# GLAD-RUC/FastEGNN

Hardware: AMD Instinct MI355X
Metric: graphs/sec (fwd+bwd), Water-3D-like 100k-node frame (higher is better)
Workload: dtype f32; 1 GPU; cfg4 Water-3D-like frame (SURVEY 8d): uniform points, radius graph r=0.035 (mean degree ~19), gravity on; 4-layer FastEGNN H=64, fwd+loss+bwd, CSR build inside the step; nodes=100000, edges=1919172, graphs_per_batch=1, virtual_channels=16, layers=4, parallelism=1 GPU, launch=whole step replayed as one captured HIP graph

## Files before the change

### fastegnn_amd/csrc/api.hip

```cpp
#include <vector>
#include "kernels.h"
#include <initializer_list>

namespace fe {

static thread_local std::string g_last_error;

void set_error(const std::string &msg) { g_last_error = msg; }

int check_launch(const char *what) {
  hipError_t e = hipGetLastError();
  if (e != hipSuccess) {
    set_error(std::string(what) + ": " + hipGetErrorString(e));
    return FASTEGNN_E_LAUNCH;
  }
  return FASTEGNN_OK;
}

bool g_prof_on = false;
namespace {
struct ProfRec { int id; hipEvent_t a, b; };
std::vector<ProfRec> g_recs;
std::vector<hipEvent_t> g_free;
std::vector<hipEvent_t> g_open(K_COUNT, nullptr);
hipEvent_t get_event() {
  if (!g_free.empty()) { hipEvent_t e = g_free.back(); g_free.pop_back(); return e; }
  hipEvent_t e; (void)hipEventCreate(&e); return e;
}
const char *kKernelNames[K_COUNT] = {
  "pack_kernel", "node_pre_fwd_kernel", "graph_xsum_kernel", "graph_pre_fwd_kernel", "edge_fwd_kernel",
  "virt_fwd_kernel", "graph_post_fwd_kernel", "graph_post_bwd_kernel", "virt_bwd_kernel", "graph_pre_bwd_kernel",
  "edge_bwd_kernel", "edge_col_reduce_kernel", "node_pre_bwd_kernel", "wgrad_tn_kernel", "wgrad_small_kernel",
  "build_csr", "misc", "wgrad_reduce_kernel", "virt_bwd_node_kernel", "virt_bwd_gv_kernel"};
}
void prof_begin(int id, hipStream_t st) {
  hipEvent_t e = get_event();
  (void)hipEventRecord(e, st);
  g_open[id] = e;
}
void prof_end(int id, hipStream_t st) {
  hipEvent_t e = get_event();
  (void)hipEventRecord(e, st);
  g_recs.push_back({id, g_open[id], e});
}

static int check_layer(const fastegnn_layer_t *L, const char *who) {
  if (!L) {
    set_error(std::string(who) + ": layer descriptor is null");
    return FASTEGNN_E_INVALID;
  }
  if (L->N < 0 || L->B < 1 || L->C < ((L->flags & FASTEGNN_F_EGNN) ? 0 : 1) || L->ea < 0 || L->na < 0) {
    set_error(std::string(who) + ": bad sizes");
    return FASTEGNN_E_INVALID;
  }
  if (!L->params) {
    set_error(std::string(who) + ": params null");
    return FASTEGNN_E_INVALID;
  }
  {
    const int act = (L->flags >> FASTEGNN_F_ACT_SHIFT) & FASTEGNN_F_ACT_MASK;
#ifdef FE_ACT_GENERIC
    if (act > FASTEGNN_ACT_SOFTPLUS) {
      set_error(std::string(who) + ": unknown activation kind in the flags");
      return FASTEGNN_E_INVALID;
    }
    if ((L->flags & FASTEGNN_F_BF16) && act != FASTEGNN_ACT_SILU) {
      set_error(std::string(who) + ": activations other than SiLU are not combined with the bf16 operand mode");
      return FASTEGNN_E_INVALID;
    }
#else
    if (act != FASTEGNN_ACT_SILU) {
      set_error(std::string(who) + ": this library is compiled for SiLU only; activations selected by the FASTEGNN_F_ACT bits "
                                   "need libfastegnn_hip_act.so (same sources, -DFE_ACT_GENERIC)");
      return FASTEGNN_E_INVALID;
    }
#endif
  }
  return FASTEGNN_OK;
}


enum GuardStage { G_GRAPH_POST, G_VIRT, G_GRAPH_PRE, G_EDGE, G_NODE_PRE };
static int guard_stage(const fastegnn_layer_t *L, const WgradBatch &wb, int stage) {
  const size_t N = (size_t)L->N, BC = (size_t)L->B * L->C, rows = wg_node_rows(L), E = (size_t)L->graph.n_edges;
  const bool det = has(L, FASTEGNN_F_DETERMINISTIC);
  struct W { const float *p; size_t n; const char *what; };
  auto guard = [&](std::initializer_list<W> ws) {
    for (const W &w : ws) {
      const int r = wb.guard_write(w.p, w.n, w.what);
      if (r) return r;
    }
    return (int)FASTEGNN_OK;
  };
  switch (stage) {
    case G_VIRT:
      return guard({{L->g_h, N * H, "g_h"}, {L->g_x, N * 3, "g_x"}, {L->g_A, N * H, "g_A"}, {L->g_aggm, N * H, "g_aggm"},
                    {L->g_aggx, N * 3, "g_aggx"}, {L->g_svel, N, "g_svel"}, {L->g_sgrav, N, "g_sgrav"}, {L->g_Bc, BC * H, "g_Bc"},
                    {L->g_Zp, BC * 3, "g_Zp"}, {L->wg_node, 2 * rows * H, "wg_node[0..2)"},
                    {L->wg_virt, L->wg_virt ? fastegnn_wg_virt_floats_for(L->N, L->C, L->flags) : 0, "wg_virt"}});
    case G_GRAPH_PRE:
      return guard({{L->g_HvT, BC * H, "g_HvT"}, {L->g_Z, BC * 3, "g_Z"}, {L->g_xbar, (size_t)L->B * 4, "g_xbar"},
                    {L->wg_node ? L->wg_node + 7 * rows * H : nullptr, rows * H, "wg_node[7..8)"}});
    case G_EDGE:
      return guard({{L->g_P, N * H, "g_P"}, {L->g_xrow, N * 3, "g_xrow"}, {det ? L->g_QXe : nullptr, E * QXLD, "g_QXe"},
                    {L->g_QX_src, (size_t)L->graph.n_src * QXLD, "g_QX_src"},
                    {L->wg_edge, fastegnn_wg_edge_floats(L->graph.n_edges), "wg_edge"}});
    case G_NODE_PRE:
      return guard({{L->g_h, N * H, "g_h"}, {L->g_x, N * 3, "g_x"}, {L->g_vel, N * 3, "g_vel"},
                    {L->wg_node ? L->wg_node + 2 * rows * H : nullptr, 2 * rows * H, "wg_node[2..4)"}});
    default: return FASTEGNN_OK;
  }
}

}

using namespace fe;

extern "C" int fastegnn_generic_activations(void) {
#ifdef FE_ACT_GENERIC
  return 1;
#else
  return 0;
#endif
}

#define STAGE(name, fn)                                               \
  int name(const fastegnn_layer_t *L, void *stream) {                 \
    int rc = check_layer(L, #name);                                   \
    if (rc) return rc;                                                \
    return fn(L, (hipStream_t)stream);                                \
  }

#define STAGE_B(name, fn, gid)                                        \
  int name(const fastegnn_layer_t *L, void *stream) {                 \
    int rc = check_layer(L, #name);                                   \
    if (rc) return rc;                                                \
    WgradBatch *wb = static_cast<WgradBatch *>(L->wgrad_batch);       \
    if (wb && (rc = guard_stage(L, *wb, gid))) return rc;             \
    return fn(L, (hipStream_t)stream, wb);                            \
  }

extern "C" {

const char *fastegnn_last_error(void) { return g_last_error.c_str(); }
int fastegnn_version(void) { return FASTEGNN_ABI_VERSION; }
size_t fastegnn_wpack_floats(int32_t C) { return wpack_floats(C); }
size_t fastegnn_wg_slab_floats(void) { return wg_slab_floats(); }
size_t fastegnn_sizeof_layer(void) { return sizeof(fastegnn_layer_t); }
size_t fastegnn_sizeof_graph(void) { return sizeof(fastegnn_graph_t); }

STAGE(fastegnn_pack_weights, pack_weights)
STAGE(fastegnn_node_pre_forward, node_pre_forward)
STAGE(fastegnn_graph_xsum, graph_xsum)
STAGE(fastegnn_graph_pre_forward, graph_pre_forward)
STAGE(fastegnn_edge_forward, edge_forward)
STAGE(fastegnn_virt_forward, virt_forward)
STAGE(fastegnn_graph_post_forward, graph_post_forward)
STAGE_B(fastegnn_graph_post_backward, graph_post_backward, G_GRAPH_POST)
STAGE_B(fastegnn_virt_backward, virt_backward, G_VIRT)
STAGE_B(fastegnn_graph_pre_backward, graph_pre_backward, G_GRAPH_PRE)
STAGE_B(fastegnn_edge_backward, edge_backward, G_EDGE)
STAGE(fastegnn_edge_col_reduce, edge_col_reduce)
STAGE_B(fastegnn_node_pre_backward, node_pre_backward, G_NODE_PRE)

int fastegnn_pack_weights_all(const fastegnn_layer_t *const *layers, int32_t n, void *stream) {
  FE_REQUIRE(layers && n >= 1, "fastegnn_pack_weights_all: no layers");
  for (int k = 0; k < n; ++k) {
    int rc = check_layer(layers[k], "fastegnn_pack_weights_all");
    if (rc) return rc;
  }
  return pack_weights_all(layers, n, (hipStream_t)stream);
}

int fastegnn_wgrad_batch_open(const fastegnn_layer_t *L, void *stream, void **batch) {
  FE_REQUIRE(L && batch && L->wg_slab, "fastegnn_wgrad_batch_open: null argument");
  WgradBatch *wb = new WgradBatch(L->wg_slab, (hipStream_t)stream, has(L, FASTEGNN_F_BF16));
  wb->max_split = 384;
  *batch = wb;
  return FASTEGNN_OK;
}
int fastegnn_wgrad_batch_close(void *batch) {
  if (!batch) return FASTEGNN_OK;
  WgradBatch *wb = static_cast<WgradBatch *>(batch);
  const int rc = wb->finish();
  delete wb;
  return rc;
}

int fastegnn_profile_enable(int32_t on) {
  g_prof_on = on != 0;
  return FASTEGNN_OK;
}
int32_t fastegnn_profile_kernels(void) { return K_COUNT; }
const char *fastegnn_profile_name(int32_t id) { return (id >= 0 && id < K_COUNT) ? kKernelNames[id] : ""; }
int fastegnn_profile_collect(double *total_ms, int64_t *launches) {
  if (!total_ms || !launches) { set_error("profile_collect: null output"); return FASTEGNN_E_INVALID; }
  for (int i = 0; i < K_COUNT; ++i) { total_ms[i] = 0.0; launches[i] = 0; }
  for (auto &r : g_recs) {
    float ms = 0.f;
    if (hipEventSynchronize(r.b) != hipSuccess || hipEventElapsedTime(&ms, r.a, r.b) != hipSuccess) {
      set_error("profile_collect: event query failed");
      return FASTEGNN_E_LAUNCH;
    }
    total_ms[r.id] += ms;
    launches[r.id] += 1;
    g_free.push_back(r.a);
    g_free.push_back(r.b);
  }
  g_recs.clear();
  return FASTEGNN_OK;
}

int fastegnn_layer_forward(const fastegnn_layer_t *L, void *stream) {
  int rc = check_layer(L, "fastegnn_layer_forward");
  if (rc) return rc;
  hipStream_t st = (hipStream_t)stream;
  if ((rc = pack_weights(L, st))) return rc;
  if ((rc = node_pre_forward(L, st))) return rc;
  if (has(L, FASTEGNN_F_EGNN)) {
    if ((rc = edge_forward(L, st))) return rc;
    return virt_forward(L, st);
  }
  if ((rc = graph_xsum(L, st))) return rc;
  if ((rc = graph_pre_forward(L, st))) return rc;
  if ((rc = edge_forward(L, st))) return rc;
  if ((rc = virt_forward(L, st))) return rc;
  return graph_post_forward(L, st);
}

int fastegnn_layer_backward(const fastegnn_layer_t *L, void *stream) {
  int rc = check_layer(L, "fastegnn_layer_backward");
  if (rc) return rc;
  hipStream_t st = (hipStream_t)stream;
  FE_REQUIRE(L->wg_slab, "fastegnn_layer_backward: wg_slab null");
  WgradBatch wb(L->wg_slab, st);
  wb.max_split = 384;
  auto guard_virt = [&]() { return guard_stage(L, wb, G_VIRT); };
  auto guard_edge = [&]() { return guard_stage(L, wb, G_EDGE); };
  auto guard_node_pre = [&]() { return guard_stage(L, wb, G_NODE_PRE); };
  if (has(L, FASTEGNN_F_EGNN)) {
    if ((rc = guard_virt())) return rc;
    if ((rc = virt_backward(L, st, &wb))) return rc;
    if ((rc = guard_edge())) return rc;
    if ((rc = edge_backward(L, st, &wb))) return rc;
    if ((rc = edge_col_reduce(L, st))) return rc;
    if ((rc = guard_node_pre())) return rc;
    if ((rc = node_pre_backward(L, st, &wb))) return rc;
    return wb.finish();
  }
  if ((rc = graph_post_backward(L, st, &wb))) return rc;
  if ((rc = guard_virt())) return rc;
  if ((rc = virt_backward(L, st, &wb))) return rc;
  if ((rc = guard_stage(L, wb, G_GRAPH_PRE))) return rc;
  if ((rc = graph_pre_backward(L, st, &wb))) return rc;
  if ((rc = guard_edge())) return rc;
  if ((rc = edge_backward(L, st, &wb))) return rc;
  if ((rc = edge_col_reduce(L, st))) return rc;
  if ((rc = guard_node_pre())) return rc;
  if ((rc = node_pre_backward(L, st, &wb))) return rc;
  return wb.finish();
}

}
```

### fastegnn_amd/csrc/common.h

```cpp
#pragma once
#include <hip/hip_runtime.h>
#include <stdint.h>

namespace fe {

typedef float f32x4 __attribute__((ext_vector_type(4)));

constexpr int H = 64;
constexpr int QXLD = 68;
constexpr int TS = 68;
constexpr int IMG = 4096;
constexpr int FEATW = 8;

struct Vec {
  f32x4 t[4];
};

__device__ __forceinline__ int lane_id() { return threadIdx.x & 63; }
__device__ __forceinline__ int wave_id() { return __builtin_amdgcn_readfirstlane((int)(threadIdx.x >> 6)); }
__device__ __forceinline__ int global_wave_id() { return (int)(blockIdx.x * (blockDim.x >> 6)) + wave_id(); }

__device__ __forceinline__ float sigmoid_f(float z) { return __builtin_amdgcn_rcpf(1.0f + __expf(-z)); }
__device__ __forceinline__ float silu_f(float z) { return z * sigmoid_f(z); }
__device__ __forceinline__ float dsilu_f(float z) {
  float s = sigmoid_f(z);
  return s * (1.0f + z * (1.0f - s));
}
__device__ __forceinline__ void silu_both(float z, float &y, float &d) {
  const float s = sigmoid_f(z);
  y = z * s;
  d = s + y * (1.0f - s);
}
__device__ __forceinline__ float rcp_f(float x) { return __builtin_amdgcn_rcpf(x); }
__device__ __forceinline__ float sqrt_f(float x) { return __builtin_amdgcn_sqrtf(x); }
__device__ __forceinline__ float tanh_f(float z) {
  const float z2 = z * z;
  const float p = z * (1.0f + z2 * (-0.33333334f + z2 * (0.13333334f + z2 * (-0.053968254f + z2 * 0.021869488f))));
  const float s = 2.0f * sigmoid_f(2.0f * z) - 1.0f;
  return fabsf(z) < 0.25f ? p : s;
}

__device__ __forceinline__ Vec vzero() {
  Vec v;
#pragma unroll
  for (int t = 0; t < 4; ++t) v.t[t] = f32x4{0.f, 0.f, 0.f, 0.f};
  return v;
}
template <typename F>
__device__ __forceinline__ Vec vmap(const Vec &a, F f) {
  Vec o;
#pragma unroll
  for (int t = 0; t < 4; ++t)
#pragma unroll
    for (int r = 0; r < 4; ++r) o.t[t][r] = f(a.t[t][r]);
  return o;
}
template <typename F>
__device__ __forceinline__ Vec vmap2(const Vec &a, const Vec &b, F f) {
  Vec o;
#pragma unroll
  for (int t = 0; t < 4; ++t)
#pragma unroll
    for (int r = 0; r < 4; ++r) o.t[t][r] = f(a.t[t][r], b.t[t][r]);
  return o;
}
__device__ __forceinline__ Vec vsilu(const Vec &a) { return vmap(a, [](float z) { return silu_f(z); }); }
__device__ __forceinline__ Vec vsilu_keep_d(Vec &z) {
  Vec y;
#pragma unroll
  for (int t = 0; t < 4; ++t)
#pragma unroll
    for (int r = 0; r < 4; ++r) {
      float yy, dd;
      silu_both(z.t[t][r], yy, dd);
      y.t[t][r] = yy;
      z.t[t][r] = dd;
    }
  return y;
}
struct Act {
  int kind;
  float p;
};
#ifdef FE_ACT_GENERIC
#define FE_ACT(a) , fe::Act{((a).flags >> FASTEGNN_F_ACT_SHIFT) & FASTEGNN_F_ACT_MASK, (a).act_param}
#define FE_ACT_P , Act act
#define FE_ACT_A , act
__device__ __forceinline__ float expm1_f(float z) {
  const float p = z * (1.0f + z * (0.5f + z * (0.16666667f + z * (0.041666668f + z * (0.008333334f + z * 0.0013888889f)))));
  return fabsf(z) < 0.3f ? p : __expf(z) - 1.0f;
}
__device__ __forceinline__ void act_both(float z, Act a, float &y, float &d) {
  switch (a.kind) {
    case FASTEGNN_ACT_RELU: y = z < 0.f ? 0.f : z; d = z > 0.f ? 1.f : 0.f; break;
    case FASTEGNN_ACT_LEAKY_RELU: y = z > 0.f ? z : a.p * z; d = z > 0.f ? 1.f : a.p; break;
    case FASTEGNN_ACT_TANH: y = tanh_f(z); d = 1.0f - y * y; break;
    case FASTEGNN_ACT_SIGMOID: y = sigmoid_f(z); d = y * (1.0f - y); break;
    case FASTEGNN_ACT_ELU: { const float e = a.p * expm1_f(z < 0.f ? z : 0.f); y = z <= 0.f ? e : z; d = z > 0.f ? 1.f : e + a.p; break; }
    case FASTEGNN_ACT_GELU: {
      const float c = 0.5f * (1.0f + erff(z * 0.70710678f));
      y = z * c;
      d = c + z * 0.3989422804f * __expf(-0.5f * z * z);
      break;
    }
    case FASTEGNN_ACT_SOFTPLUS: {
      const float bz = a.p * z;
      const float s = sigmoid_f(bz);
      y = bz <= 20.f ? log1pf(__expf(bz)) / a.p : z;
      d = bz > 20.f ? 1.f : s;
      break;
    }
    default: silu_both(z, y, d); break;
  }
}
__device__ __forceinline__ float act_f(float z, Act a) { float y, d; act_both(z, a, y, d); return y; }
__device__ __forceinline__ float dact_f(float z, Act a) { float y, d; act_both(z, a, y, d); return d; }
__device__ __forceinline__ Vec vsilu(const Vec &v, Act a) { return vmap(v, [a](float z) { return act_f(z, a); }); }
__device__ __forceinline__ Vec vsilu_keep_d(Vec &z, Act a) {
  Vec y;
#pragma unroll
  for (int t = 0; t < 4; ++t)
#pragma unroll
    for (int r = 0; r < 4; ++r) {
      float yy, dd;
      act_both(z.t[t][r], a, yy, dd);
      y.t[t][r] = yy;
      z.t[t][r] = dd;
    }
  return y;
}
__device__ __forceinline__ float dsilu_f(float z, Act a) { return dact_f(z, a); }
#else
#define FE_ACT(a)
#define FE_ACT_P
#define FE_ACT_A
#endif
__device__ __forceinline__ Vec vmul(const Vec &a, const Vec &b) {
  return vmap2(a, b, [](float x, float y) { return x * y; });
}
__device__ __forceinline__ Vec vscale(const Vec &a, float s) { return vmap(a, [s](float z) { return z * s; }); }
__device__ __forceinline__ void vaxpy(Vec &acc, float s, const Vec &a) {
#pragma unroll
  for (int t = 0; t < 4; ++t)
#pragma unroll
    for (int r = 0; r < 4; ++r) acc.t[t][r] = __builtin_fmaf(s, a.t[t][r], acc.t[t][r]);
}
__device__ __forceinline__ void vadd(Vec &acc, const Vec &a) {
#pragma unroll
  for (int t = 0; t < 4; ++t)
#pragma unroll
    for (int r = 0; r < 4; ++r) acc.t[t][r] += a.t[t][r];
}

__device__ __forceinline__ Vec vload_vec(const float *w, int q) {
  Vec v;
#pragma unroll
  for (int t = 0; t < 4; ++t) v.t[t] = *reinterpret_cast<const f32x4 *>(w + 16 * t + 4 * q);
  return v;
}
__device__ __forceinline__ Vec vload_row(const float *row, int q) { return vload_vec(row, q); }
__device__ __forceinline__ void vstore_row(float *row, int q, const Vec &v) {
#pragma unroll
  for (int t = 0; t < 4; ++t) *reinterpret_cast<f32x4 *>(row + 16 * t + 4 * q) = v.t[t];
}

__device__ __forceinline__ Vec vload_u(const float *base, unsigned off) {
  Vec v;
  const unsigned bo = off * 4u;
  const char *p = reinterpret_cast<const char *>(base);
#pragma unroll
  for (int t = 0; t < 4; ++t) v.t[t] = *reinterpret_cast<const f32x4 *>(p + (bo + 64u * t));
  return v;
}
__device__ __forceinline__ void vstore_u(float *base, unsigned off, const Vec &v) {
  const unsigned bo = off * 4u;
  char *p = reinterpret_cast<char *>(base);
#pragma unroll
  for (int t = 0; t < 4; ++t) *reinterpret_cast<f32x4 *>(p + (bo + 64u * t)) = v.t[t];
}

__device__ __forceinline__ float qsum(float p) {
  float a = p, b = p;
  asm("s_nop 1\n\tv_permlane16_swap_b32 %0, %1" : "+v"(a), "+v"(b));
  p = a + b;
  a = p; b = p;
  asm("s_nop 1\n\tv_permlane32_swap_b32 %0, %1" : "+v"(a), "+v"(b));
  return a + b;
}
__device__ __forceinline__ float jsum_dpp(float p) {
  p += __builtin_bit_cast(float, __builtin_amdgcn_update_dpp(0, __builtin_bit_cast(int, p), 0x128, 0xf, 0xf, false));
  p += __builtin_bit_cast(float, __builtin_amdgcn_update_dpp(0, __builtin_bit_cast(int, p), 0x124, 0xf, 0xf, false));
  p += __builtin_bit_cast(float, __builtin_amdgcn_update_dpp(0, __builtin_bit_cast(int, p), 0x122, 0xf, 0xf, false));
  p += __builtin_bit_cast(float, __builtin_amdgcn_update_dpp(0, __builtin_bit_cast(int, p), 0x121, 0xf, 0xf, false));
  return p;
}
__device__ __forceinline__ float jsum(float p) { return jsum_dpp(p); }
__device__ __forceinline__ float jreduce16(const Vec &u) {
  float y[8], z[4], w[2];
#pragma unroll
  for (int k = 0; k < 8; ++k) {
    const float a = u.t[k >> 2][k & 3], b = u.t[(k + 8) >> 2][k & 3];
    asm("s_nop 1\n\tv_add_f32_dpp %0, %1, %1 row_shl:8 row_mask:0xf bank_mask:0x3\n\t"
        "v_add_f32_dpp %0, %2, %2 row_shr:8 row_mask:0xf bank_mask:0xc"
        : "=&v"(y[k]) : "v"(a), "v"(b));
  }
#pragma unroll
  for (int k = 0; k < 4; ++k)
    asm("s_nop 1\n\tv_add_f32_dpp %0, %1, %1 row_shl:4 row_mask:0xf bank_mask:0x5\n\t"
        "v_add_f32_dpp %0, %2, %2 row_shr:4 row_mask:0xf bank_mask:0xa"
        : "=&v"(z[k]) : "v"(y[k]), "v"(y[k + 4]));
  const int lane = lane_id();
  const bool b1 = lane & 2, b0 = lane & 1;
#pragma unroll
  for (int k = 0; k < 2; ++k) {
    const float keep = b1 ? z[k + 2] : z[k], send = b1 ? z[k] : z[k + 2];
    w[k] = keep + __builtin_bit_cast(float, __builtin_amdgcn_update_dpp(0, __builtin_bit_cast(int, send), 0x4e, 0xf, 0xf, false));
  }
  const float keep = b0 ? w[1] : w[0], send = b0 ? w[0] : w[1];
  return keep + __builtin_bit_cast(float, __builtin_amdgcn_update_dpp(0, __builtin_bit_cast(int, send), 0xb1, 0xf, 0xf, false));
}
__device__ __forceinline__ void tile_sum_add(float *row, const Vec &u, int j, int q) {
  const float s = jreduce16(u);
  atomicAdd(&row[16 * (j >> 2) + 4 * q + (j & 3)], s);
}
__device__ __forceinline__ float vdot(const Vec &v, const Vec &w) {
  float p = 0.f;
#pragma unroll
  for (int t = 0; t < 4; ++t)
#pragma unroll
    for (int r = 0; r < 4; ++r) p += v.t[t][r] * w.t[t][r];
  return qsum(p);
}

#ifdef FE_STAMP_VF
__device__ unsigned long long g_vf_stamps[16];
struct VfStamp {
  unsigned long long prev, acc[12];
};
#define VF_TP , VfStamp &_vst
#define VF_TA , _vst
#define VF_T0() VfStamp _vst; for (int _k = 0; _k < 12; ++_k) _vst.acc[_k] = 0; _vst.prev = __builtin_amdgcn_s_memtime();
#define VF_T(i) { __builtin_amdgcn_sched_barrier(0); unsigned long long _t = __builtin_amdgcn_s_memtime(); \
                  _vst.acc[i] += _t - _vst.prev; _vst.prev = _t; __builtin_amdgcn_sched_barrier(0); }
#define VF_TEND() if (lane_id() == 0) { for (int _k = 0; _k < 12; ++_k) atomicAdd(&g_vf_stamps[_k], _vst.acc[_k]); }
#else
#define VF_TP
#define VF_TA
#define VF_T0()
#define VF_T(i)
#define VF_TEND()
#endif
#ifdef FE_STAMP
__device__ unsigned long long g_stamps[16];
struct Stamp {
  unsigned long long prev, acc[12];
};
#define FE_TP , Stamp &_st
#define FE_TA , _st
#define FE_T0() Stamp _st; for (int _k = 0; _k < 12; ++_k) _st.acc[_k] = 0; _st.prev = __builtin_amdgcn_s_memtime();
#define FE_T(i) { __builtin_amdgcn_sched_barrier(0); unsigned long long _t = __builtin_amdgcn_s_memtime(); \
                  _st.acc[i] += _t - _st.prev; _st.prev = _t; __builtin_amdgcn_sched_barrier(0); }
#define FE_TEND() if (lane_id() == 0) { for (int _k = 0; _k < 12; ++_k) atomicAdd(&g_stamps[_k], _st.acc[_k]); }
#elif defined(FE_ISA_MARK)
#define FE_TP
#define FE_TA
#define FE_T0()
#define FE_T(i) { __builtin_amdgcn_sched_barrier(0); asm volatile("; FE_MARK " #i); __builtin_amdgcn_sched_barrier(0); }
#define FE_TEND()
#else
#define FE_TP
#define FE_TA
#define FE_T0()
#define FE_T(i)
#define FE_TEND()
#endif

__host__ __device__ __forceinline__ int img_index(int o, int k) {
  int t = o >> 4, i = o & 15, tp = k >> 4, q = (k >> 2) & 3, r = k & 3;
  return ((t * 4 + tp) * 64 + q * 16 + i) * 4 + r;
}

__device__ __forceinline__ void gemm64(const float *img, const Vec &in, Vec &acc) {
  const f32x4 *ip = reinterpret_cast<const f32x4 *>(img) + lane_id();
#pragma unroll
  for (int tp = 0; tp < 4; ++tp) {
    f32x4 a[4];
#pragma unroll
    for (int t = 0; t < 4; ++t) a[t] = ip[(t * 4 + tp) * 64];
#pragma unroll
    for (int r = 0; r < 4; ++r)
#pragma unroll
      for (int t = 0; t < 4; ++t)
        acc.t[t] = __builtin_amdgcn_mfma_f32_16x16x4f32(a[t][r], in.t[tp][r], acc.t[t], 0, 0, 0);
  }
}

typedef unsigned u32x4 __attribute__((ext_vector_type(4)));
typedef __bf16 bf16x8 __attribute__((ext_vector_type(8)));
constexpr int IMG3 = 3 * 2048;

struct Split {
  u32x4 p[3][2];
};
__device__ __forceinline__ unsigned f2u(float x) { return __builtin_bit_cast(unsigned, x); }
__device__ __forceinline__ unsigned part_pack(float &a0, float &a1) {
  typedef float f32x2_ __attribute__((ext_vector_type(2)));
  typedef __bf16 bf16x2_ __attribute__((ext_vector_type(2)));
  const unsigned p = __builtin_bit_cast(unsigned, __builtin_convertvector(f32x2_{a0, a1}, bf16x2_));
  a0 -= __builtin_bit_cast(float, p << 16);
  a1 -= __builtin_bit_cast(float, p & 0xffff0000u);
  return p;
}
__host__ __device__ __forceinline__ int img3_index(int part, int o, int k) {
  const int t = o >> 4, i = o & 15, tile = k >> 4, q = (k >> 2) & 3, r = k & 3;
  const int s = tile >> 1, e = ((tile & 1) << 2) | r;
  return part * 2048 + ((t * 2 + s) * 64 + q * 16 + i) * 4 + (e >> 1);
}
__device__ __forceinline__ unsigned split_word(float w0, float w1, int part) {
  float a0 = w0, a1 = w1;
  unsigned p = 0;
  for (int k = 0; k <= part; ++k) p = part_pack(a0, a1);
  return p;
}
__device__ __forceinline__ Split vsplit(const Vec &v) {
  Split S;
#pragma unroll
  for (int s = 0; s < 2; ++s) {
    float x[8];
#pragma unroll
    for (int e = 0; e < 8; ++e) x[e] = v.t[2 * s + (e >> 2)][e & 3];
#pragma unroll
    for (int w = 0; w < 4; ++w) {
      S.p[0][s][w] = part_pack(x[2 * w], x[2 * w + 1]);
      S.p[1][s][w] = part_pack(x[2 * w], x[2 * w + 1]);
      S.p[2][s][w] = part_pack(x[2 * w], x[2 * w + 1]);
    }
  }
  return S;
}
__device__ __forceinline__ void gemm64_x3(const unsigned *img3, const Split &in, Vec &acc) {
  const u32x4 *ip = reinterpret_cast<const u32x4 *>(img3) + lane_id();
  __builtin_amdgcn_sched_barrier(0);
  u32x4 fr[2][3];
#pragma unroll
  for (int p = 0; p < 3; ++p) fr[0][p] = ip[p * 512];
  __builtin_amdgcn_sched_group_barrier(0x100, 3, 0);
#pragma unroll
  for (int g = 0; g < 8; ++g) {
    const int s = g >> 2, t = g & 3, cb = g & 1;
    if (g + 1 < 8) {
      const int sn = (g + 1) >> 2, tn = (g + 1) & 3;
#pragma unroll
      for (int p = 0; p < 3; ++p) fr[cb ^ 1][p] = ip[p * 512 + (tn * 2 + sn) * 64];
      __builtin_amdgcn_sched_group_barrier(0x100, 3, 0);
    }
    const bf16x8 ah = __builtin_bit_cast(bf16x8, fr[cb][0]), am = __builtin_bit_cast(bf16x8, fr[cb][1]),
                 al = __builtin_bit_cast(bf16x8, fr[cb][2]);
    const bf16x8 xh = __builtin_bit_cast(bf16x8, in.p[0][s]);
    const bf16x8 xm = __builtin_bit_cast(bf16x8, in.p[1][s]);
    const bf16x8 xl = __builtin_bit_cast(bf16x8, in.p[2][s]);
    acc.t[t] = __builtin_amdgcn_mfma_f32_16x16x32_bf16(al, xh, acc.t[t], 0, 0, 0);
    acc.t[t] = __builtin_amdgcn_mfma_f32_16x16x32_bf16(am, xm, acc.t[t], 0, 0, 0);
    acc.t[t] = __builtin_amdgcn_mfma_f32_16x16x32_bf16(ah, xl, acc.t[t], 0, 0, 0);
    acc.t[t] = __builtin_amdgcn_mfma_f32_16x16x32_bf16(am, xh, acc.t[t], 0, 0, 0);
    acc.t[t] = __builtin_amdgcn_mfma_f32_16x16x32_bf16(ah, xm, acc.t[t], 0, 0, 0);
    acc.t[t] = __builtin_amdgcn_mfma_f32_16x16x32_bf16(ah, xh, acc.t[t], 0, 0, 0);
    __builtin_amdgcn_sched_group_barrier(0x008, 6, 0);
  }
  __builtin_amdgcn_sched_barrier(0);
}
__device__ __forceinline__ void gemm64_x3(const unsigned *img3, const Vec &in, Vec &acc) { gemm64_x3(img3, vsplit(in), acc); }

typedef float f32x2 __attribute__((ext_vector_type(2)));
typedef __bf16 bf16x2 __attribute__((ext_vector_type(2)));
__device__ __forceinline__ unsigned pack_rne(float x0, float x1) {
  return __builtin_bit_cast(unsigned, __builtin_convertvector(f32x2{x0, x1}, bf16x2));
}
__device__ __forceinline__ float round_bf(float x) { return (float)(__bf16)x; }
struct BfOp {
  u32x4 p[2];
};
__device__ __forceinline__ BfOp vpack_bf(const Vec &v) {
  BfOp B;
#pragma unroll
  for (int s = 0; s < 2; ++s)
#pragma unroll
    for (int w = 0; w < 4; ++w) {
      const int e = 2 * w;
      B.p[s][w] = pack_rne(v.t[2 * s + (e >> 2)][e & 3], v.t[2 * s + ((e + 1) >> 2)][(e + 1) & 3]);
    }
  return B;
}
__device__ __forceinline__ Vec vround(const Vec &v) { return vmap(v, [](float z) { return round_bf(z); }); }
__device__ __forceinline__ void gemm64_b1(const unsigned *img3, const BfOp &in, Vec &acc) {
  const u32x4 *ip = reinterpret_cast<const u32x4 *>(img3) + lane_id();
#pragma unroll
  for (int s = 0; s < 2; ++s) {
    const bf16x8 x = __builtin_bit_cast(bf16x8, in.p[s]);
#pragma unroll
    for (int t = 0; t < 4; ++t)
      acc.t[t] = __builtin_amdgcn_mfma_f32_16x16x32_bf16(__builtin_bit_cast(bf16x8, ip[(t * 2 + s) * 64]), x, acc.t[t], 0, 0, 0);
  }
}

constexpr int RM_RS = 144;
constexpr int RM_PART = 64 * RM_RS;
constexpr int RM_BYTES = 3 * RM_PART;
constexpr int RM_WORDS = RM_BYTES / 4;
typedef unsigned u32x2 __attribute__((ext_vector_type(2)));
typedef short s16x4 __attribute__((ext_vector_type(4)));
__device__ __forceinline__ u32x2 lds_tr_read(const char *p) {
  return __builtin_bit_cast(u32x2, __builtin_amdgcn_ds_read_tr16_b64_v4i16(
                                       (__attribute__((address_space(3))) s16x4 *)(p)));
}
template <bool TR>
__device__ __forceinline__ bf16x8 rm_frag(const char *img, int part, int t, int s) {
  const int l = lane_id(), i = l & 15, q = l >> 4;
  u32x2 lo, hi;
  if constexpr (TR) {
    const char *p = img + part * RM_PART + (32 * s + 4 * q + (i >> 2)) * RM_RS + (16 * t + 4 * (i & 3)) * 2;
    lo = lds_tr_read(p);
    hi = lds_tr_read(p + 16 * RM_RS);
  } else {
    const char *p = img + part * RM_PART + (16 * t + i) * RM_RS + (32 * s + 4 * q) * 2;
    typedef __attribute__((address_space(3))) const volatile u32x2 *lds_vu32x2;
    lo = *(lds_vu32x2)(p);
    hi = *(lds_vu32x2)(p + 32);
  }
  return __builtin_bit_cast(bf16x8, u32x4{lo[0], lo[1], hi[0], hi[1]});
}
template <bool TR, bool PIPE = true>
__device__ __forceinline__ void gemm64_x3_rm(const char *img, const Split &in, Vec &acc) {
  if constexpr (!PIPE) {
#pragma unroll
  for (int s = 0; s < 2; ++s)
#pragma unroll
    for (int t = 0; t < 4; ++t) {
      const bf16x8 ah = rm_frag<TR>(img, 0, t, s), am = rm_frag<TR>(img, 1, t, s), al = rm_frag<TR>(img, 2, t, s);
      const bf16x8 xh = __builtin_bit_cast(bf16x8, in.p[0][s]);
      const bf16x8 xm = __builtin_bit_cast(bf16x8, in.p[1][s]);
      const bf16x8 xl = __builtin_bit_cast(bf16x8, in.p[2][s]);
      acc.t[t] = __builtin_amdgcn_mfma_f32_16x16x32_bf16(al, xh, acc.t[t], 0, 0, 0);
      acc.t[t] = __builtin_amdgcn_mfma_f32_16x16x32_bf16(am, xm, acc.t[t], 0, 0, 0);
      acc.t[t] = __builtin_amdgcn_mfma_f32_16x16x32_bf16(ah, xl, acc.t[t], 0, 0, 0);
      acc.t[t] = __builtin_amdgcn_mfma_f32_16x16x32_bf16(am, xh, acc.t[t], 0, 0, 0);
      acc.t[t] = __builtin_amdgcn_mfma_f32_16x16x32_bf16(ah, xm, acc.t[t], 0, 0, 0);
      acc.t[t] = __builtin_amdgcn_mfma_f32_16x16x32_bf16(ah, xh, acc.t[t], 0, 0, 0);
    }
  } else {
  __builtin_amdgcn_sched_barrier(0);
  bf16x8 fr[2][3];
#pragma unroll
  for (int p = 0; p < 3; ++p) fr[0][p] = rm_frag<TR>(img, p, 0, 0);
  __builtin_amdgcn_sched_group_barrier(0x100, 6, 0);
#pragma unroll
  for (int g = 0; g < 8; ++g) {
    const int s = g >> 2, t = g & 3, cb = g & 1;
    if (g + 1 < 8) {
#pragma unroll
      for (int p = 0; p < 3; ++p) fr[cb ^ 1][p] = rm_frag<TR>(img, p, (g + 1) & 3, (g + 1) >> 2);
      __builtin_amdgcn_sched_group_barrier(0x100, 6, 0);
    }
    const bf16x8 ah = fr[cb][0], am = fr[cb][1], al = fr[cb][2];
    const bf16x8 xh = __builtin_bit_cast(bf16x8, in.p[0][s]);
    const bf16x8 xm = __builtin_bit_cast(bf16x8, in.p[1][s]);
    const bf16x8 xl = __builtin_bit_cast(bf16x8, in.p[2][s]);
    acc.t[t] = __builtin_amdgcn_mfma_f32_16x16x32_bf16(al, xh, acc.t[t], 0, 0, 0);
    acc.t[t] = __builtin_amdgcn_mfma_f32_16x16x32_bf16(am, xm, acc.t[t], 0, 0, 0);
    acc.t[t] = __builtin_amdgcn_mfma_f32_16x16x32_bf16(ah, xl, acc.t[t], 0, 0, 0);
    acc.t[t] = __builtin_amdgcn_mfma_f32_16x16x32_bf16(am, xh, acc.t[t], 0, 0, 0);
    acc.t[t] = __builtin_amdgcn_mfma_f32_16x16x32_bf16(ah, xm, acc.t[t], 0, 0, 0);
    acc.t[t] = __builtin_amdgcn_mfma_f32_16x16x32_bf16(ah, xh, acc.t[t], 0, 0, 0);
    __builtin_amdgcn_sched_group_barrier(0x008, 6, 0);
  }
  __builtin_amdgcn_sched_barrier(0);
  }
}
template <bool TR>
__device__ __forceinline__ void gemm64_b1_rm(const char *img, const BfOp &in, Vec &acc) {
#pragma unroll
  for (int s = 0; s < 2; ++s) {
    const bf16x8 x = __builtin_bit_cast(bf16x8, in.p[s]);
#pragma unroll
    for (int t = 0; t < 4; ++t) acc.t[t] = __builtin_amdgcn_mfma_f32_16x16x32_bf16(rm_frag<TR>(img, 0, t, s), x, acc.t[t], 0, 0, 0);
  }
}

struct Split8 {
  u32x4 h, m, l;
};
__device__ __forceinline__ Split8 split8(const float (&x_)[8]) {
  float x[8];
#pragma unroll
  for (int e = 0; e < 8; ++e) x[e] = x_[e];
  Split8 S;
#pragma unroll
  for (int w = 0; w < 4; ++w) {
    S.h[w] = part_pack(x[2 * w], x[2 * w + 1]);
    S.m[w] = part_pack(x[2 * w], x[2 * w + 1]);
    S.l[w] = part_pack(x[2 * w], x[2 * w + 1]);
  }
  return S;
}
__device__ __forceinline__ u32x4 round8(const float (&x)[8]) {
  u32x4 r;
#pragma unroll
  for (int w = 0; w < 4; ++w) r[w] = pack_rne(x[2 * w], x[2 * w + 1]);
  return r;
}

typedef _Float16 f16x8 __attribute__((ext_vector_type(8)));
typedef _Float16 f16x2 __attribute__((ext_vector_type(2)));
constexpr float F2_UP = 2048.f, F2_DOWN = 1.0f / 2048.f;
struct Split2 {
  u32x4 p[2][2];
};
__device__ __forceinline__ void part2_pack(float a0, float a1, unsigned &ph, unsigned &pl) {
  const unsigned h = __builtin_bit_cast(unsigned, __builtin_convertvector(f32x2{a0, a1}, f16x2));
  float r0, r1;
  asm("v_fma_mix_f32 %0, %1, -1.0, %2 op_sel_hi:[1,0,0]" : "=v"(r0) : "v"(h), "v"(a0));
  asm("v_fma_mix_f32 %0, %1, -1.0, %2 op_sel:[1,0,0] op_sel_hi:[1,0,0]" : "=v"(r1) : "v"(h), "v"(a1));
  unsigned l;
  asm("v_fma_mixlo_f16 %0, %1, %3, 0\n\tv_fma_mixhi_f16 %0, %2, %3, 0\n\ts_nop 1" : "=&v"(l) : "v"(r0), "v"(r1), "s"(F2_UP));
  ph = h;
  pl = l;
}
__device__ __forceinline__ unsigned split2_word(float w0, float w1, int part) {
  unsigned h, l;
  part2_pack(w0, w1, h, l);
  return part == 0 ? h : l;
}
#ifdef FE_HAZARD_SELFTEST
#define FE_MIX_PAD ""
#else
#define FE_MIX_PAD "s_nop 1"
#endif
template <bool IN_PLACE = false>
__device__ __forceinline__ void mix_pack4(const float (&r)[8], float sc, unsigned (&l)[4]) {
  if constexpr (IN_PLACE) {
#pragma unroll
    for (int w = 0; w < 4; ++w) l[w] = f2u(r[2 * w]);
    asm("v_fma_mixlo_f16 %0, %0, %8, 0\n\tv_fma_mixhi_f16 %0, %4, %8, 0\n\t"
        "v_fma_mixlo_f16 %1, %1, %8, 0\n\tv_fma_mixhi_f16 %1, %5, %8, 0\n\t"
        "v_fma_mixlo_f16 %2, %2, %8, 0\n\tv_fma_mixhi_f16 %2, %6, %8, 0\n\t"
        "v_fma_mixlo_f16 %3, %3, %8, 0\n\tv_fma_mixhi_f16 %3, %7, %8, 0\n\t"
        FE_MIX_PAD
        : "+v"(l[0]), "+v"(l[1]), "+v"(l[2]), "+v"(l[3])
        : "v"(r[1]), "v"(r[3]), "v"(r[5]), "v"(r[7]), "v"(sc));
  } else {
  asm("v_fma_mixlo_f16 %0, %4, %12, 0\n\tv_fma_mixhi_f16 %0, %5, %12, 0\n\t"
      "v_fma_mixlo_f16 %1, %6, %12, 0\n\tv_fma_mixhi_f16 %1, %7, %12, 0\n\t"
      "v_fma_mixlo_f16 %2, %8, %12, 0\n\tv_fma_mixhi_f16 %2, %9, %12, 0\n\t"
      "v_fma_mixlo_f16 %3, %10, %12, 0\n\tv_fma_mixhi_f16 %3, %11, %12, 0\n\t"
      FE_MIX_PAD
      : "=&v"(l[0]), "=&v"(l[1]), "=&v"(l[2]), "=&v"(l[3])
      : "v"(r[0]), "v"(r[1]), "v"(r[2]), "v"(r[3]), "v"(r[4]), "v"(r[5]), "v"(r[6]), "v"(r[7]), "v"(sc));
  }
}
__device__ __forceinline__ Split2 vsplit2(const Vec &v) {
  Split2 S;
#pragma unroll
  for (int s = 0; s < 2; ++s) {
    float r[8];
#pragma unroll
    for (int w = 0; w < 4; ++w) {
      const int e = 2 * w;
      const float a0 = v.t[2 * s + (e >> 2)][e & 3], a1 = v.t[2 * s + ((e + 1) >> 2)][(e + 1) & 3];
      const unsigned h = __builtin_bit_cast(unsigned, __builtin_convertvector(f32x2{a0, a1}, f16x2));
      asm("v_fma_mix_f32 %0, %1, -1.0, %2 op_sel_hi:[1,0,0]" : "=v"(r[e]) : "v"(h), "v"(a0));
      asm("v_fma_mix_f32 %0, %1, -1.0, %2 op_sel:[1,0,0] op_sel_hi:[1,0,0]" : "=v"(r[e + 1]) : "v"(h), "v"(a1));
      S.p[0][s][w] = h;
    }
    unsigned l[4];
    mix_pack4<true>(r, F2_UP, l);
#pragma unroll
    for (int w = 0; w < 4; ++w) S.p[1][s][w] = l[w];
  }
  return S;
}
#ifndef FE_F2_PIPE_FWD
#define FE_F2_PIPE_FWD 1
#endif
template <bool PIPE = false>
__device__ __forceinline__ void gemm64_f2(const unsigned *img3, const Split2 &in, Vec &acc, int off4 = 0) {
  const u32x4 *ip = reinterpret_cast<const u32x4 *>(img3) + (lane_id() + off4);
  const f16x8 xh0 = __builtin_bit_cast(f16x8, in.p[0][0]), xh1 = __builtin_bit_cast(f16x8, in.p[0][1]);
  const f16x8 xl0 = __builtin_bit_cast(f16x8, in.p[1][0]), xl1 = __builtin_bit_cast(f16x8, in.p[1][1]);
  if constexpr (PIPE && FE_F2_PIPE_FWD != 0) {
  __builtin_amdgcn_sched_barrier(0);
  u32x4 fr[2][4];
#pragma unroll
  for (int k = 0; k < 4; ++k) fr[0][k] = ip[(k >> 1) * 512 + (k & 1) * 64];
  __builtin_amdgcn_sched_group_barrier(0x100, 4, 0);
  f32x4 lo_p = {0.f, 0.f, 0.f, 0.f}, hi_p = {0.f, 0.f, 0.f, 0.f};
#pragma unroll
  for (int t = 0; t < 4; ++t) {
    const int cb = t & 1;
// ... 437 lines not shown
```

### fastegnn_amd/csrc/kernels.h

```cpp
#pragma once
#include <hip/hip_runtime.h>
#include <string>
#include "../../include/fastegnn_hip.h"
#include "common.h"

namespace fe {

void set_error(const std::string &msg);
int check_launch(const char *what);

#define FE_REQUIRE(cond, msg)            \
  do {                                   \
    if (!(cond)) {                       \
      fe::set_error(msg);                \
      return FASTEGNN_E_INVALID;         \
    }                                    \
  } while (0)

inline bool has(const fastegnn_layer_t *L, int f) { return (L->flags & f) != 0; }
inline int cdiv(long a, long b) { return (int)((a + b - 1) / b); }

enum KernelId {
  K_PACK = 0, K_NODE_PRE_FWD, K_XSUM, K_GRAPH_PRE_FWD, K_EDGE_FWD, K_VIRT_FWD, K_GRAPH_POST_FWD,
  K_GRAPH_POST_BWD, K_VIRT_BWD, K_GRAPH_PRE_BWD, K_EDGE_BWD, K_COL_REDUCE, K_NODE_PRE_BWD,
  K_WGRAD_TN, K_WGRAD_SMALL, K_CSR, K_MISC, K_WGRAD_REDUCE, K_VIRT_BWD_NODE, K_VIRT_BWD_GV, K_COUNT
};
extern bool g_prof_on;
void prof_begin(int id, hipStream_t st);
void prof_end(int id, hipStream_t st);
struct ProfScope {
  int id; hipStream_t st; bool on;
  ProfScope(int id_, hipStream_t st_) : id(id_), st(st_), on(g_prof_on) { if (on) prof_begin(id, st); }
  ~ProfScope() { if (on) prof_end(id, st); }
};

constexpr int WGV_PAD = 16;
constexpr int WG_MAX_JOBS = 24;
constexpr int WG_SLABS = 8192;
struct WgJob {
  const float *G, *T;
  float *dW, *db;
  long M, sG, sT, sW;
  int ldg, ldt, lddw, c0, ks, kmax, rows_per_wg, nsplit, nb, wg_begin, slab_begin;
  int round;
};
struct WgTable {
  WgJob job[WG_MAX_JOBS];
  float *slab, *slab_b;
  int n_jobs;
};
struct WgradBatch {
  WgTable tab;
  hipStream_t st;
  int n_wg, n_slab, max_nb;
  bool round;
  int min_rows;
  int max_split;
  int slab_base, slab_cap;
  int slab_top;
  bool planned;
  WgradBatch(float *slab, hipStream_t st, bool round_bf16 = false, int slab_base = 0, int slab_cap = WG_SLABS / 2);
  int add(const float *G, int ldg, const float *T, int ldt, long M, float *dW, int lddw, int c0, int ks, float *db,
          int nb = 1, long sG = 0, long sT = 0, long sW = 0, int kmax = 64);
  int plan();
  int add_slabs(float *dW, int lddw, int c0, int ks, float *db, int nsplit, int *slab_begin);
  int add_slabs_ext(const float *ext, float *dW, int lddw, int c0, int ks, int nsplit, int nb, long sW);
  int finish();
  int guard_write(const float *p, size_t n, const char *what) const;
};
inline size_t wg_slab_floats() { return (size_t)WG_SLABS * (IMG + H); }
int launch_dgrad_small(const float *G, long N, int kf, const float *W, int ldw, int c0, float *g_in, int accumulate,
                       hipStream_t st);
int launch_wgrad_small(const float *G, int ldg, const float *F, int ldf, int kf, long M, float *dW, int lddw, int c0,
                       hipStream_t st);

int csr_chunk_count(int E);
void launch_chunk_rows(const int32_t *rowptr, int n_rows, int n_chunks, int32_t *chunk_row, hipStream_t st);

int pack_weights(const fastegnn_layer_t *L, hipStream_t st);
int pack_weights_all(const fastegnn_layer_t *const *layers, int n, hipStream_t st);
int node_pre_forward(const fastegnn_layer_t *L, hipStream_t st);
int graph_xsum(const fastegnn_layer_t *L, hipStream_t st);
int graph_pre_forward(const fastegnn_layer_t *L, hipStream_t st);
int edge_forward(const fastegnn_layer_t *L, hipStream_t st);
int virt_forward(const fastegnn_layer_t *L, hipStream_t st);
int graph_post_forward(const fastegnn_layer_t *L, hipStream_t st);
int graph_post_backward(const fastegnn_layer_t *L, hipStream_t st, WgradBatch *shared = nullptr);
int virt_backward(const fastegnn_layer_t *L, hipStream_t st, WgradBatch *shared = nullptr);
int graph_pre_backward(const fastegnn_layer_t *L, hipStream_t st, WgradBatch *shared = nullptr);
int edge_backward(const fastegnn_layer_t *L, hipStream_t st, WgradBatch *shared = nullptr);
size_t virt_pc_wg_floats(size_t N, size_t C);
bool virt_cs_applies(long N, int C, int flags);
size_t virt_cs_wg_floats(size_t C);
int edge_col_reduce(const fastegnn_layer_t *L, hipStream_t st);
int node_pre_backward(const fastegnn_layer_t *L, hipStream_t st, WgradBatch *shared = nullptr);
inline size_t wg_node_rows(const fastegnn_layer_t *L) { const size_t bc = (size_t)L->B * L->C; return (size_t)L->N > bc ? (size_t)L->N : bc; }

}
```

### fastegnn_amd/csrc/layer_bwd.hip

```cpp
#include "stages.h"

namespace fe {

__device__ __forceinline__ Vec vdsilu_mul(const Vec &g, const Vec &z FE_ACT_P) {
  return vmap2(g, z, [=](float a, float b) { return a * dsilu_f(b FE_ACT_A); });
}

__device__ __forceinline__ void vec_reduce_lds(float *red_row, const Vec &acc, int j, int q) {
#pragma unroll
  for (int t = 0; t < 4; ++t)
#pragma unroll
    for (int r = 0; r < 4; ++r) {
      float s = jsum(acc.t[t][r]);
      if (j == 0) atomicAdd(&red_row[16 * t + 4 * q + r], s);
    }
}

struct GraphPostBwdArgs {
  const float *xsum, *HvT, *poolV, *g_Z_out, *g_HvT_out, *wpack, *b5;
  float *g_Z, *g_HvT, *g_poolV, *g_poolX, *wg_u, *wg_gz5, *wg_pm;
  int B, C, flags;
  float act_param = 0.f;
};
__global__ __launch_bounds__(256) void graph_post_bwd_kernel(GraphPostBwdArgs a) {
  const bool bf = a.flags & FASTEGNN_F_BF16;
  auto rb = [&](const Vec &v) { return bf ? vround(v) : v; };
  const int l = lane_id(), j = l & 15, q = l >> 4;
  const int wave = global_wave_id(), nwaves = (gridDim.x * blockDim.x) >> 6;
  const int M = a.B * a.C, ntiles = (M + 15) >> 4;
  for (int i = blockIdx.x * blockDim.x + threadIdx.x; i < a.B * 3 * a.C; i += gridDim.x * blockDim.x) {
    const int b = i / (3 * a.C);
    const float g = a.g_Z_out[i];
    a.g_Z[i] = g;
    a.g_poolX[i] = g / fmaxf(a.xsum[b * 4 + 3], 1.f);
  }
  if (a.flags & FASTEGNN_F_RF) {
    for (int i = blockIdx.x * blockDim.x + threadIdx.x; i < M * H; i += gridDim.x * blockDim.x) {
      a.g_HvT[i] = a.g_HvT_out[i];
      a.g_poolV[i] = 0.f;
    }
    return;
  }
  for (int tile = wave; tile < ntiles; tile += nwaves) {
    const int m = tile * 16 + j;
    const bool valid = m < M;
    const int mc = valid ? m : M - 1;
    const int b = mc / a.C;
    const float inv = 1.0f / fmaxf(a.xsum[b * 4 + 3], 1.f);
    const Vec hv = vload_row(a.HvT + (size_t)mc * H, q);
    const Vec pm = vscale(vload_row(a.poolV + (size_t)mc * H, q), inv);
    Vec z5 = vload_vec(a.b5, q);
    gemm64(a.wpack + (size_t)I_W5A * IMG, rb(hv), z5);
    gemm64(a.wpack + (size_t)I_W5B * IMG, rb(pm), z5);
    const Vec g_out = vload_row(a.g_HvT_out + (size_t)mc * H, q);
    Vec g_u = vzero();
    gemm64(a.wpack + (size_t)I_W6T * IMG, rb(g_out), g_u);
    const Vec g_z5 = vdsilu_mul(g_u, z5 FE_ACT(a));
    Vec g_hv = (a.flags & FASTEGNN_F_RESIDUAL) ? g_out : vzero();
    gemm64(a.wpack + (size_t)I_W5AT * IMG, rb(g_z5), g_hv);
    Vec g_pm = vzero();
    gemm64(a.wpack + (size_t)I_W5BT * IMG, rb(g_z5), g_pm);
    if (valid) {
      vstore_row(a.wg_u + (size_t)m * H, q, vsilu(z5 FE_ACT(a)));
      vstore_row(a.wg_gz5 + (size_t)m * H, q, g_z5);
      vstore_row(a.wg_pm + (size_t)m * H, q, pm);
      vstore_row(a.g_HvT + (size_t)m * H, q, g_hv);
      vstore_row(a.g_poolV + (size_t)m * H, q, vscale(g_pm, inv));
    }
  }
}

__global__ __launch_bounds__(256) void graph_post_bwd_coords_kernel(const float *xsum, const float *g_Z_out, float *g_Z, float *g_poolX,
                                                                    float *g_HvT, int B, int C) {
  for (int i = blockIdx.x * blockDim.x + threadIdx.x; i < B * 3 * C; i += gridDim.x * blockDim.x) {
    const int b = i / (3 * C);
    const float g = g_Z_out[i];
    g_Z[i] = g;
    g_poolX[i] = g / fmaxf(xsum[b * 4 + 3], 1.f);
  }
  for (int i = blockIdx.x * blockDim.x + threadIdx.x; i < B * C * H; i += gridDim.x * blockDim.x) g_HvT[i] = 0.f;
}

int graph_post_backward(const fastegnn_layer_t *L, hipStream_t st, WgradBatch *shared) {
  if (!L->g_HvT_out && !has(L, FASTEGNN_F_RF)) {
    FE_REQUIRE(!L->g_h_out, "graph_post_backward: g_HvT_out is null and g_h_out is not (both null: no gradient for h / Hv; otherwise neither)");
    FE_REQUIRE(L->xsum && L->g_Z_out && L->g_Z && L->g_HvT && L->g_poolX, "graph_post_backward: null buffer");
    int grid = cdiv((long)L->B * L->C * H, 256);
    if (grid > 256) grid = 256;
    if (grid < 1) grid = 1;
    { ProfScope _ps_graph_post_bwd_kernel(K_GRAPH_POST_BWD, st); hipLaunchKernelGGL(graph_post_bwd_coords_kernel, dim3(grid), dim3(256), 0, st, L->xsum, L->g_Z_out, L->g_Z, L->g_poolX, L->g_HvT, L->B, L->C); }
    return check_launch("graph_post_bwd_coords_kernel");
  }
  FE_REQUIRE(L->xsum && L->HvT && L->poolV && L->g_Z_out && L->g_HvT_out && L->g_Z && L->g_HvT && L->g_poolV &&
                 L->g_poolX && L->wg_node && L->grads && L->wpack,
             "graph_post_backward: null buffer");
  const long M = (long)L->B * L->C;
  float *wg_gp = L->wg_node + 4 * wg_node_rows(L) * H;
  float *wg_u = wg_gp, *wg_gz5 = wg_gp + M * H, *wg_pm = wg_gp + 2 * M * H;
  GraphPostBwdArgs a{L->xsum, L->HvT, L->poolV, L->g_Z_out, L->g_HvT_out, L->wpack, L->params[FASTEGNN_P_NODEV0_B],
                     L->g_Z, L->g_HvT, L->g_poolV, L->g_poolX, wg_u, wg_gz5, wg_pm, L->B, L->C, L->flags, L->act_param};
  int grid = cdiv(cdiv(M, 16), 4);
  if (grid > 256) grid = 256;
  if (grid < 1) grid = 1;
  { ProfScope _ps_graph_post_bwd_kernel(K_GRAPH_POST_BWD, st); hipLaunchKernelGGL(graph_post_bwd_kernel, dim3(grid), dim3(256), 0, st, a); }
  int rc = check_launch("graph_post_bwd_kernel");
  if (rc) return rc;
  if (has(L, FASTEGNN_F_RF)) return FASTEGNN_OK;
  float *const *g = L->grads;
  WgradBatch local(L->wg_slab, st);
  WgradBatch &wb = shared ? *shared : local;
  wb.round = has(L, FASTEGNN_F_BF16);
  if ((rc = wb.add(L->g_HvT_out, H, wg_u, H, M, g[FASTEGNN_P_NODEV2_W], H, 0, 1, g[FASTEGNN_P_NODEV2_B]))) return rc;
  if ((rc = wb.add(wg_gz5, H, L->HvT, H, M, g[FASTEGNN_P_NODEV0_W], 2 * H, 0, 1, g[FASTEGNN_P_NODEV0_B]))) return rc;
  if ((rc = wb.add(wg_gz5, H, wg_pm, H, M, g[FASTEGNN_P_NODEV0_W], 2 * H, H, 1, nullptr))) return rc;
  return shared ? FASTEGNN_OK : wb.finish();
}


struct GraphPreBwdArgs {
  const float *xsum, *Z, *g_Bc, *g_Zp, *V0W;
  float *g_Z, *g_HvT, *g_xbar, *wg_mxt;
  int B, C, bf16;
};
constexpr int GPB_SPLIT = 4;
__global__ __launch_bounds__(256) void graph_pre_bwd_kernel(GraphPreBwdArgs a) {
  extern __shared__ float sm[];
  const int C = a.C, b = blockIdx.x, ld = 2 * H + 1 + C;
  const int i0 = blockIdx.y * 256 + threadIdx.x, istep = 256 * gridDim.y;
  float *mz = sm;
  float *gmX = sm + 3 * C;
  float *gmz = gmX + C * C;
  const float cnt = fmaxf(a.xsum[b * 4 + 3], 1.f);
  for (int i = threadIdx.x; i < 3 * C; i += 256) mz[i] = a.Z[(size_t)b * 3 * C + i] - a.xsum[b * 4 + i / C] / cnt;
  __syncthreads();
  for (int i = i0; i < C * H; i += istep) {
    int c = i >> 6, d = i & 63;
    float v = 0.f;
    if (d < C) v = mz[c] * mz[d] + mz[C + c] * mz[C + d] + mz[2 * C + c] * mz[2 * C + d];
    a.wg_mxt[((size_t)b * C + c) * H + d] = v;
  }
  for (int i = i0; i < C * H; i += istep) {
    int c = i >> 6, k = i & 63;
    const float *gb = a.g_Bc + ((size_t)b * C + c) * H;
    float acc = 0.f;
    if (a.bf16) { for (int o = 0; o < H; ++o) acc += round_bf(gb[o]) * round_bf(a.V0W[(size_t)o * ld + H + k]); }
    else { for (int o = 0; o < H; ++o) acc += gb[o] * a.V0W[(size_t)o * ld + H + k]; }
    a.g_HvT[((size_t)b * C + c) * H + k] += acc;
  }
  for (int i = threadIdx.x; i < C * C; i += 256) {
    int cp = i / C, c = i % C;
    const float *gb = a.g_Bc + ((size_t)b * C + c) * H;
    float acc = 0.f;
    for (int o = 0; o < H; ++o) acc += gb[o] * a.V0W[(size_t)o * ld + 2 * H + 1 + cp];
    gmX[cp * C + c] = acc;
  }
  __syncthreads();
  for (int i = threadIdx.x; i < 3 * C; i += 256) {
    int k = i / C, c = i % C;
    float acc = 0.f;
    for (int d = 0; d < C; ++d) acc += (gmX[c * C + d] + gmX[d * C + c]) * mz[k * C + d];
    gmz[i] = acc;
    if (i % gridDim.y == blockIdx.y) a.g_Z[(size_t)b * 3 * C + i] += acc + a.g_Zp[(size_t)b * 3 * C + i];
  }
  __syncthreads();
  if (threadIdx.x < 3 && blockIdx.y == 0) {
    float acc = 0.f;
    for (int c = 0; c < C; ++c) acc += gmz[threadIdx.x * C + c];
    a.g_xbar[b * 3 + threadIdx.x] = -acc / cnt;
  }
}
int graph_pre_backward(const fastegnn_layer_t *L, hipStream_t st, WgradBatch *shared) {
  FE_REQUIRE(L->xsum && L->Z && L->HvT && L->g_Bc && L->g_Zp && L->g_Z && L->g_HvT && L->g_xbar && L->wg_node && L->grads,
             "graph_pre_backward: null buffer");
  const long M = (long)L->B * L->C;
  float *wg_mxt = L->wg_node + 7 * wg_node_rows(L) * H;
  GraphPreBwdArgs a{L->xsum, L->Z, L->g_Bc, L->g_Zp, L->params[FASTEGNN_P_VIRT0_W], L->g_Z, L->g_HvT, L->g_xbar, wg_mxt,
                    L->B, L->C, has(L, FASTEGNN_F_BF16) ? 1 : 0};
  const size_t lds = (size_t)(6 * L->C + L->C * L->C) * sizeof(float);
  { ProfScope _ps_graph_pre_bwd_kernel(K_GRAPH_PRE_BWD, st); hipLaunchKernelGGL(graph_pre_bwd_kernel, dim3(L->B, GPB_SPLIT), dim3(256), lds, st, a); }
  int rc = check_launch("graph_pre_bwd_kernel");
  if (rc) return rc;
  float *const *g = L->grads;
  const int ld = 2 * H + 1 + L->C;
  WgradBatch local(L->wg_slab, st);
  WgradBatch &wb = shared ? *shared : local;
  wb.round = has(L, FASTEGNN_F_BF16);
  if ((rc = wb.add(L->g_Bc, H, L->HvT, H, M, g[FASTEGNN_P_VIRT0_W], ld, H, 1, g[FASTEGNN_P_VIRT0_B]))) return rc;
  wb.round = false;
  if ((rc = wb.add(L->g_Bc, H, wg_mxt, H, M, g[FASTEGNN_P_VIRT0_W], ld, 2 * H + 1, 1, nullptr, 1, 0, 0, 0, L->C))) return rc;
  return shared ? FASTEGNN_OK : wb.finish();
}

struct EdgeBwdArgs {
  EdgeArgs f;
  const float *g_aggm, *g_aggx;
  float *g_P, *g_xrow, *g_QXe;
  float *g_QXs_atomic;
  float *g_ea;
  float *d_wx2, *d_attw, *d_attb, *d_bx2;
  float *d_wr, *d_we;
  int ld_e0, C;
  float *slab, *slab_b;
  int slab_w2, slab_wx1;
  float *cons_scratch;
};
#ifndef FE_PC_PRIO
#define FE_PC_PRIO 3
#endif

#ifndef FE_PC_WAVES
#define FE_PC_WAVES 8
#endif
constexpr int PC_WAVES = FE_PC_WAVES;
constexpr int PC_CONS = 3, PC_CONS2 = 7;
constexpr int PC_PROD = PC_WAVES - 2;
#ifndef FE_PC_CONS32
#define FE_PC_CONS32 1
#endif
#ifndef FE_PC_RING
#define FE_PC_RING 3
#endif
constexpr int PC_RING = FE_PC_RING;
#ifndef FE_PC_FLUSH
#define FE_PC_FLUSH 48
#endif
constexpr int PC_FLUSH = FE_PC_FLUSH;
constexpr int PC_RS = 68;
constexpr int PC_SLOT = 2 * 16 * PC_RS;
template <int MODE> constexpr int pc_img_floats() { return 2 * (rm_lds_bytes<MODE>() / 4); }
enum { PC_HEAD = 0, PC_TOTAL = 2, PC_FILLED = 4, PC_DRAINED = 4 + 2 * PC_RING, PC_CTRL = 4 + 4 * PC_RING };
#ifdef FE_SAFE_WAITS
__device__ __forceinline__ int lds_ld(const int *p) { return __hip_atomic_load(p, __ATOMIC_ACQUIRE, __HIP_MEMORY_SCOPE_WORKGROUP); }
__device__ __forceinline__ void lds_st(int *p, int v) { __hip_atomic_store(p, v, __ATOMIC_RELEASE, __HIP_MEMORY_SCOPE_WORKGROUP); }
#else
__device__ __forceinline__ int lds_ld(const int *p) { return __atomic_load_n(p, __ATOMIC_RELAXED); }
__device__ __forceinline__ void lds_st(int *p, int v) { __atomic_store_n(p, v, __ATOMIC_RELAXED); }
#endif
__device__ __forceinline__ void pc_tile_store(float *tile, int j, int q, const Vec &v) {
#pragma unroll
  for (int t = 0; t < 4; ++t) *reinterpret_cast<f32x4 *>(tile + j * PC_RS + 16 * t + 4 * q) = v.t[t];
}
template <int MODE, int EA>
__global__ __launch_bounds__(64 * PC_WAVES) void edge_bwd_pc_kernel(EdgeBwdArgs A) {
  extern __shared__ __attribute__((aligned(16))) float lds[];
#ifdef FE_ISA_CONST
  A.f.flags = FE_ISA_CONST; A.f.ea_dim = 2; A.f.bx2 = nullptr; A.f.attw = nullptr; A.g_ea = nullptr; A.d_bx2 = nullptr;
#endif
  const EdgeArgs &a = A.f;
  float *img = lds;
  float *vec = lds + pc_img_floats<MODE>();
  float *tiles = vec + EV_COUNT * H;
  float *ring = tiles + PC_PROD * 16 * TS;
  int *ctrl = reinterpret_cast<int *>(ring + 2 * PC_RING * PC_SLOT);
  {
    constexpr int RMS = rm_lds_bytes<MODE>();
    const char *src = wpack_rm(a.wpack, A.C, (MODE == GM_F16 ? RM_F16 : 0) + 3);
    for (int i = threadIdx.x; i < 2 * (RMS / 16); i += blockDim.x) {
      const int im = i / (RMS / 16), k = i % (RMS / 16);
      reinterpret_cast<u32x4 *>(reinterpret_cast<char *>(img) + im * RMS)[k] = reinterpret_cast<const u32x4 *>(src + (size_t)im * RM_BYTES)[k];
    }
  }
  edge_load_vecs(vec, a);
  if (threadIdx.x < PC_CTRL) ctrl[threadIdx.x] = 0;
  __syncthreads();
  const int l = lane_id(), j = l & 15, q = l >> 4, wv = wave_id();
  const bool consumer = wv == PC_CONS || wv == PC_CONS2;
  const int ckind = wv == PC_CONS ? 0 : 1;
  const int pw = wv - (wv > PC_CONS ? 1 : 0) - (wv > PC_CONS2 ? 1 : 0);
  float *pt = tiles + (consumer ? 0 : pw) * 16 * TS;
  const int wave = (int)blockIdx.x * PC_PROD + pw, nwaves = (int)gridDim.x * PC_PROD;
  const bool mean = !(a.flags & FASTEGNN_F_COORDS_SUM);
  float accW[8] = {0.f, 0.f, 0.f, 0.f, 0.f, 0.f, 0.f, 0.f};
  const bool tanh_on = a.flags & FASTEGNN_F_TANH, att_on = a.flags & FASTEGNN_F_ATTENTION,
             norm_on = a.flags & FASTEGNN_F_NORMALIZE;
  Vec acc_wx2 = vzero(), acc_att = vzero();
  float acc_attb = 0.f, acc_bx2 = 0.f;
  FE_T0()
  int r0 = 0, r1 = 0, e0 = 0, e1 = 0;
  if (!consumer) {
    const int c0 = (int)((long)wave * a.n_chunks / nwaves), c1 = (int)((long)(wave + 1) * a.n_chunks / nwaves);
    r0 = a.chunk_row[c0];
    r1 = a.chunk_row[c1];
    if (r0 < r1) {
      e0 = a.rowptr[r0];
      e1 = a.rowptr[r1];
      if (l == 0) atomicAdd(&ctrl[PC_TOTAL], (e1 - e0 + 15) >> 4);
    }
  }
  __syncthreads();
  auto publish = [&](int kind, const Vec &Gv, const Vec &Tv) {
    int tk = 0;
    if (l == 0) tk = atomicAdd(&ctrl[PC_HEAD + kind], 1);
    tk = __builtin_amdgcn_readfirstlane(tk);
    const int sl = tk % PC_RING, round = tk / PC_RING;
    while (lds_ld(&ctrl[PC_DRAINED + kind * PC_RING + sl]) != round) __builtin_amdgcn_s_sleep(2);
    __builtin_amdgcn_fence(__ATOMIC_ACQUIRE, "workgroup", "local");
    float *slot = ring + (kind * PC_RING + sl) * PC_SLOT;
    pc_tile_store(slot, j, q, Gv);
    pc_tile_store(slot + 16 * PC_RS, j, q, Tv);
    __builtin_amdgcn_fence(__ATOMIC_RELEASE, "workgroup", "local");
    if (l == 0) lds_st(&ctrl[PC_FILLED + kind * PC_RING + sl], round + 1);
  };
  constexpr bool CONS32 = MODE == GM_F16 && FE_PC_CONS32 != 0;
  if (CONS32 && consumer) {
    if constexpr (CONS32) {
#if FE_PC_PRIO
    __builtin_amdgcn_s_setprio(FE_PC_PRIO);
#endif
    const int total = lds_ld(&ctrl[PC_TOTAL]);
    WgAcc32 acc;
    wg32_zero(acc);
    WgScale sG{0}, sT{0};
    double bs[2] = {0., 0.};
    auto scp = [&](int blk, int e4) {
      char *b = reinterpret_cast<char *>(A.cons_scratch + ((size_t)blockIdx.x * 2 + ckind) * IMG) + (size_t)((blk * 4 + e4) * 64 * 16);
      asm volatile("" : "+s"(b));
      return reinterpret_cast<f32x4 *>(b + (unsigned)l * 16u);
    };
    bool flushed = false;
    const size_t sl = (size_t)(ckind == 0 ? A.slab_w2 : A.slab_wx1) + blockIdx.x;
    auto flush = [&](bool last) {
      const float ig = sG.inv(), it = sT.inv();
      float *slab_dst = A.slab + sl * IMG;
#pragma unroll
      for (int bo = 0; bo < 2; ++bo)
#pragma unroll
        for (int bk = 0; bk < 2; ++bk)
#pragma unroll
          for (int e4 = 0; e4 < 4; ++e4) {
            f32x4 v;
#pragma unroll
            for (int r = 0; r < 4; ++r) v[r] = (acc.c[bo][bk][4 * e4 + r] * ig) * it;
            f32x4 *d = scp(bo * 2 + bk, e4);
            if (flushed) v += *d;
            if (!last) {
              *d = v;
            } else {
#pragma unroll
              for (int r = 0; r < 4; ++r) slab_dst[(32 * bo + 8 * e4 + 4 * (l >> 5) + r) * H + 32 * bk + (l & 31)] = v[r];
            }
#pragma unroll
            for (int r = 0; r < 4; ++r) acc.c[bo][bk][4 * e4 + r] = 0.f;
          }
    };
    int since = 0;
    for (int done = 0; done < total; ++done) {
      const int s0 = done % PC_RING, r0w = done / PC_RING;
      while (lds_ld(&ctrl[PC_FILLED + ckind * PC_RING + s0]) != r0w + 1) __builtin_amdgcn_s_sleep(1);
      __builtin_amdgcn_fence(__ATOMIC_ACQUIRE, "workgroup", "local");
      const float *g0 = ring + (ckind * PC_RING + s0) * PC_SLOT;
      float xg[2][8], xt[2][8];
      wg32_read<PC_RS>(g0, xg);
      wg32_read<PC_RS>(g0 + 16 * PC_RS, xt);
      __builtin_amdgcn_fence(__ATOMIC_RELEASE, "workgroup", "local");
      __builtin_amdgcn_s_waitcnt(0xc07f);
      if (l == 0) lds_st(&ctrl[PC_DRAINED + ckind * PC_RING + s0], r0w + 1);
      const float f = sG.update_lazy(xg) * sT.update_lazy(xt);
      if (f != 1.f) wg32_scale_acc(acc, f);
      const WgOp32 G = wg32_split(xg, sG.scale()), T = wg32_split(xt, sT.scale());
#pragma unroll
      for (int b = 0; b < 2; ++b)
        bs[b] += (double)(((xg[b][0] + xg[b][1]) + (xg[b][2] + xg[b][3])) + ((xg[b][4] + xg[b][5]) + (xg[b][6] + xg[b][7])));
      wg32_mma(acc, G, T);
      if (++since >= PC_FLUSH && done + 1 < total) {
        flush(false);
        flushed = true;
        since = 0;
      }
    }
    flush(true);
#pragma unroll
    for (int b = 0; b < 2; ++b) {
      double s0 = bs[b];
      s0 += __shfl_xor(s0, 32);
      if (l < 32) A.slab_b[sl * H + 32 * b + l] = (float)s0;
    }
    }
  } else if (consumer) {
#if FE_PC_PRIO
    __builtin_amdgcn_s_setprio(FE_PC_PRIO);
#endif
    const int total = lds_ld(&ctrl[PC_TOTAL]);
    f32x4 accA[4][4];
    double bsA[4] = {0., 0., 0., 0.};
#pragma unroll
    for (int ti = 0; ti < 4; ++ti)
#pragma unroll
      for (int tk = 0; tk < 4; ++tk) accA[ti][tk] = f32x4{0.f, 0.f, 0.f, 0.f};
    auto contract = [&](int kind, int tk, f32x4 (&acc)[4][4], double (&bs)[4]) {
      const int s0 = tk % PC_RING, r0w = tk / PC_RING;
      const bool two = tk + 1 < total;
      const int s1 = (tk + 1) % PC_RING, r1w = (tk + 1) / PC_RING;
      while (lds_ld(&ctrl[PC_FILLED + kind * PC_RING + s0]) != r0w + 1) __builtin_amdgcn_s_sleep(2);
      if (two)
        while (lds_ld(&ctrl[PC_FILLED + kind * PC_RING + s1]) != r1w + 1) __builtin_amdgcn_s_sleep(2);
      __builtin_amdgcn_fence(__ATOMIC_ACQUIRE, "workgroup", "local");
      const float *g0 = ring + (kind * PC_RING + s0) * PC_SLOT, *g1 = ring + (kind * PC_RING + s1) * PC_SLOT;
      float xb[4][8], xa[4][8];
#pragma unroll
      for (int t = 0; t < 4; ++t)
#pragma unroll
        for (int e = 0; e < 4; ++e) {
          xb[t][e] = g0[16 * PC_RS + (4 * q + e) * PC_RS + 16 * t + j];
          xb[t][4 + e] = two ? g1[16 * PC_RS + (4 * q + e) * PC_RS + 16 * t + j] : 0.f;
          xa[t][e] = g0[(4 * q + e) * PC_RS + 16 * t + j];
          xa[t][4 + e] = two ? g1[(4 * q + e) * PC_RS + 16 * t + j] : 0.f;
        }
      __builtin_amdgcn_fence(__ATOMIC_RELEASE, "workgroup", "local");
      __builtin_amdgcn_s_waitcnt(0xc07f);
      if (l == 0) {
        lds_st(&ctrl[PC_DRAINED + kind * PC_RING + s0], r0w + 1);
        if (two) lds_st(&ctrl[PC_DRAINED + kind * PC_RING + s1], r1w + 1);
      }
      Split8 B[4];
#pragma unroll
      for (int t = 0; t < 4; ++t) {
        if constexpr (MODE == GM_BF16) B[t].h = round8(xb[t]);
        else B[t] = split8(xb[t]);
      }
#pragma unroll
      for (int ti = 0; ti < 4; ++ti) {
        const float (&x)[8] = xa[ti];
        bs[ti] += (double)(((x[0] + x[1]) + (x[2] + x[3])) + ((x[4] + x[5]) + (x[6] + x[7])));
        if constexpr (MODE == GM_BF16) {
          const bf16x8 ah = __builtin_bit_cast(bf16x8, round8(x));
#pragma unroll
          for (int t = 0; t < 4; ++t)
            acc[ti][t] = __builtin_amdgcn_mfma_f32_16x16x32_bf16(ah, __builtin_bit_cast(bf16x8, B[t].h), acc[ti][t], 0, 0, 0);
          continue;
        }
        const Split8 Aop = split8(x);
        const bf16x8 ah = __builtin_bit_cast(bf16x8, Aop.h), am = __builtin_bit_cast(bf16x8, Aop.m),
                     al = __builtin_bit_cast(bf16x8, Aop.l);
#pragma unroll
        for (int t = 0; t < 4; ++t) {
          const bf16x8 bh = __builtin_bit_cast(bf16x8, B[t].h), bm = __builtin_bit_cast(bf16x8, B[t].m),
                       bl = __builtin_bit_cast(bf16x8, B[t].l);
          f32x4 c = acc[ti][t];
          c = __builtin_amdgcn_mfma_f32_16x16x32_bf16(al, bh, c, 0, 0, 0);
          c = __builtin_amdgcn_mfma_f32_16x16x32_bf16(am, bm, c, 0, 0, 0);
          c = __builtin_amdgcn_mfma_f32_16x16x32_bf16(ah, bl, c, 0, 0, 0);
          c = __builtin_amdgcn_mfma_f32_16x16x32_bf16(am, bh, c, 0, 0, 0);
          c = __builtin_amdgcn_mfma_f32_16x16x32_bf16(ah, bm, c, 0, 0, 0);
          c = __builtin_amdgcn_mfma_f32_16x16x32_bf16(ah, bh, c, 0, 0, 0);
          acc[ti][t] = c;
        }
      }
    };
    auto ready = [&](int kind, int done) {
      const int s0 = done % PC_RING, s1 = (done + 1) % PC_RING;
      if (lds_ld(&ctrl[PC_FILLED + kind * PC_RING + s0]) != done / PC_RING + 1) return false;
      return done + 1 >= total || lds_ld(&ctrl[PC_FILLED + kind * PC_RING + s1]) == (done + 1) / PC_RING + 1;
    };
    f32x4 *sc = reinterpret_cast<f32x4 *>(A.cons_scratch + ((size_t)blockIdx.x * 2 + ckind) * IMG) + l;
    double bs_tot[4] = {0., 0., 0., 0.};
    bool flushed = false;
    int done = 0, since = 0;
    while (done < total) {
      if (ready(ckind, done)) {
        contract(ckind, done, accA, bsA);
        done += 2;
        since += 2;
        if (since >= PC_FLUSH && done < total) {
#pragma unroll
          for (int ti = 0; ti < 4; ++ti) {
#pragma unroll
            for (int tk2 = 0; tk2 < 4; ++tk2) {
              f32x4 *d = sc + (ti * 4 + tk2) * 64;
              if (flushed) accA[ti][tk2] += *d;
              *d = accA[ti][tk2];
              accA[ti][tk2] = f32x4{0.f, 0.f, 0.f, 0.f};
            }
            bs_tot[ti] += bsA[ti];
            bsA[ti] = 0.;
          }
          flushed = true;
          since = 0;
        }
      } else {
        __builtin_amdgcn_s_sleep(1);
      }
// ... 529 lines not shown
```

### fastegnn_amd/csrc/layer_fwd.hip

```cpp
#include <cstdlib>
#include "stages.h"

namespace fe {

struct NodePreArgs {
  const float *h, *x, *wpack;
  const float *b1, *bv0, *wv2, *bv2, *bg0, *wg2, *bg2;
  float *P, *QX, *A, *svel, *sgrav;
  int N, gravity, has_vel;
  const float *vel, *wv0;
  int C;
  int flags = 0;
  float act_param = 0.f;
};

template <int MODE>
__global__ __launch_bounds__(64 * NODE_PRE_WAVES) void node_pre_fwd_kernel(NodePreArgs a) {
  extern __shared__ __attribute__((aligned(16))) float lds[];
  unsigned *img = reinterpret_cast<unsigned *>(lds);
  float *vec = lds + 5 * IMG3;
  const int nimg = a.gravity ? 5 : 4;
  load_images_x3(img, wpack_x3(a.wpack, a.C, I_W1A), nimg);
  if constexpr (edge_fold_first<MODE>()) { for (int i = threadIdx.x; i < H; i += blockDim.x) vec[i] = a.b1 ? a.b1[i] * LOG2E_F : 0.f; }
  else load_floats(vec + 0 * H, a.b1, H);
  load_floats(vec + 1 * H, a.bv0, H);
  load_floats(vec + 2 * H, a.wv2, H);
  load_floats(vec + 3 * H, a.bg0, H);
  load_floats(vec + 4 * H, a.wg2, H);
  load_floats(vec + 5 * H, a.wv0, H);
  __syncthreads();
  const int l = lane_id(), j = l & 15, q = l >> 4;
  const int wave = global_wave_id(), nwaves = (gridDim.x * blockDim.x) >> 6;
  const int ntiles = (a.N + 15) >> 4;
  const float bv2 = (a.has_vel || a.wv0) ? a.bv2[0] : 0.f;
  const float bg2 = a.gravity ? a.bg2[0] : 0.f;
  for (int tile = wave; tile < ntiles; tile += nwaves) {
    const int n = tile * 16 + j;
    const bool valid = n < a.N;
    const int nc = valid ? n : a.N - 1;
    const typename OperandOf<MODE>::type hv = make_operand<MODE>(vload_row(a.h + (size_t)nc * H, q));
    Vec acc = vload_vec(vec, q);
    gemm_op<MODE>(img, 0, hv, acc);
    if (valid) vstore_row(a.P + (size_t)n * H, q, acc);
    acc = vzero();
    gemm_op<MODE>(img, 1, hv, acc);
    if (valid) {
      vstore_row(a.QX + (size_t)n * QXLD, q, acc);
      if (q == 0) {
        f32x4 xv = {a.x[(size_t)n * 3], a.x[(size_t)n * 3 + 1], a.x[(size_t)n * 3 + 2], 0.f};
        *reinterpret_cast<f32x4 *>(a.QX + (size_t)n * QXLD + H) = xv;
      }
    }
    acc = vzero();
    gemm_op<MODE>(img, 2, hv, acc);
    if (valid) vstore_row(a.A + (size_t)n * H, q, acc);
    float s = 0.f;
    if (a.has_vel) {
      acc = vload_vec(vec + 1 * H, q);
      gemm_op<MODE>(img, 3, hv, acc);
      s = vdot(vsilu(acc FE_ACT(a)), vload_vec(vec + 2 * H, q)) + bv2;
    } else if (a.wv0) {
      const float vx = a.vel[(size_t)nc * 3], vy = a.vel[(size_t)nc * 3 + 1], vz = a.vel[(size_t)nc * 3 + 2];
      acc = vload_vec(vec + 1 * H, q);
      vaxpy(acc, sqrt_f(vx * vx + vy * vy + vz * vz), vload_vec(vec + 5 * H, q));
      s = vdot(vsilu(acc FE_ACT(a)), vload_vec(vec + 2 * H, q)) + bv2;
    }
    if (valid && q == 0) a.svel[n] = s;
    if (a.gravity) {
      acc = vload_vec(vec + 3 * H, q);
      gemm_op<MODE>(img, 4, hv, acc);
      s = vdot(vsilu(acc FE_ACT(a)), vload_vec(vec + 4 * H, q)) + bg2;
      if (valid && q == 0) a.sgrav[n] = s;
    }
  }
}

int node_pre_forward(const fastegnn_layer_t *L, hipStream_t st) {
  FE_REQUIRE(L->h && L->x && L->wpack && L->P && L->QX && L->A && L->svel, "node_pre_forward: null buffer");
  if (L->N == 0) return FASTEGNN_OK;
  const bool grav = has(L, FASTEGNN_F_GRAVITY);
  FE_REQUIRE(!grav || L->sgrav, "node_pre_forward: sgrav null");
  const float *const *p = L->params;
  NodePreArgs a{L->h, L->x, L->wpack, p[FASTEGNN_P_EDGE0_B], p[FASTEGNN_P_VEL0_B], p[FASTEGNN_P_VEL2_W],
                p[FASTEGNN_P_VEL2_B], p[FASTEGNN_P_GRAV0_B], p[FASTEGNN_P_GRAV2_W], p[FASTEGNN_P_GRAV2_B],
                L->P, L->QX, L->A, L->svel, L->sgrav, L->N, grav ? 1 : 0,
                (p[FASTEGNN_P_VEL0_W] && !has(L, FASTEGNN_F_RF)) ? 1 : 0,
                L->vel, has(L, FASTEGNN_F_RF) ? p[FASTEGNN_P_VEL0_W] : nullptr, L->C, L->flags, L->act_param};
  FE_REQUIRE(!has(L, FASTEGNN_F_RF) || (L->vel && p[FASTEGNN_P_VEL0_W] && p[FASTEGNN_P_VEL0_B] && p[FASTEGNN_P_VEL2_W] &&
                                         p[FASTEGNN_P_VEL2_B]),
             "node_pre_forward: FastRF needs vel and the coord_mlp_vel parameters");
  const int ntiles = (L->N + 15) / 16;
  int grid = cdiv(ntiles, NODE_PRE_WAVES);
  if (grid > 256) grid = 256;
  const size_t lds = (5 * IMG3 + 6 * H) * sizeof(float);
  {
    ProfScope _ps_node_pre_fwd_kernel(K_NODE_PRE_FWD, st);
    if (has(L, FASTEGNN_F_BF16)) hipLaunchKernelGGL(node_pre_fwd_kernel<GM_BF16>, dim3(grid), dim3(64 * NODE_PRE_WAVES), lds, st, a);
    else hipLaunchKernelGGL(node_pre_fwd_kernel<GM_NODE_PRE_FWD>, dim3(grid), dim3(64 * NODE_PRE_WAVES), lds, st, a);
  }
  return check_launch("node_pre_fwd_kernel");
}

#ifndef FE_XSUM_PER_WAVE
#define FE_XSUM_PER_WAVE 1024
#endif
constexpr int XSUM_PER_WAVE = FE_XSUM_PER_WAVE;
__global__ __launch_bounds__(256) void graph_xsum_kernel(const float *x, const int32_t *batch, int N, float *xsum, int PER_WAVE) {
  const int l = lane_id();
  const int n0 = global_wave_id() * PER_WAVE, n1 = min(N, n0 + PER_WAVE);
  if (n0 >= n1) return;
  int cur = -1;
  float s[4] = {0.f, 0.f, 0.f, 0.f};
  auto flush = [&]() {
    float mine = 0.f;
#pragma unroll
    for (int k = 0; k < 4; ++k) {
      float v = s[k];
      for (int off = 32; off > 0; off >>= 1) v += __shfl_xor(v, off);
      if (l == k) mine = v;
      s[k] = 0.f;
    }
    if (l < 4) atomicAdd(&xsum[cur * 4 + l], mine);
  };
  for (int base = n0; base < n1; base += 64) {
    const int n = base + l;
    const bool ok = n < n1;
    const int b = batch[ok ? n : n1 - 1];
    const int bf = __builtin_amdgcn_readfirstlane(b), bl = batch[min(base + 63, n1 - 1)];
    float xv[3] = {0.f, 0.f, 0.f};
    if (ok) { xv[0] = x[(size_t)n * 3]; xv[1] = x[(size_t)n * 3 + 1]; xv[2] = x[(size_t)n * 3 + 2]; }
    if (bf == bl) {
      if (bf != cur) {
        if (cur >= 0) flush();
        cur = bf;
      }
      s[0] += xv[0]; s[1] += xv[1]; s[2] += xv[2]; s[3] += ok ? 1.f : 0.f;
    } else {
      if (cur >= 0) flush();
      cur = -1;
      const int bb = ok ? b : -1;
      float v[4] = {xv[0], xv[1], xv[2], ok ? 1.f : 0.f};
#pragma unroll
      for (int off = 1; off < 64; off <<= 1) {
        const int bu = __shfl_up(bb, off);
        float u[4];
#pragma unroll
        for (int k = 0; k < 4; ++k) u[k] = __shfl_up(v[k], off);
        if (l >= off && bu == bb) {
#pragma unroll
          for (int k = 0; k < 4; ++k) v[k] += u[k];
        }
      }
      const int bn = __shfl_down(bb, 1);
      if (ok && (l == 63 || bn != bb)) {
#pragma unroll
        for (int k = 0; k < 4; ++k) atomicAdd(&xsum[b * 4 + k], v[k]);
      }
    }
  }
  if (cur >= 0) flush();
}

int graph_xsum(const fastegnn_layer_t *L, hipStream_t st) {
  FE_REQUIRE(L->xsum && L->batch && L->x, "graph_xsum: null buffer");
  (void)hipMemsetAsync(L->xsum, 0, (size_t)L->B * 4 * sizeof(float), st);
  int per_wave = (cdiv(L->N, 64) + 63) / 64 * 64;
  per_wave = per_wave < 64 ? 64 : (per_wave > XSUM_PER_WAVE ? XSUM_PER_WAVE : per_wave);
  if (L->N > 0) { ProfScope _ps_graph_xsum_kernel(K_XSUM, st); hipLaunchKernelGGL(graph_xsum_kernel, dim3(cdiv(L->N, 4 * per_wave)), dim3(256), 0, st, L->x, L->batch, L->N, L->xsum, per_wave); }
  return check_launch("graph_xsum_kernel");
}

struct GraphPreArgs {
  const float *xsum, *Z, *HvT, *V0W, *V0B;
  float *Bc;
  int B, C, bf16;
};
constexpr int GP_SPLIT = 4;
__global__ __launch_bounds__(256) void graph_pre_fwd_kernel(GraphPreArgs a) {
  extern __shared__ float sm[];
  const int C = a.C, b = blockIdx.x, ld = 2 * H + 1 + C;
  float *mz = sm;
  float *mX = sm + 3 * C;
  const float cnt = fmaxf(a.xsum[b * 4 + 3], 1.f);
  for (int i = threadIdx.x; i < 3 * C; i += 256) {
    int k = i / C;
    mz[i] = a.Z[(size_t)b * 3 * C + i] - a.xsum[b * 4 + k] / cnt;
  }
  __syncthreads();
  for (int i = threadIdx.x; i < C * C; i += 256) {
    int c = i / C, d = i % C;
    mX[i] = mz[c] * mz[d] + mz[C + c] * mz[C + d] + mz[2 * C + c] * mz[2 * C + d];
  }
  __syncthreads();
  for (int i = blockIdx.y * 256 + threadIdx.x; i < C * H; i += 256 * gridDim.y) {
    int c = i >> 6, o = i & 63;
    const float *w = a.V0W + (size_t)o * ld;
    const float *hv = a.HvT + ((size_t)b * C + c) * H;
    float acc = a.V0B[o];
    if (a.bf16) { for (int k = 0; k < H; ++k) acc += round_bf(w[H + k]) * round_bf(hv[k]); }
    else { for (int k = 0; k < H; ++k) acc += w[H + k] * hv[k]; }
    for (int d = 0; d < C; ++d) acc += w[2 * H + 1 + d] * mX[d * C + c];
    a.Bc[((size_t)b * C + c) * H + o] = acc;
  }
}
int graph_pre_forward(const fastegnn_layer_t *L, hipStream_t st) {
  FE_REQUIRE(L->xsum && L->Z && L->HvT && L->Bc, "graph_pre_forward: null buffer");
  GraphPreArgs a{L->xsum, L->Z, L->HvT, L->params[FASTEGNN_P_VIRT0_W], L->params[FASTEGNN_P_VIRT0_B], L->Bc, L->B, L->C,
                 has(L, FASTEGNN_F_BF16) ? 1 : 0};
  const size_t lds = (size_t)(3 * L->C + L->C * L->C) * sizeof(float);
  { ProfScope _ps_graph_pre_fwd_kernel(K_GRAPH_PRE_FWD, st); hipLaunchKernelGGL(graph_pre_fwd_kernel, dim3(L->B, GP_SPLIT), dim3(256), lds, st, a); }
  return check_launch("graph_pre_fwd_kernel");
}

constexpr int EDGE_FWD_IMG_FLOATS = 2 * IMG3;
template <int MODE>
__global__ __launch_bounds__(64 * EDGE_FWD_WAVES) void edge_fwd_kernel(EdgeArgs a, int C) {
  extern __shared__ __attribute__((aligned(16))) float lds[];
#ifdef FE_ISA_CONST
  a.flags = FE_ISA_CONST; a.ea_dim = 2; a.bx2 = nullptr; a.attw = nullptr;
#endif
  float *img = lds;
  float *vec = lds + EDGE_FWD_IMG_FLOATS;
  float *tiles = vec + EV_COUNT * H;
  load_images_x3(reinterpret_cast<unsigned *>(img), wpack_x3(a.wpack, C, I_W2), 2);
  constexpr bool FOLD = edge_fold<false, MODE, false>();
  edge_load_vecs(vec, a, FOLD);
  __syncthreads();
  const int l = lane_id(), j = l & 15, q = l >> 4, wv = wave_id();
  float *mt = tiles + wv * (16 * TS + 64);
  float *xt = mt + 16 * TS;
  const int wave = global_wave_id(), nwaves = (gridDim.x * blockDim.x) >> 6;
  const bool mean = !(a.flags & FASTEGNN_F_COORDS_SUM);
  FE_T0()
  const int c0 = (int)((long)wave * a.n_chunks / nwaves), c1 = (int)((long)(wave + 1) * a.n_chunks / nwaves);
  {
    const int r0 = a.chunk_row[c0], r1 = a.chunk_row[c1];
    if (r0 < r1) {
      const int e0 = a.rowptr[r0], e1 = a.rowptr[r1];
      int cur = -1;
      float acc = 0.f, accx = 0.f;
      FE_T(7)
      int cnt = 0;
      auto flush = [&]() {
        const float inv = rcp_f((float)cnt);
        a.aggm[(size_t)cur * H + l] = acc * (FOLD ? inv * LN2_F : inv);
        if (l < 3) a.aggx[(size_t)cur * 3 + l] = mean ? accx * inv : accx;
      };
      auto zero_rows = [&](int ra, int rb) {
        for (int r = ra; r < rb; ++r) {
          a.aggm[(size_t)r * H + l] = 0.f;
          if (l < 3) a.aggx[(size_t)r * 3 + l] = 0.f;
        }
      };
      EdgeIdx cur_i, nxt_i;
      if (e0 < e1) edge_load_idx(a, min(e0 + j, e1 - 1), cur_i);
      for (int base = e0; base < e1; base += 16) {
        const int nvalid = min(16, e1 - base);
        nxt_i = cur_i;
        if (base + 16 < e1) edge_load_idx(a, min(base + 16 + j, e1 - 1), nxt_i);
        EdgeFwdState S;
        Vec pre;
        edge_tile_forward<false, MODE>(a, img, vec, cur_i, q, S, pre FE_TA);
        cur_i = nxt_i;
        tile_store(mt, j, q, S.m);
        if (q == 0) {
          xt[j * 4 + 0] = S.dn[0] * S.s;
          xt[j * 4 + 1] = S.dn[1] * S.s;
          xt[j * 4 + 2] = S.dn[2] * S.s;
        }
        __builtin_amdgcn_wave_barrier();
        FE_T(5)
        float mv[16], xv[16];
#pragma unroll
        for (int ee = 0; ee < 16; ++ee) {
          mv[ee] = mt[ee * TS + l];
          xv[ee] = xt[ee * 4 + (l & 3)];
        }
        const int rowv = S.row;
        const int prevrow = __builtin_amdgcn_update_dpp(rowv, rowv, 0x111, 0xf, 0xf, false);
        const unsigned long long chg = __builtin_amdgcn_ballot_w64(j == 0 ? rowv != cur : rowv != prevrow);
        const unsigned starts = (unsigned)chg & 0xffffu;
#pragma unroll
        for (int ee = 0; ee < 16; ++ee) {
          if (ee < nvalid) {
            if ((starts >> ee) & 1u) {
              const int rw = __builtin_amdgcn_readlane(rowv, ee);
              if (cur >= 0) flush();
              zero_rows(cur >= 0 ? cur + 1 : r0, rw);
              cur = rw;
              acc = 0.f;
              accx = 0.f;
              cnt = 0;
            }
            acc += mv[ee];
            accx += xv[ee];
            ++cnt;
          }
        }
        __builtin_amdgcn_wave_barrier();
        FE_T(6)
      }
      if (cur >= 0) flush();
      zero_rows(cur >= 0 ? cur + 1 : r0, r1);
    }
  }
  FE_TEND()
}

int edge_forward(const fastegnn_layer_t *L, hipStream_t st) {
  FE_REQUIRE(L->P && L->QX && L->aggm && L->aggx && L->wpack, "edge_forward: null buffer");
  FE_REQUIRE(L->ea <= 7, "edge_forward: edge_attr_nf > 7 unsupported");
  FE_REQUIRE(!has(L, FASTEGNN_F_ATTENTION) || (L->params[FASTEGNN_P_ATT_W] && L->params[FASTEGNN_P_ATT_B]),
             "edge_forward: attention params null");
  const fastegnn_graph_t &g = L->graph;
  if (g.n_edges == 0 || L->N == 0) {
    (void)hipMemsetAsync(L->aggm, 0, (size_t)L->N * H * sizeof(float), st);
    (void)hipMemsetAsync(L->aggx, 0, (size_t)L->N * 3 * sizeof(float), st);
    return check_launch("edge_forward(memset)");
  }
  FE_REQUIRE(g.rowptr && g.erow && g.col && g.chunk_row && (L->ea == 0 || L->ea_sorted), "edge_forward: null graph");
  EdgeArgs a = make_edge_args(L);
  FE_REQUIRE((size_t)L->N * QXLD < (1u << 30) && (size_t)g.n_src * QXLD < (1u << 30) && (size_t)g.n_edges * 8 < (1u << 30),
             "edge_forward: tables exceed the 32-bit offset range of the gather path");
  int grid = cdiv(g.n_chunks, EDGE_FWD_WAVES);
  if (grid > 256) grid = 256;
  const size_t lds = (EDGE_FWD_IMG_FLOATS + EV_COUNT * H + EDGE_FWD_WAVES * (16 * TS + 64)) * sizeof(float);
  {
    ProfScope _ps_edge_fwd_kernel(K_EDGE_FWD, st);
    if (has(L, FASTEGNN_F_BF16)) hipLaunchKernelGGL(edge_fwd_kernel<GM_BF16>, dim3(grid), dim3(64 * EDGE_FWD_WAVES), lds, st, a, L->C);
    else hipLaunchKernelGGL(edge_fwd_kernel<GM_EDGE_FWD>, dim3(grid), dim3(64 * EDGE_FWD_WAVES), lds, st, a, L->C);
  }
  return check_launch("edge_fwd_kernel");
}


}
#include "virt_fwd.h"
namespace fe {

int virt_forward(const fastegnn_layer_t *L, hipStream_t st) {
  const bool egnn = has(L, FASTEGNN_F_EGNN);
  const bool node = egnn || has(L, FASTEGNN_F_RF) || L->h_out;
  FE_REQUIRE(node || !L->HvT_out, "virt_forward: h_out is null and HvT_out is not (both null: no node update; otherwise neither)");
  FE_REQUIRE(L->h && L->A && L->x && L->vel && L->aggm && L->aggx && L->svel && (!node || (L->npre && L->h_out)) && L->x_out &&
                 L->batch && L->wpack,
             "virt_forward: null buffer");
  FE_REQUIRE(egnn ? L->C == 0 : (L->Bc && L->Z && (!node || L->poolV) && L->poolX && L->C >= 1 && L->C <= 64),
             "virt_forward: virtual_channels must be in [1,64] (0 with FASTEGNN_F_EGNN) and the virtual buffers non-null");
  FE_REQUIRE(L->na == 0 || L->node_attr, "virt_forward: node_attr null");
  if (L->C > 0) {
    if (node) (void)hipMemsetAsync(L->poolV, 0, (size_t)L->B * L->C * H * sizeof(float), st);
    (void)hipMemsetAsync(L->poolX, 0, (size_t)L->B * 3 * L->C * sizeof(float), st);
  }
  if (L->N == 0) return check_launch("virt_forward(memset)");
  VirtArgs a = make_virt_args(L);
  static const bool pair_off = getenv("FASTEGNN_VIRT_FWD_PAIR") && atoi(getenv("FASTEGNN_VIRT_FWD_PAIR")) == 0;
  const bool pair = GM_VIRT_FWD == GM_F16 && !pair_off && !has(L, FASTEGNN_F_BF16) && !has(L, FASTEGNN_F_RF) && !egnn && L->C >= 2 &&
                    cdiv(L->N, 16 * (VIRT_WAVES / 2)) <= 256 && virt_fwd_lds_bytes(L->C, true) <= 160 * 1024;
  const int ntg = cdiv(L->N, 16 * (pair ? VIRT_WAVES / 2 : VIRT_WAVES));
  int grid = ntg < 256 ? ntg : 256;
  {
    ProfScope _ps_virt_fwd_kernel(K_VIRT_FWD, st);
    const size_t lds = virt_fwd_lds_bytes(L->C, pair);
    if (!node) {
      if (has(L, FASTEGNN_F_BF16)) hipLaunchKernelGGL((virt_fwd_kernel<GM_BF16, false, false>), dim3(grid), dim3(64 * VIRT_WAVES), lds, st, a);
      else if (pair) launch_virt_fwd_pair_nonode(a, grid, lds, st);
      else hipLaunchKernelGGL((virt_fwd_kernel<GM_VIRT_FWD, false, false>), dim3(grid), dim3(64 * VIRT_WAVES), lds, st, a);
    }
    else if (has(L, FASTEGNN_F_BF16)) hipLaunchKernelGGL(virt_fwd_kernel<GM_BF16>, dim3(grid), dim3(64 * VIRT_WAVES), lds, st, a);
    else if (pair) launch_virt_fwd_pair(a, grid, lds, st);
    else hipLaunchKernelGGL(virt_fwd_kernel<GM_VIRT_FWD>, dim3(grid), dim3(64 * VIRT_WAVES), lds, st, a);
  }
  return check_launch("virt_fwd_kernel");
}

struct GraphPostArgs {
  const float *xsum, *Z, *HvT, *poolV, *poolX, *wpack, *b5, *b6;
  float *Z_out, *HvT_out;
  int B, C, flags;
  float act_param = 0.f;
};
__global__ __launch_bounds__(256) void graph_post_fwd_kernel(GraphPostArgs a) {
  const bool bf = a.flags & FASTEGNN_F_BF16;
  const int l = lane_id(), j = l & 15, q = l >> 4;
  const int wave = global_wave_id(), nwaves = (gridDim.x * blockDim.x) >> 6;
  const int M = a.B * a.C, ntiles = (M + 15) >> 4;
  for (int i = blockIdx.x * blockDim.x + threadIdx.x; i < a.B * 3 * a.C; i += gridDim.x * blockDim.x) {
    const int b = i / (3 * a.C);
    a.Z_out[i] = a.Z[i] + a.poolX[i] / fmaxf(a.xsum[b * 4 + 3], 1.f);
  }
  if (a.flags & FASTEGNN_F_RF) {
    for (int i = blockIdx.x * blockDim.x + threadIdx.x; i < M * H; i += gridDim.x * blockDim.x) a.HvT_out[i] = a.HvT[i];
    return;
  }
  for (int tile = wave; tile < ntiles; tile += nwaves) {
    const int m = tile * 16 + j;
    const bool valid = m < M;
    const int mc = valid ? m : M - 1;
    const int b = mc / a.C;
    const float inv = 1.0f / fmaxf(a.xsum[b * 4 + 3], 1.f);
    const Vec hv = vload_row(a.HvT + (size_t)mc * H, q);
    const Vec pm = vscale(vload_row(a.poolV + (size_t)mc * H, q), inv);
    Vec z5 = vload_vec(a.b5, q);
    gemm64(a.wpack + (size_t)I_W5A * IMG, bf ? vround(hv) : hv, z5);
    gemm64(a.wpack + (size_t)I_W5B * IMG, bf ? vround(pm) : pm, z5);
    Vec out = vload_vec(a.b6, q);
    const Vec u5 = vsilu(z5 FE_ACT(a));
    gemm64(a.wpack + (size_t)I_W6 * IMG, bf ? vround(u5) : u5, out);
    if (a.flags & FASTEGNN_F_RESIDUAL) vadd(out, hv);
    if (valid) vstore_row(a.HvT_out + (size_t)m * H, q, out);
  }
}
__global__ __launch_bounds__(256) void graph_post_fwd_coords_kernel(const float *xsum, const float *Z, const float *poolX, float *Z_out,
                                                                    int B, int C) {
  for (int i = blockIdx.x * blockDim.x + threadIdx.x; i < B * 3 * C; i += gridDim.x * blockDim.x) {
    const int b = i / (3 * C);
    Z_out[i] = Z[i] + poolX[i] / fmaxf(xsum[b * 4 + 3], 1.f);
  }
}
int graph_post_forward(const fastegnn_layer_t *L, hipStream_t st) {
  if (!L->HvT_out && !has(L, FASTEGNN_F_RF)) {
    FE_REQUIRE(!L->h_out, "graph_post_forward: HvT_out is null and h_out is not (both null: no node update; otherwise neither)");
    FE_REQUIRE(L->xsum && L->Z && L->poolX && L->Z_out, "graph_post_forward: null buffer");
    int grid = cdiv((long)L->B * 3 * L->C, 256);
    if (grid > 256) grid = 256;
    if (grid < 1) grid = 1;
    { ProfScope _ps_graph_post_fwd_kernel(K_GRAPH_POST_FWD, st); hipLaunchKernelGGL(graph_post_fwd_coords_kernel, dim3(grid), dim3(256), 0, st, L->xsum, L->Z, L->poolX, L->Z_out, L->B, L->C); }
    return check_launch("graph_post_fwd_coords_kernel");
  }
  FE_REQUIRE(L->xsum && L->Z && L->HvT && L->poolV && L->poolX && L->Z_out && L->HvT_out && L->wpack,
             "graph_post_forward: null buffer");
  GraphPostArgs a{L->xsum, L->Z, L->HvT, L->poolV, L->poolX, L->wpack, L->params[FASTEGNN_P_NODEV0_B],
                  L->params[FASTEGNN_P_NODEV2_B], L->Z_out, L->HvT_out, L->B, L->C, L->flags, L->act_param};
  int grid = cdiv(cdiv((long)L->B * L->C, 16), 4);
  if (grid > 256) grid = 256;
  if (grid < 1) grid = 1;
  { ProfScope _ps_graph_post_fwd_kernel(K_GRAPH_POST_FWD, st); hipLaunchKernelGGL(graph_post_fwd_kernel, dim3(grid), dim3(256), 0, st, a); }
  return check_launch("graph_post_fwd_kernel");
}

}

#ifdef FE_STAMP_VF
extern "C" int fastegnn_debug_read_stamps_vf(unsigned long long *out, int reset) {
  if (hipMemcpyFromSymbol(out, HIP_SYMBOL(fe::g_vf_stamps), sizeof(unsigned long long) * 16) != hipSuccess) return -1;
  if (reset) {
    unsigned long long z[16] = {0};
    (void)hipMemcpyToSymbol(HIP_SYMBOL(fe::g_vf_stamps), z, sizeof(z));
  }
  return 0;
}
#endif
#ifdef FE_STAMP
extern "C" int fastegnn_debug_read_stamps(unsigned long long *out, int reset) {
  if (hipMemcpyFromSymbol(out, HIP_SYMBOL(fe::g_stamps), sizeof(unsigned long long) * 16) != hipSuccess) return -1;
  if (reset) {
    unsigned long long z[16] = {0};
    (void)hipMemcpyToSymbol(HIP_SYMBOL(fe::g_stamps), z, sizeof(z));
  }
  return 0;
}
#endif
```

### fastegnn_amd/csrc/misc.hip

```cpp
#include <cstdlib>
#include "kernels.h"

namespace fe {

__global__ void embed_fwd_kernel(const float *nf, int N, int nfd, const float *W, const float *b, float *h) {
  long idx = (long)blockIdx.x * blockDim.x + threadIdx.x;
  if (idx >= (long)N * H) return;
  int n = (int)(idx >> 6), o = (int)(idx & 63);
  float acc = b[o];
  for (int a = 0; a < nfd; ++a) acc += nf[(size_t)n * nfd + a] * W[o * nfd + a];
  h[idx] = acc;
}
__global__ void dgrad_small_kernel(const float *G, long N, int kf, const float *W, int ldw, int c0, float *g_in, int accumulate) {
  long idx = (long)blockIdx.x * blockDim.x + threadIdx.x;
  if (idx >= N * kf) return;
  long n = idx / kf;
  int a = (int)(idx % kf);
  float acc = 0.f;
  for (int o = 0; o < H; ++o) acc += G[(size_t)n * H + o] * W[(size_t)o * ldw + c0 + a];
  g_in[idx] = accumulate ? g_in[idx] + acc : acc;
}

__global__ void virtual_init_kernel(const float *vnf, int B, int C, float *HvT) {
  long idx = (long)blockIdx.x * blockDim.x + threadIdx.x;
// ... 129 lines not shown
  };
  long m = m_first;
  if (m < m1) {
    load_g(m);
#pragma unroll
    for (int t = 0; t < 4; ++t) load_t(m, t);
  }
  for (; m < m1; m += step) {
    const bool full = m + 32 <= m1;
    const bool more = m + step < m1;
    WgParts gp[4];
#pragma unroll
    for (int t = 0; t < 4; ++t) {
      if (!full) {
#pragma unroll
        for (int e = 0; e < 8; ++e)
          if (m + 8 * q + e >= m1) gr[t][e] = 0.f;
      }
      if (want_bias) {
#pragma unroll
        for (int e = 0; e < 8; ++e) bsum[t] += gr[t][e];
      }
      gp[t] = wg_split8<BF>(gr[t]);
    }
    if (more) load_g(m + step);
#pragma unroll
    for (int tk = 0; tk < 4; ++tk) {
      if (!full) {
#pragma unroll
        for (int e = 0; e < 8; ++e)
          if (m + 8 * q + e >= m1) tr[tk][e] = 0.f;
      }
      const WgParts tp = wg_split8<BF>(tr[tk]);
      if (more) load_t(m + step, tk);
      const bf16x8 bh = __builtin_bit_cast(bf16x8, tp.p[0]), bm = __builtin_bit_cast(bf16x8, tp.p[1]),
                   bl = __builtin_bit_cast(bf16x8, tp.p[2]);
#pragma unroll
      for (int ti = 0; ti < 4; ++ti) {
        const bf16x8 ah = __builtin_bit_cast(bf16x8, gp[ti].p[0]);
        if constexpr (BF) {
          acc[ti][tk] = __builtin_amdgcn_mfma_f32_16x16x32_bf16(ah, bh, acc[ti][tk], 0, 0, 0);
        } else {
          const bf16x8 am = __builtin_bit_cast(bf16x8, gp[ti].p[1]), al = __builtin_bit_cast(bf16x8, gp[ti].p[2]);
          acc[ti][tk] = __builtin_amdgcn_mfma_f32_16x16x32_bf16(al, bh, acc[ti][tk], 0, 0, 0);
          acc[ti][tk] = __builtin_amdgcn_mfma_f32_16x16x32_bf16(am, bm, acc[ti][tk], 0, 0, 0);
          acc[ti][tk] = __builtin_amdgcn_mfma_f32_16x16x32_bf16(ah, bl, acc[ti][tk], 0, 0, 0);
          acc[ti][tk] = __builtin_amdgcn_mfma_f32_16x16x32_bf16(am, bh, acc[ti][tk], 0, 0, 0);
          acc[ti][tk] = __builtin_amdgcn_mfma_f32_16x16x32_bf16(ah, bm, acc[ti][tk], 0, 0, 0);
          acc[ti][tk] = __builtin_amdgcn_mfma_f32_16x16x32_bf16(ah, bh, acc[ti][tk], 0, 0, 0);
        }
      }
    }
  }
}

__global__ __launch_bounds__(256, FE_WG_OCC) void wgrad_tn_kernel(WgTable tab) {
  __shared__ __attribute__((aligned(16))) float smem[4 * IMG];
  __shared__ float redb[H];
  int jb = 0;
#pragma unroll 1
  while (jb + 1 < tab.n_jobs && (int)blockIdx.x >= tab.job[jb + 1].wg_begin) ++jb;
  const WgJob &a = tab.job[jb];
  const int local = blockIdx.x - a.wg_begin;
  const int bidx = local % a.nb, split = local / a.nb;
  const int l = lane_id(), i = l & 15, q = l >> 4, w = wave_id();
  const float *G = a.G + (size_t)bidx * a.sG;
  const float *T = a.T + (size_t)bidx * a.sT;
  const long m0 = (long)split * a.rows_per_wg;
  long m1 = m0 + a.rows_per_wg;
  if (m1 > a.M) m1 = a.M;
  if (threadIdx.x < H) redb[threadIdx.x] = 0.f;
  f32x4 acc[4][4];
  float bsum[4] = {0.f, 0.f, 0.f, 0.f};
#pragma unroll
  for (int ti = 0; ti < 4; ++ti)
#pragma unroll
    for (int tk = 0; tk < 4; ++tk) acc[ti][tk] = f32x4{0.f, 0.f, 0.f, 0.f};
  const bool want_bias = a.db != nullptr;
  if (a.round) wg_accumulate_x3<true>(G, T, a.ldg, a.ldt, m0 + 32 * w, m1, 128, want_bias, acc, bsum);
  else wg_accumulate_x3<false>(G, T, a.ldg, a.ldt, m0 + 32 * w, m1, 128, want_bias, acc, bsum);
  f32x4 *part = reinterpret_cast<f32x4 *>(smem) + (size_t)w * (IMG / 4);
#pragma unroll
  for (int ti = 0; ti < 4; ++ti)
#pragma unroll
    for (int tk = 0; tk < 4; ++tk) part[(ti * 4 + tk) * 64 + l] = acc[ti][tk];
#pragma unroll
  for (int ti = 0; ti < 4; ++ti) {
    float s = qsum(bsum[ti]);
    if (q == 0) atomicAdd(&redb[16 * ti + i], s);
  }
  __syncthreads();
  const size_t sidx = (size_t)a.slab_begin + (size_t)bidx * a.nsplit + split;
  float *dst = tab.slab + sidx * IMG;
  const f32x4 *p0 = reinterpret_cast<const f32x4 *>(smem);
#pragma unroll
  for (int u = 0; u < 4; ++u) {
    const int k = w * 4 + u, ti = k >> 2, tk = k & 3;
    const f32x4 v = ((p0[k * 64 + l] + p0[IMG / 4 + k * 64 + l]) + p0[2 * (IMG / 4) + k * 64 + l]) + p0[3 * (IMG / 4) + k * 64 + l];
#pragma unroll
    for (int r = 0; r < 4; ++r) dst[(16 * ti + 4 * q + r) * H + 16 * tk + i] = v[r];
  }
  if (threadIdx.x < H) tab.slab_b[sidx * H + threadIdx.x] = redb[threadIdx.x];
}

__global__ __launch_bounds__(512) void wgrad_reduce_kernel(WgTable tab) {
  __shared__ double part[8][H];
  const WgJob &a = tab.job[blockIdx.x];
  const int bidx = blockIdx.y;
  const bool merged = a.nb > 1 && a.sW == 0;
  if (bidx >= (merged ? 1 : a.nb)) return;
  const int n_part = merged ? a.nsplit * a.nb : a.nsplit;
  const size_t s0 = (size_t)a.slab_begin + (size_t)bidx * a.nsplit;
  float *dW = a.dW + (size_t)bidx * a.sW;
  const int e = threadIdx.x & 63, pl = threadIdx.x >> 6;
  const bool bias_block = blockIdx.z == IMG / H;
  const bool ext = a.T == nullptr && a.G != nullptr;
  const float *slabs = ext ? a.G : tab.slab;
  const size_t sx = ext ? (size_t)bidx * a.nsplit : s0;
  const size_t eoff = (size_t)blockIdx.z * H + e;
  int o_ = blockIdx.z, k_ = e;
  if (ext && !bias_block) {
    const int idx = (int)eoff, ln = (idx >> 2) & 63;
    o_ = 32 * (idx >> 11) + 8 * ((idx >> 8) & 3) + 4 * (ln >> 5) + (idx & 3);
    k_ = 32 * ((idx >> 10) & 1) + (ln & 31);
  }
  const float *base = bias_block ? tab.slab_b + s0 * H + e : slabs + sx * IMG + eoff;
  const size_t stride = bias_block ? H : IMG;
  if (bias_block && !a.db) return;
  double s[8] = {0., 0., 0., 0., 0., 0., 0., 0.};
  int p = pl;
  for (; p + 56 < n_part; p += 64) {
    float v[8];
#pragma unroll
    for (int u = 0; u < 8; ++u) v[u] = base[(size_t)(p + 8 * u) * stride];
#pragma unroll
    for (int u = 0; u < 8; ++u) s[u] += (double)v[u];
  }
  for (; p < n_part; p += 8) s[0] += (double)base[(size_t)p * stride];
  part[pl][e] = ((s[0] + s[1]) + (s[2] + s[3])) + ((s[4] + s[5]) + (s[6] + s[7]));
  __syncthreads();
  if (pl == 0) {
    double t = 0.;
#pragma unroll
    for (int u = 0; u < 8; ++u) t += part[u][e];
    if (bias_block) {
      atomicAdd(&a.db[e], (float)t);
    } else {
      const int o = o_, k = k_;
      if (k < a.kmax) atomicAdd(dW + (size_t)o * a.lddw + a.c0 + (size_t)k * a.ks, (float)t);
    }
  }
}

WgradBatch::WgradBatch(float *slab, hipStream_t st_, bool round_bf16, int slab_base_, int slab_cap_)
    : st(st_), round(round_bf16), slab_base(slab_base_), slab_cap(slab_cap_) {
  tab.n_jobs = 0;
  min_rows = 256;
  static const int cap_default = getenv("FE_WG_CAP") ? atoi(getenv("FE_WG_CAP")) : 512;
  max_split = cap_default;
  tab.slab = slab;
  tab.slab_b = slab ? slab + (size_t)WG_SLABS * IMG : nullptr;
  n_wg = 0;
  n_slab = slab_base;
  slab_top = slab_base + slab_cap;
  planned = false;
  max_nb = 1;
}

int WgradBatch::add(const float *G, int ldg, const float *T, int ldt, long M, float *dW, int lddw, int c0, int ks,
                    float *db, int nb, long sG, long sT, long sW, int kmax) {
  if (M <= 0 || !dW) return FASTEGNN_OK;
  FE_REQUIRE(G && T, "wgrad: null operand");
  FE_REQUIRE(tab.slab, "wgrad: wg_slab workspace is null");
  FE_REQUIRE(tab.n_jobs < WG_MAX_JOBS, "wgrad: too many jobs in one batch");
  FE_REQUIRE((ldg % 4) == 0 && (ldt % 4) == 0, "wgrad: operand rows must be 16-byte aligned");
  FE_REQUIRE(!planned, "wgrad: add() after the batch has been planned");
  long nsplit = (M + 1023) / 1024;
  static const long fill = getenv("FE_WG_FILL") ? atol(getenv("FE_WG_FILL")) : 128;
  if (nsplit < fill) nsplit = (M + min_rows - 1) / min_rows;
  if (nsplit > fill && M < fill * 1024) nsplit = fill;
  long cap = max_split / nb;
  if (cap < 4) cap = 4;
  if (nsplit > cap) nsplit = cap;
  WgJob &j = tab.job[tab.n_jobs++];
  j.G = G; j.T = T; j.dW = dW; j.db = db; j.M = M; j.sG = sG; j.sT = sT; j.sW = sW;
  j.ldg = ldg; j.ldt = ldt; j.lddw = lddw; j.c0 = c0; j.ks = ks; j.kmax = kmax;
  j.nsplit = (int)nsplit; j.nb = nb; j.rows_per_wg = 0;
  j.wg_begin = -1; j.slab_begin = -1;
  j.round = round ? 1 : 0;
  if (nb > max_nb) max_nb = nb;
  return FASTEGNN_OK;
}

int WgradBatch::plan() {
  if (planned) return FASTEGNN_OK;
  long want = 0;
  for (int k = 0; k < tab.n_jobs; ++k)
    if (tab.job[k].T) want += (long)tab.job[k].nsplit * tab.job[k].nb;
  const long avail = (long)slab_top - slab_base;
  long need_min = 0;
  for (int k = 0; k < tab.n_jobs; ++k)
    if (tab.job[k].T) need_min += tab.job[k].nb;
  FE_REQUIRE(need_min <= avail, "wgrad: slab workspace exhausted");
  n_wg = 0;
  n_slab = slab_base;
  for (int k = 0; k < tab.n_jobs; ++k) {
    WgJob &j = tab.job[k];
    if (!j.T) { j.wg_begin = n_wg; continue; }
    long nsplit = j.nsplit;
    if (want > avail) {
      nsplit = nsplit * (avail - need_min) / want;
      if (nsplit < 1) nsplit = 1;
    }
    long rows = (j.M + nsplit - 1) / nsplit;
    rows = (rows + 63) / 64 * 64;
    nsplit = (j.M + rows - 1) / rows;
    j.rows_per_wg = (int)rows;
    j.nsplit = (int)nsplit;
    j.wg_begin = n_wg;
    j.slab_begin = n_slab;
    n_wg += (int)(nsplit * j.nb);
    n_slab += (int)(nsplit * j.nb);
  }
  FE_REQUIRE(n_slab <= slab_top, "wgrad: slab workspace exhausted");
  planned = true;
  return FASTEGNN_OK;
}

int WgradBatch::guard_write(const float *p, size_t n, const char *what) const {
  if (!p || n == 0) return FASTEGNN_OK;
  const char *w0 = reinterpret_cast<const char *>(p), *w1 = w0 + n * sizeof(float);
  for (int k = 0; k < tab.n_jobs; ++k) {
    const WgJob &j = tab.job[k];
    if (!j.G || j.M <= 0) continue;
    const size_t span_g = (size_t)(j.nb - 1) * (size_t)(j.sG > 0 ? j.sG : 0) + (size_t)(j.M - 1) * j.ldg + H;
    const size_t span_t = (size_t)(j.nb - 1) * (size_t)(j.sT > 0 ? j.sT : 0) + (size_t)(j.M - 1) * j.ldt + H;
    const char *g0 = reinterpret_cast<const char *>(j.G), *t0 = reinterpret_cast<const char *>(j.T);
    const bool hit = (w0 < g0 + span_g * sizeof(float) && g0 < w1) || (w0 < t0 + span_t * sizeof(float) && t0 < w1);
    if (hit) {
      set_error(std::string("wgrad: a stage is about to overwrite ") + what + " while queued weight-gradient job " +
                std::to_string(k) + " still has to read it (the contractions run at finish())");
      return FASTEGNN_E_INVALID;
    }
  }
  return FASTEGNN_OK;
}

int WgradBatch::add_slabs(float *dW, int lddw, int c0, int ks, float *db, int nsplit, int *slab_begin) {
  FE_REQUIRE(dW && slab_begin && nsplit > 0, "wgrad: add_slabs arguments");
  FE_REQUIRE(tab.slab, "wgrad: wg_slab workspace is null");
  FE_REQUIRE(tab.n_jobs < WG_MAX_JOBS, "wgrad: too many jobs in one batch");
  FE_REQUIRE(!planned, "wgrad: add_slabs() after the batch has been planned");
  FE_REQUIRE(slab_top - nsplit >= slab_base, "wgrad: slab workspace exhausted");
  slab_top -= nsplit;
  WgJob &j = tab.job[tab.n_jobs++];
  j.G = nullptr; j.T = nullptr; j.dW = dW; j.db = db; j.M = 0; j.sG = j.sT = j.sW = 0;
  j.ldg = j.ldt = H; j.lddw = lddw; j.c0 = c0; j.ks = ks; j.kmax = 64;
  j.rows_per_wg = 0; j.nsplit = nsplit; j.nb = 1;
  j.round = 0;
  j.wg_begin = -1; j.slab_begin = slab_top;
  *slab_begin = slab_top;
  return FASTEGNN_OK;
}

int WgradBatch::add_slabs_ext(const float *ext, float *dW, int lddw, int c0, int ks, int nsplit, int nb, long sW) {
  FE_REQUIRE(ext && dW && nsplit > 0 && nb > 0 && sW != 0, "wgrad: add_slabs_ext arguments");
  FE_REQUIRE(tab.n_jobs < WG_MAX_JOBS, "wgrad: too many jobs in one batch");
  FE_REQUIRE(!planned, "wgrad: add_slabs_ext() after the batch has been planned");
  WgJob &j = tab.job[tab.n_jobs++];
  j.G = ext; j.T = nullptr; j.dW = dW; j.db = nullptr; j.M = 0; j.sG = j.sT = 0; j.sW = sW;
  j.ldg = j.ldt = H; j.lddw = lddw; j.c0 = c0; j.ks = ks; j.kmax = 64;
  j.rows_per_wg = 0; j.nsplit = nsplit; j.nb = nb;
  j.round = 0;
  j.wg_begin = -1; j.slab_begin = 0;
  if (nb > max_nb) max_nb = nb;
  return FASTEGNN_OK;
}

int WgradBatch::finish() {
  if (tab.n_jobs == 0) return FASTEGNN_OK;
  int rc = plan();
  if (rc) return rc;
  if (n_wg > 0) {
    { ProfScope _ps(K_WGRAD_TN, st); hipLaunchKernelGGL(wgrad_tn_kernel, dim3((unsigned)n_wg), dim3(256), 0, st, tab); }
    rc = check_launch("wgrad_tn_kernel");
    if (rc) return rc;
  }
  { ProfScope _ps(K_WGRAD_REDUCE, st); hipLaunchKernelGGL(wgrad_reduce_kernel, dim3((unsigned)tab.n_jobs, (unsigned)max_nb, IMG / H + 1), dim3(512), 0, st, tab); }
  tab.n_jobs = 0;
  n_wg = 0;
  n_slab = slab_base;
  slab_top = slab_base + slab_cap;
  planned = false;
  max_nb = 1;
  return check_launch("wgrad_reduce_kernel");
}

struct WgsArgs {
  const float *G, *F;
  float *dW, *db;
  long M;
  int ldg, ldf, kf, lddw, c0, rows_per_wg;
};
__global__ __launch_bounds__(256) void wgrad_small_kernel(WgsArgs a) {
  const int o = threadIdx.x & 63, w = wave_id();
  const long m0 = (long)blockIdx.x * a.rows_per_wg;
  long m1 = m0 + a.rows_per_wg;
  if (m1 > a.M) m1 = a.M;
  double acc[8] = {0, 0, 0, 0, 0, 0, 0, 0};
  double bs = 0.;
  long m = m0 + w;
  for (; m + 12 < m1; m += 16) {
    float g[4];
#pragma unroll
    for (int u = 0; u < 4; ++u) g[u] = a.G[(size_t)(m + 4 * u) * a.ldg + o];
#pragma unroll
    for (int u = 0; u < 4; ++u) {
      bs += (double)g[u];
#pragma unroll
      for (int k = 0; k < 8; ++k)
        if (k < a.kf) acc[k] += (double)g[u] * (double)a.F[(size_t)(m + 4 * u) * a.ldf + k];
    }
  }
  for (; m < m1; m += 4) {
    const float g = a.G[(size_t)m * a.ldg + o];
    bs += (double)g;
#pragma unroll
    for (int k = 0; k < 8; ++k)
      if (k < a.kf) acc[k] += (double)g * (double)a.F[(size_t)m * a.ldf + k];
  }
  __shared__ double red[4][9][H];
#pragma unroll
  for (int k = 0; k < 8; ++k) red[w][k][o] = acc[k];
  red[w][8][o] = bs;
  __syncthreads();
  if (w == 0) {
    for (int k = 0; k < a.kf; ++k)
      atomicAdd(&a.dW[(size_t)o * a.lddw + a.c0 + k], (float)((red[0][k][o] + red[1][k][o]) + (red[2][k][o] + red[3][k][o])));
    if (a.db) atomicAdd(&a.db[o], (float)((red[0][8][o] + red[1][8][o]) + (red[2][8][o] + red[3][8][o])));
  }
}
static int launch_wgrad_small_b(const float *G, int ldg, const float *F, int ldf, int kf, long M, float *dW, int lddw,
                                int c0, float *db, hipStream_t st) {
  if (M <= 0 || !dW) return FASTEGNN_OK;
  FE_REQUIRE(kf >= 0 && kf <= 8, "wgrad_small: kf > 8 unsupported");
  WgsArgs a{G, F, dW, db, M, ldg, ldf, kf, lddw, c0, 0};
  long nsplit = (M + 255) / 256;
  if (nsplit > 256) nsplit = 256;
  long rows = (M + nsplit - 1) / nsplit;
  a.rows_per_wg = (int)rows;
  nsplit = (M + rows - 1) / rows;
  { ProfScope _ps_wgrad_small_kernel(K_WGRAD_SMALL, st); hipLaunchKernelGGL(wgrad_small_kernel, dim3((unsigned)nsplit), dim3(256), 0, st, a); }
  return check_launch("wgrad_small_kernel");
}
int launch_dgrad_small(const float *G, long N, int kf, const float *W, int ldw, int c0, float *g_in, int accumulate,
                       hipStream_t st) {
  if (N == 0 || kf == 0) return FASTEGNN_OK;
  hipLaunchKernelGGL(dgrad_small_kernel, dim3(cdiv(N * kf, 256)), dim3(256), 0, st, G, N, kf, W, ldw, c0, g_in, accumulate);
  return check_launch("dgrad_small_kernel");
}

int launch_wgrad_small(const float *G, int ldg, const float *F, int ldf, int kf, long M, float *dW, int lddw, int c0,
                       hipStream_t st) {
  return launch_wgrad_small_b(G, ldg, F, ldf, kf, M, dW, lddw, c0, nullptr, st);
}

__global__ __launch_bounds__(256) void stream_kernel(const f32x4 *src, f32x4 *dst, size_t n, int mode) {
  const size_t stride = (size_t)gridDim.x * blockDim.x;
  size_t k = (size_t)blockIdx.x * blockDim.x + threadIdx.x;
  f32x4 acc = {0.f, 0.f, 0.f, 0.f};
  if (mode == 0) {
    for (; k + 3 * stride < n; k += 4 * stride) {
      const f32x4 a = src[k], b = src[k + stride], c = src[k + 2 * stride], d = src[k + 3 * stride];
      acc += (a + b) + (c + d);
    }
    for (; k < n; k += stride) acc += src[k];
    if (acc[0] + acc[1] + acc[2] + acc[3] == 12345.678f) dst[0] = acc;
  } else if (mode == 1) {
    for (; k < n; k += stride) dst[k] = src[k];
  } else {
    for (; k < n; k += stride) dst[k] = acc;
  }
}

__global__ __launch_bounds__(64) void selftest_gemm_kernel(const float *W, const float *X, float *Y, int transposed) {
  __shared__ __attribute__((aligned(16))) float img[IMG];
  for (int idx = threadIdx.x; idx < IMG; idx += 64) {
    int o = idx >> 6, k = idx & 63;
    img[img_index(o, k)] = transposed ? W[k * H + o] : W[o * H + k];
  }
  __syncthreads();
  const int l = lane_id(), j = l & 15, q = l >> 4;
  Vec in = vload_row(X + j * H, q);
  Vec acc = vzero();
  gemm64(img, in, acc);
  vstore_row(Y + j * H, q, acc);
}

__global__ __launch_bounds__(64) void selftest_rm_kernel(const float *W, const float *X, float *Y, int transposed, int mode) {
  __shared__ __attribute__((aligned(16))) unsigned rm[RM_WORDS];
  for (int idx = threadIdx.x; idx < 64 * (RM_RS / 4); idx += 64) {
    const int o = idx / (RM_RS / 4), w = idx % (RM_RS / 4);
    float w0 = w < 32 ? W[o * H + 2 * w] : 0.f, w1 = w < 32 ? W[o * H + 2 * w + 1] : 0.f;
    if (mode == 1) { w0 = round_bf(w0); w1 = round_bf(w1); }
    for (int p = 0; p < 3; ++p) rm[p * (RM_PART / 4) + idx] = split_word(w0, w1, p);
  }
  __syncthreads();
  const int l = lane_id(), j = l & 15, q = l >> 4;
  const Vec in = vload_row(X + j * H, q);
  Vec acc = vzero();
  const char *img = reinterpret_cast<const char *>(rm);
  if (mode == 0) {
    if (transposed) gemm_rm<GM_X3, true>(img, vsplit(in), acc);
    else gemm_rm<GM_X3, false>(img, vsplit(in), acc);
  } else {
    if (transposed) gemm_rm<GM_BF16, true>(img, vpack_bf(in), acc);
    else gemm_rm<GM_BF16, false>(img, vpack_bf(in), acc);
  }
  vstore_row(Y + j * H, q, acc);
}

__global__ __launch_bounds__(64) void selftest_lane_sums_kernel(const float *X, float *out) {
  const float x = X[threadIdx.x];
  out[threadIdx.x] = qsum(x);
  out[64 + threadIdx.x] = jsum(x);
}
__global__ __launch_bounds__(64) void selftest_jreduce_kernel(const float *X, float *out) {
  const int l = lane_id(), j = l & 15, q = l >> 4;
  const Vec v = vload_row(X + j * H, q);
  out[l] = jreduce16(v);
}

template <int WAVES>
__global__ __launch_bounds__(64 * WAVES) void chain_bf3_kernel(const float *W, const float *X, float *out, int iters,
                                                               int mode) {
  extern __shared__ __attribute__((aligned(16))) unsigned lds3[];
  for (int idx = threadIdx.x; idx < 3 * 2048; idx += blockDim.x) lds3[idx] = 0u;
  __syncthreads();
  for (int idx = threadIdx.x; idx < IMG; idx += blockDim.x) {
    const int o = idx >> 6, k = idx & 63;
    float w = W[idx], dummy = 0.f;
    const int tile = k >> 4, r = k & 3, e = ((tile & 1) << 2) | r;
    for (int p = 0; p < 3; ++p) {
      const unsigned hb = part_pack(w, dummy) & 0xffffu;
      atomicOr(&lds3[img3_index(p, o, k)], (e & 1) ? (hb << 16) : hb);
    }
  }
  __syncthreads();
  if (mode & 8) {
    for (int idx = threadIdx.x; idx < 3 * 2048; idx += blockDim.x) lds3[idx] = 0u;
    __syncthreads();
    for (int idx = threadIdx.x; idx < IMG / 2; idx += blockDim.x) {
      const int o = idx >> 5, k = (idx & 31) * 2;
      lds3[img3_index(0, o, k)] = split2_word(W[o * H + k], W[o * H + k + 1], 0);
      lds3[img3_index(1, o, k)] = split2_word(W[o * H + k], W[o * H + k + 1], 1);
    }
    __syncthreads();
  }
  const int l = lane_id(), j = l & 15, q = l >> 4;
  Vec x = vload_row(X + j * H, q);
  for (int it = 0; it < iters; ++it) {
    Vec acc = vzero();
    if (mode & 8) gemm64_f2(lds3, vsplit2(x), acc);
    else gemm64_x3(lds3, vsplit(x), acc);
    x = (mode & 1) ? vsilu(acc) : vscale(acc, 0.125f);
    if (mode & 4) x = acc;
  }
  if (blockIdx.x == 0 && threadIdx.x < 64) vstore_row(out + j * H, q, x);
}

template <int WAVES>
__global__ __launch_bounds__(64 * WAVES) void chain_kernel(const float *wimg, float *out, int iters, int mode) {
  extern __shared__ __attribute__((aligned(16))) float lds[];
  load_images(lds, wimg, 1);
  __syncthreads();
  const int l = lane_id(), q = l >> 4;
  const float *img = (mode & 2) ? wimg : lds;
  Vec x;
#pragma unroll
  for (int t = 0; t < 4; ++t) x.t[t] = f32x4{0.01f * l, 0.02f, -0.01f * t, 0.03f};
  for (int it = 0; it < iters; ++it) {
    Vec acc = vzero();
    gemm64(img, x, acc);
    x = (mode & 1) ? vsilu(acc) : vscale(acc, 0.125f);
  }
  if (out) vstore_row(out + ((size_t)blockIdx.x * blockDim.x + threadIdx.x) / 64 * 64 * 0, q, x);
}

}

using namespace fe;

extern "C" {

int fastegnn_embed_forward(const float *node_feat, int32_t N, int32_t nf, const float *W, const float *b, float *h,
                           void *stream) {
  FE_REQUIRE(node_feat && W && b && h, "embed_forward: null pointer");
  if (N == 0) return FASTEGNN_OK;
  hipLaunchKernelGGL(embed_fwd_kernel, dim3(cdiv((long)N * H, 256)), dim3(256), 0, (hipStream_t)stream, node_feat, N, nf,
                     W, b, h);
  return check_launch("embed_fwd_kernel");
}

int fastegnn_embed_backward(const float *node_feat, const float *g_h, int32_t N, int32_t nf, const float *W, float *gW,
                            float *gb, float *g_node_feat, void *stream) {
  FE_REQUIRE(node_feat && g_h && W, "embed_backward: null pointer");
  FE_REQUIRE(nf <= 8, "embed_backward: node_feat_nf > 8 unsupported");
  if (N == 0) return FASTEGNN_OK;
  hipStream_t st = (hipStream_t)stream;
  int rc = launch_wgrad_small_b(g_h, H, node_feat, nf, nf, N, gW, nf, 0, gb, st);
  if (rc) return rc;
  if (g_node_feat) {
    return launch_dgrad_small(g_h, N, nf, W, nf, 0, g_node_feat, 0, st);
  }
  return FASTEGNN_OK;
}

int fastegnn_virtual_init(const float *vnf, int32_t B, int32_t C, float *HvT, void *stream) {
  FE_REQUIRE(vnf && HvT, "virtual_init: null pointer");
  hipLaunchKernelGGL(virtual_init_kernel, dim3(cdiv((long)B * C * H, 256)), dim3(256), 0, (hipStream_t)stream, vnf, B, C,
                     HvT);
  return check_launch("virtual_init_kernel");
}

int fastegnn_virtual_init_backward(const float *g_HvT, int32_t B, int32_t C, float *g_vnf, void *stream) {
  FE_REQUIRE(g_HvT && g_vnf, "virtual_init_backward: null pointer");
  hipLaunchKernelGGL(virtual_init_bwd_kernel, dim3(cdiv((long)C * H, 256)), dim3(256), 0, (hipStream_t)stream, g_HvT, B,
                     C, g_vnf);
  return check_launch("virtual_init_bwd_kernel");
}

int fastegnn_pad_params(const fastegnn_pad_desc_t *desc, int32_t n, int32_t h, int32_t reverse, void *stream) {
  FE_REQUIRE(n == 0 || desc, "pad_params: null descriptors");
  FE_REQUIRE(h >= 1 && h <= fe::H, "pad_params: hidden_nf must be in [1,64]");
  for (int k0 = 0; k0 < n; k0 += fe::PAD_MAX_DESC) {
    fe::PadTable tab;
    tab.n = n - k0 < fe::PAD_MAX_DESC ? n - k0 : fe::PAD_MAX_DESC;
    tab.h = h;
    long most = 0;
    for (int k = 0; k < tab.n; ++k) {
      const fastegnn_pad_desc_t &d = desc[k0 + k];
      FE_REQUIRE(d.src && d.dst && d.rows >= 0 && d.cols >= 0 && d.rows_dst >= d.rows && d.nblk >= 0 && d.nblk <= 3 && d.lead >= 0,
                 "pad_params: bad descriptor");
      int cs = d.lead, cd = d.lead;
      for (int b = 0; b < d.nblk; ++b) {
        FE_REQUIRE(d.blk[b] >= 0 && d.blk[b] % h == 0, "pad_params: a block must be a multiple of hidden_nf columns");
        cs += d.blk[b];
        cd += d.blk[b] / h * fe::H;
      }
      FE_REQUIRE(cs <= d.cols && d.cols_dst == cd + (d.cols - cs), "pad_params: column blocks do not add up");
      tab.d[k] = d;
      const long elems = reverse ? (long)d.rows * d.cols : (long)d.rows_dst * d.cols_dst;
      if (elems > most) most = elems;
    }
    if (most == 0) continue;
    hipLaunchKernelGGL(fe::pad_params_kernel, dim3((unsigned)cdiv(most, 256), (unsigned)tab.n), dim3(256), 0, (hipStream_t)stream,
                       tab, reverse);
  }
  return check_launch("pad_params_kernel");
}

int fastegnn_permute_rows(const float *in, const int32_t *perm, int32_t E, int32_t width, float *out, void *stream) {
  if (E == 0 || width == 0) return FASTEGNN_OK;
  FE_REQUIRE(in && perm && out, "permute_rows: null pointer");
  hipLaunchKernelGGL(permute_rows_kernel, dim3(cdiv((long)E * width, 256)), dim3(256), 0, (hipStream_t)stream, in, perm, E,
                     width, out);
  return check_launch("permute_rows_kernel");
}

int fastegnn_build_batch(const int64_t *batch64, int32_t N, int32_t B, int32_t *batch, int32_t *gptr, void *stream) {
  FE_REQUIRE(batch64 && batch && gptr, "build_batch: null pointer");
  int n = N > B + 1 ? N : B + 1;
  hipLaunchKernelGGL(build_batch_kernel, dim3(cdiv(n, 256)), dim3(256), 0, (hipStream_t)stream, batch64, N, B, batch, gptr);
  return check_launch("build_batch_kernel");
}

int fastegnn_selftest_gemm(const float *W, const float *X, float *Y, int32_t transposed, void *stream) {
  FE_REQUIRE(W && X && Y, "selftest_gemm: null pointer");
  hipLaunchKernelGGL(selftest_gemm_kernel, dim3(1), dim3(64), 0, (hipStream_t)stream, W, X, Y, transposed);
  return check_launch("selftest_gemm_kernel");
}

int fastegnn_selftest_lane_sums(const float *X, float *out, void *stream) {
  FE_REQUIRE(X && out, "selftest_lane_sums: null pointer");
  hipLaunchKernelGGL(selftest_lane_sums_kernel, dim3(1), dim3(64), 0, (hipStream_t)stream, X, out);
  return check_launch("selftest_lane_sums_kernel");
}

int fastegnn_selftest_jreduce(const float *X, float *out, void *stream) {
  FE_REQUIRE(X && out, "selftest_jreduce: null pointer");
  hipLaunchKernelGGL(selftest_jreduce_kernel, dim3(1), dim3(64), 0, (hipStream_t)stream, X, out);
  return check_launch("selftest_jreduce_kernel");
}

int fastegnn_selftest_rm(const float *W, const float *X, float *Y, int32_t transposed, int32_t mode, void *stream) {
  FE_REQUIRE(W && X && Y, "selftest_rm: null pointer");
  hipLaunchKernelGGL(selftest_rm_kernel, dim3(1), dim3(64), 0, (hipStream_t)stream, W, X, Y, transposed, mode);
  return check_launch("selftest_rm_kernel");
}

int fastegnn_selftest_chain(const float *wimg, float *out, int32_t iters, int32_t mode, int32_t waves, int32_t grid,
                            void *stream) {
  FE_REQUIRE(wimg && out, "selftest_chain: null pointer");
  hipStream_t st = (hipStream_t)stream;
  const size_t lds = IMG * sizeof(float);
  if (waves == 4) hipLaunchKernelGGL(chain_kernel<4>, dim3(grid), dim3(256), lds, st, wimg, out, iters, mode);
  else if (waves == 8) hipLaunchKernelGGL(chain_kernel<8>, dim3(grid), dim3(512), lds, st, wimg, out, iters, mode);
  else if (waves == 16) hipLaunchKernelGGL(chain_kernel<16>, dim3(grid), dim3(1024), lds, st, wimg, out, iters, mode);
  else { set_error("selftest_chain: waves must be 4, 8 or 16"); return FASTEGNN_E_INVALID; }
  return check_launch("chain_kernel");
}

int fastegnn_selftest_chain_bf3(const float *W, const float *X, float *out, int32_t iters, int32_t mode, int32_t waves,
                                int32_t grid, void *stream) {
  FE_REQUIRE(W && X && out, "selftest_chain_bf3: null pointer");
  hipStream_t st = (hipStream_t)stream;
  const size_t lds = 3 * 2048 * sizeof(unsigned);
  if (waves == 4) hipLaunchKernelGGL(chain_bf3_kernel<4>, dim3(grid), dim3(256), lds, st, W, X, out, iters, mode);
  else if (waves == 8) hipLaunchKernelGGL(chain_bf3_kernel<8>, dim3(grid), dim3(512), lds, st, W, X, out, iters, mode);
  else if (waves == 16) hipLaunchKernelGGL(chain_bf3_kernel<16>, dim3(grid), dim3(1024), lds, st, W, X, out, iters, mode);
  else { set_error("selftest_chain_bf3: waves must be 4, 8 or 16"); return FASTEGNN_E_INVALID; }
  return check_launch("chain_bf3_kernel");
}

int fastegnn_selftest_stream(const float *src, float *dst, size_t n_floats, int32_t mode, void *stream) {
  FE_REQUIRE(src && dst && n_floats % 4 == 0, "selftest_stream: bad arguments");
  hipLaunchKernelGGL(stream_kernel, dim3(256 * 8), dim3(256), 0, (hipStream_t)stream, reinterpret_cast<const f32x4 *>(src),
                     reinterpret_cast<f32x4 *>(dst), n_floats / 4, mode);
  return check_launch("stream_kernel");
}

int fastegnn_selftest_wgrad_plan(const int64_t *M, const int32_t *nb, int32_t n_jobs, int32_t n_slab_jobs, int32_t slabs_each,
                                 int32_t max_split, int32_t slab_cap, int32_t *nsplit_out) {
  FE_REQUIRE(M && nb && nsplit_out && n_jobs >= 0, "selftest_wgrad_plan: bad arguments");
  static float dummy[4];
  WgradBatch wb(dummy, nullptr, false, 0, slab_cap);
  wb.max_split = max_split;
  for (int k = 0; k < n_jobs; ++k) {
    int rc = wb.add(dummy, H, dummy, H, (long)M[k], dummy, H, 0, 1, nullptr, nb[k], 0, 0, 0);
    if (rc) return rc;
  }
  for (int k = 0; k < n_slab_jobs; ++k) {
    int first = 0;
    int rc = wb.add_slabs(dummy, H, 0, 1, nullptr, slabs_each, &first);
    if (rc) return rc;
  }
  int rc = wb.plan();
  if (rc) return rc;
  for (int k = 0; k < n_jobs; ++k) nsplit_out[k] = wb.tab.job[k].nsplit;
  FE_REQUIRE(wb.n_slab <= wb.slab_top, "selftest_wgrad_plan: slab budget exceeded");
  return FASTEGNN_OK;
}

int fastegnn_selftest_wgrad_guard(int64_t M, int64_t probe_off, int64_t probe_n) {
  static float arena[4];
// ... 17 lines not shown
```

### fastegnn_amd/csrc/virt_bwd.hip

```cpp
#include <cstdlib>
#include "stages.h"

namespace fe {

#ifdef FE_SAFE_WAITS
__device__ __forceinline__ int vb_ld(const int *p) { return __hip_atomic_load(p, __ATOMIC_ACQUIRE, __HIP_MEMORY_SCOPE_WORKGROUP); }
__device__ __forceinline__ void vb_st(int *p, int v) { __hip_atomic_store(p, v, __ATOMIC_RELEASE, __HIP_MEMORY_SCOPE_WORKGROUP); }
#else
__device__ __forceinline__ int vb_ld(const int *p) { return __atomic_load_n(p, __ATOMIC_RELAXED); }
__device__ __forceinline__ void vb_st(int *p, int v) { __atomic_store_n(p, v, __ATOMIC_RELAXED); }
#endif

#ifdef FE_STAMP
__device__ unsigned long long g_vb2_stamps[32];
#define VB2_T0() unsigned _vp = (unsigned)__builtin_amdgcn_s_memtime(); unsigned _va[12] = {0, 0, 0, 0, 0, 0, 0, 0, 0, 0, 0, 0};
#define VB2_T(i) { __builtin_amdgcn_sched_barrier(0); const unsigned _t = (unsigned)__builtin_amdgcn_s_memtime(); \
                   _va[i] += _t - _vp; _vp = _t; __builtin_amdgcn_sched_barrier(0); }
#define VB2_TEND(base) if (lane_id() == 0) { for (int _k = 0; _k < 12; ++_k) atomicAdd(&g_vb2_stamps[(base) + _k], (unsigned long long)_va[_k]); }
#elif defined(FE_ISA_MARK)
#define VB2_T0()
#define VB2_T(i) { __builtin_amdgcn_sched_barrier(0); asm volatile("; FE_MARK " #i); __builtin_amdgcn_sched_barrier(0); }
#define VB2_TEND(base)
#else
#define VB2_T0()
// ... 1200 lines not shown
      VB2_T(6)
      Vec gnp = vzero();
      if constexpr (NODE) gnp = vb_mask(vload_u(A.g_np, offN), valid);
      {
        int tk = 0;
        if (l == 0) tk = atomicAdd(&ctrl[VBSC_HEAD + 0], 1);
        tk = __builtin_amdgcn_readfirstlane(tk);
        const int sl = tk % A.ringA, round = tk / A.ringA;
        VBS_SPIN(4, vb_ld(&ctrl[VBSC_DRAINED + 0 * VB_MAXRING + sl]) != round, 2);
        if constexpr (NODE) VBS_SPIN(5, vb_ld(&ctrl[VBSC_DRAINED + 1 * VB_MAXRING + sl]) != round, 2);
        __builtin_amdgcn_fence(__ATOMIC_ACQUIRE, "workgroup", "local");
        float *slot = ringA + sl * VBS_SLOT_A;
        vb_tile_store(slot, j, q, g_ux);
        vb_tile_store(slot + VB_TILE, j, q, g_uX);
        vb_tile_store(slot + 2 * VB_TILE, j, q, valid ? v : vzero());
        if constexpr (NODE) {
          vb_tile_store(slot + 3 * VB_TILE, j, q, gnp);
          if (l == 0) ctrl[VBSC_SLOTCH + sl] = c | (nb << 8) | (blk << 20);
        }
        __builtin_amdgcn_fence(__ATOMIC_RELEASE, "workgroup", "local");
        if (l == 0) vb_st(&ctrl[VBSC_FILLED + sl], round + 1);
        asm volatile("" ::: "memory");
      }
      VB2_T(7)
      Vec g_v = vzero();
      if constexpr (NODE) {
        g_v = vb_mask(vload_u(A.g_poolV, offB), valid);
        gemm64_f2_scaled(w3 + (ph & 1) * VBS_W3_WORDS, vsplit2_scaled(gnp), g_v);
      }
      mmT(1, g_ux, g_v);
      mmT(2, g_uX, g_v);
      VB2_T(8)
      float g_vd[3];
#pragma unroll
      for (int k = 0; k < 3; ++k) g_vd[k] = -sx * invC * gxn[k] + sX * gpX[k];
      Vec g_v0 = g_v;
      if constexpr (ATT) {
        const float g_a = vdot(g_v, v0);
        const float g_z = g_a * att * (1.f - att);
        vb_accum_items(racc + 3 * H, vscale(v0, g_z), j, q);
        const float sz = jsum(q == 0 ? g_z : 0.f);
        if (l == 0) atomicAdd(&racc[4 * H], sz);
        g_v0 = vscale(g_v, att);
        vaxpy(g_v0, g_z, vload_vec(vec + VV_ATT * H, q));
      }
      Vec g_t = vzero();
      Vec ga = vzero();
      {
        const Vec g_vp = vmul(g_v0, vp);
        {
          int tk = 0;
          if (l == 0) tk = atomicAdd(&ctrl[VBSC_HEAD + 1], 1);
          tk = __builtin_amdgcn_readfirstlane(tk);
          const int sl = tk % A.ringB, round = tk / A.ringB;
          VBS_SPIN(3, vb_ld(&ctrl[VBSC_DRAINED + 2 * VB_MAXRING + sl]) != round, 2);
          __builtin_amdgcn_fence(__ATOMIC_ACQUIRE, "workgroup", "local");
          float *slot = ringB + sl * VB_SLOT_B;
          vb_tile_store(slot, j, q, g_vp);
          vb_tile_store(slot + VB_TILE, j, q, t);
          __builtin_amdgcn_fence(__ATOMIC_RELEASE, "workgroup", "local");
          if (l == 0) vb_st(&ctrl[VBSC_FILLED + VB_MAXRING + sl], round + 1);
          asm volatile("" ::: "memory");
        }
        if (c > 0) ga = vload_u(A.g_A, offN);
        mmT(0, g_vp, g_t);
      }
      VB2_T(9)
      const Vec g_pre = vmul(g_t, d_pre);
      vadd(ga, g_pre);
      if (valid) vstore_u(A.g_A, offN, ga);
      vb_accum_items(racc + 2 * H, vscale(g_pre, vr), j, q);
      const float g_vr = vdot(g_pre, vload_vec(vec + VV_WVR * H, q));
      const float ivr = vr > 0.f ? g_vr * rcp_f(vr) : 0.f;
#pragma unroll
      for (int k = 0; k < 3; ++k) {
        g_vd[k] += ivr * vd[k];
        gx[k] -= g_vd[k];
      }
      if (valid && q == 0) {
#pragma unroll
        for (int k = 0; k < 3; ++k) A.g_x[(size_t)n * 3 + k] = gx[k];
      }
      if (pmode < 2) {
        float pz[3];
#pragma unroll
        for (int k = 0; k < 3; ++k) pz[k] = jsum((valid && q == 0) ? g_vd[k] : 0.f);
        vb_accum_items(pmode == 0 ? gBc_l + (ph & 1) * H : A.g_Bc + ((size_t)b0 * C + c) * H, g_pre, j, q);
        if (l < 3) {
          const float pzl = l == 0 ? pz[0] : (l == 1 ? pz[1] : pz[2]);
          if (pmode == 0) atomicAdd(&gZ_l[(ph & 1) * 4 + l], pzl);
          else atomicAdd(&A.g_Zp[((size_t)b0 * 3 + l) * C + c], pzl);
        }
      } else {
        if (valid && q == 0) {
#pragma unroll
          for (int k = 0; k < 3; ++k) atomicAdd(&A.g_Zp[((size_t)b * 3 + k) * C + c], g_vd[k]);
        }
        if (valid) {
#pragma unroll
          for (int t2 = 0; t2 < 4; ++t2)
#pragma unroll
            for (int r = 0; r < 4; ++r)
              atomicAdd(&A.g_Bc[((size_t)b * C + c) * H + 16 * t2 + 4 * q + r], g_pre.t[t2][r]);
        }
      }
      pend_tile = tile - t_lo;
      pend_c = c;
      __builtin_amdgcn_fence(__ATOMIC_RELEASE, "workgroup", "local");
      int dn = 0;
      if (l == 0) dn = atomicAdd(&ctrl[VBSC_DONE + ph % VBS_NPH], 1);
      dn = __builtin_amdgcn_readfirstlane(dn);
      if (dn == nb - 1) {
        __builtin_amdgcn_fence(__ATOMIC_ACQUIRE, "workgroup", "local");
        const float pb = gBc_l[(ph & 1) * H + l];
        atomicAdd(&A.g_Bc[((size_t)cur * C + c) * H + l], pb);
        gBc_l[(ph & 1) * H + l] = 0.f;
        if (l < 3) {
          atomicAdd(&A.g_Zp[((size_t)cur * 3 + l) * C + c], gZ_l[(ph & 1) * 4 + l]);
          gZ_l[(ph & 1) * 4 + l] = 0.f;
        }
        if (l == 0) ctrl[VBSC_DONE + ph % VBS_NPH] = 0;
        if (ph + 2 < nphase) {
          if constexpr (NODE) stage_w3(ph + 2);
          asm volatile("" ::: "memory");
          if (l == 0) __hip_atomic_store(&ctrl[VBSC_READY + (ph + 2) % VBS_NPH], ph + 3, __ATOMIC_RELEASE, __HIP_MEMORY_SCOPE_WORKGROUP);
          asm volatile("" ::: "memory");
        }
      }
      VB2_T(10)
    }
    VB2_TEND(0)
  }
  VB2_T0()
  __syncthreads();
  VB2_T(11)
  VB2_TEND(consumer ? 12 : 0)
  if (threadIdx.x < H) {
    const int o = threadIdx.x;
    float s5[5] = {0.f, 0.f, 0.f, 0.f, 0.f};
    for (int bk = 0; bk < A.nbank; ++bk) {
      const float *r = racc0 + bk * VB_RACC;
#pragma unroll
      for (int k = 0; k < 4; ++k) s5[k] += r[k * H + o];
      s5[4] += r[4 * H];
    }
    atomicAdd(&A.d_wxv2[o], s5[0]);
    atomicAdd(&A.d_wxx2[o], s5[1]);
    atomicAdd(&A.d_wvr[(size_t)o * A.ld_v0], s5[2]);
    if constexpr (ATT) {
      atomicAdd(&A.d_attw[o], s5[3]);
      if (o == 0) atomicAdd(A.d_attb, s5[4]);
    }
  }
}

static int virt_cs_grid(long N) {
  const long g = ((N + 15) / 16) / VBS_MIN_TILES;
  return (int)(g > 256 ? 256 : g);
}
static int virt_cs_min_grid() {
  static const int v = getenv("FASTEGNN_VIRT_CS_MIN_GRID") ? atoi(getenv("FASTEGNN_VIRT_CS_MIN_GRID")) : 256;
  return v < 1 ? 1 : v;
}
bool virt_cs_applies(long N, int C, int flags) {
  if (!(FE_VB_CS && GM_VIRT_BWD == GM_F16 && FE_VB_CONS32)) return false;
  static const bool off = getenv("FASTEGNN_VIRT_CS") && atoi(getenv("FASTEGNN_VIRT_CS")) == 0;
  if (off || (flags & (FASTEGNN_F_BF16 | FASTEGNN_F_RF | FASTEGNN_F_EGNN)) || C < 1 || C > VBS_MAXC) return false;
  const int grid = virt_cs_grid(N);
  if (grid < 1) return false;
  static const int max_tiles = getenv("FASTEGNN_VIRT_CS_MAX_TILES") ? atoi(getenv("FASTEGNN_VIRT_CS_MAX_TILES")) : 64;
  const long nt = ((N + 15) / 16 + grid - 1) / grid;
  return grid >= virt_cs_min_grid() && nt <= VBS_MAXTILES && nt <= max_tiles;
}
size_t virt_cs_wg_floats(size_t C) { return (size_t)256 * (5 + C) * IMG; }

size_t virt_pc_wg_floats(size_t N, size_t C) {
  const size_t NGF = (C + VB_GF - 1) / VB_GF;
  return (N + WGV_PAD) * C * H + (size_t)256 * VB_FINE_TILES * (NGF - 1) * 16 * (H + 4) + (size_t)256 * 3 * IMG;
}

static int virt_backward_channels_cs(const fastegnn_layer_t *L, hipStream_t st, float *wg_gnp, bool node) {
  const int C = L->C;
  const bool att = has(L, FASTEGNN_F_ATTENTION);
  float *const *g = L->grads;
  const int grid = virt_cs_grid(L->N);
  FE_REQUIRE(!node || L->g_poolV, "virt_backward: g_poolV null");
  WgradBatch bb(L->wg_slab, st, false, WG_SLABS / 2, WG_SLABS / 2);
  VirtCsArgs A;
  A.f = make_virt_args(L);
  A.g_x_out = L->g_x_out; A.g_poolX = L->g_poolX; A.g_poolV = L->g_poolV; A.g_np = wg_gnp;
  A.g_x = L->g_x; A.g_A = L->g_A; A.g_Bc = L->g_Bc; A.g_Zp = L->g_Zp;
  A.cons_scratch = L->wg_virt;
  A.w_slab = L->wg_virt + (size_t)grid * 5 * IMG;
  A.ld_v0 = 2 * H + 1 + C;
  A.d_wxv2 = g[FASTEGNN_P_CRV2_W]; A.d_wxx2 = g[FASTEGNN_P_CVV2_W];
  A.d_wvr = g[FASTEGNN_P_VIRT0_W] + 2 * H;
  A.d_attw = g[FASTEGNN_P_ATTV_W]; A.d_attb = g[FASTEGNN_P_ATTV_B];
  int rc;
  if ((rc = bb.add_slabs(g[FASTEGNN_P_CRV0_W], H, 0, 1, g[FASTEGNN_P_CRV0_B], grid, &A.slab_x))) return rc;
  if ((rc = bb.add_slabs(g[FASTEGNN_P_CVV0_W], H, 0, 1, g[FASTEGNN_P_CVV0_B], grid, &A.slab_X))) return rc;
  if ((rc = bb.add_slabs(g[FASTEGNN_P_VIRT2_W], H, 0, 1, g[FASTEGNN_P_VIRT2_B], grid, &A.slab_v2))) return rc;
  A.slab = bb.tab.slab; A.slab_b = bb.tab.slab_b;
  static const int ring_want = getenv("FE_VBS_RING") ? atoi(getenv("FE_VBS_RING")) : 32;
  static const int block_want = getenv("FASTEGNN_VIRT_CS_BLOCK") ? atoi(getenv("FASTEGNN_VIRT_CS_BLOCK")) : VBS_BLOCK;
  A.block = block_want < 1 ? 1 : (block_want > 0xfff ? 0xfff : block_want);
  A.ringA = ring_want / 10; A.ringB = ring_want % 10; A.nbank = 1;
  if (A.ringA < 2 || A.ringA > VB_MAXRING) A.ringA = 3;
  if (A.ringB < 2 || A.ringB > VB_MAXRING) A.ringB = 2;
  while (vbs_lds_floats(A.ringA, A.ringB, 1) * sizeof(float) > 160 * 1024 && A.ringB > 2) --A.ringB;
  while (vbs_lds_floats(A.ringA, A.ringB, 1) * sizeof(float) > 160 * 1024 && A.ringA > 2) --A.ringA;
  while (A.nbank < VB_MAXBANK && vbs_lds_floats(A.ringA, A.ringB, A.nbank + 1) * sizeof(float) <= 160 * 1024) ++A.nbank;
  const size_t lds = vbs_lds_floats(A.ringA, A.ringB, A.nbank) * sizeof(float);
  FE_REQUIRE(lds <= 160 * 1024, "virt_backward: LDS budget exceeded");
  {
    ProfScope ps(K_VIRT_BWD, st);
    const dim3 g3(grid), b3(64 * VB_WAVES);
    if (!node) {
      if (att) hipLaunchKernelGGL((virt_bwd_cs_kernel<true, false>), g3, b3, lds, st, A);
      else hipLaunchKernelGGL((virt_bwd_cs_kernel<false, false>), g3, b3, lds, st, A);
    }
    else if (att) hipLaunchKernelGGL((virt_bwd_cs_kernel<true>), g3, b3, lds, st, A);
    else hipLaunchKernelGGL((virt_bwd_cs_kernel<false>), g3, b3, lds, st, A);
  }
  if ((rc = check_launch("virt_bwd_cs_kernel"))) return rc;
  if (!node) return bb.finish();
  const int ld_n0 = 2 * H + H * C + L->na;
  if ((rc = bb.add_slabs_ext(A.w_slab, g[FASTEGNN_P_NODE0_W], ld_n0, 2 * H, C, grid, C, 1))) return rc;
  return bb.finish();
}

static int virt_backward_channels(const fastegnn_layer_t *L, hipStream_t st, float *wg_gnp, bool node) {
  if (virt_cs_applies(L->N, L->C, L->flags)) return virt_backward_channels_cs(L, st, wg_gnp, node);
  const int N = L->N, C = L->C, ntiles = cdiv(N, 16);
  const bool bf = has(L, FASTEGNN_F_BF16), att = has(L, FASTEGNN_F_ATTENTION), rf = has(L, FASTEGNN_F_RF);
  float *const *g = L->grads;
  const size_t cstride = ((size_t)N + WGV_PAD) * H;
  float *wg_v = L->wg_virt, *Gv = L->wg_virt;
  const int NGF = (C + VB_GF - 1) / VB_GF;
  float *gA_part = Gv + cstride * C, *gx_part = gA_part + (size_t)256 * VB_FINE_TILES * (NGF - 1) * 16 * H;
  int rc;
  if (rf) {
    (void)hipMemsetAsync(Gv, 0, cstride * C * sizeof(float), st);
  } else if (!node) {
    ProfScope ps(K_VIRT_BWD_GV, st);
    (void)hipMemsetAsync(Gv, 0, cstride * C * sizeof(float), st);
  } else {
    const int ngroups = cdiv(C, VB_GV_CH);
    int nranges = 256 / ngroups;
    const int max_ranges = cdiv(ntiles, VB_GV_WAVES);
    if (nranges > max_ranges) nranges = max_ranges;
    if (nranges < 1) nranges = 1;
    VirtGvArgs a{wg_gnp, L->g_poolV, L->wpack, L->batch, Gv, cstride, N, C, ngroups, nranges};
    const size_t lds = (size_t)VB_GV_CH * RM_BYTES;
    ProfScope ps(K_VIRT_BWD_GV, st);
    if (bf) hipLaunchKernelGGL((virt_bwd_gv_kernel<true>), dim3(ngroups * nranges), dim3(64 * VB_GV_WAVES), lds, st, a);
    else hipLaunchKernelGGL((virt_bwd_gv_kernel<false>), dim3(ngroups * nranges), dim3(64 * VB_GV_WAVES), lds, st, a);
  }
  if ((rc = check_launch("virt_bwd_gv_kernel"))) return rc;
  WgradBatch bb(L->wg_slab, st, bf, WG_SLABS / 2, WG_SLABS / 2);
  VirtBwd2Args A;
  A.f = make_virt_args(L);
  A.g_x_out = L->g_x_out; A.g_poolX = L->g_poolX; A.Gv = Gv;
  A.g_x = L->g_x; A.g_A = L->g_A; A.g_Bc = L->g_Bc; A.g_Zp = L->g_Zp;
  A.gA_part = gA_part; A.gx_part = gx_part; A.wg_v = wg_v; A.cstride = cstride;
  A.cons_scratch = gx_part + (size_t)256 * VB_FINE_TILES * (NGF - 1) * 16 * 4;
  A.ld_v0 = 2 * H + 1 + C;
  A.d_wxv2 = g[FASTEGNN_P_CRV2_W]; A.d_wxx2 = g[FASTEGNN_P_CVV2_W];
  A.d_wvr = g[FASTEGNN_P_VIRT0_W] + 2 * H;
  A.d_attw = g[FASTEGNN_P_ATTV_W]; A.d_attb = g[FASTEGNN_P_ATTV_B];
  A.NGF = NGF;
  int grid = ntiles < 256 ? ntiles : 256;
  if ((rc = bb.add_slabs(g[FASTEGNN_P_CRV0_W], H, 0, 1, g[FASTEGNN_P_CRV0_B], grid, &A.slab_x))) return rc;
  if ((rc = bb.add_slabs(g[FASTEGNN_P_CVV0_W], H, 0, 1, g[FASTEGNN_P_CVV0_B], grid, &A.slab_X))) return rc;
  if ((rc = bb.add_slabs(g[FASTEGNN_P_VIRT2_W], H, 0, 1, g[FASTEGNN_P_VIRT2_B], grid, &A.slab_v2))) return rc;
  A.slab = bb.tab.slab; A.slab_b = bb.tab.slab_b;
  static const int ring_want = getenv("FE_VB_RING") ? atoi(getenv("FE_VB_RING")) : 54;
  const int imgb = bf ? RM_BYTES : (GM_VIRT_BWD == GM_F16 ? rm_lds_bytes<GM_F16>() : RM_BYTES);
  A.ringA = ring_want / 10; A.ringB = ring_want % 10; A.nbank = 1;
  if (A.ringA < 2 || A.ringA > VB_MAXRING) A.ringA = 3;
  if (A.ringB < 2 || A.ringB > VB_MAXRING) A.ringB = 3;
  while (vb_lds_floats(C, A.ringA, A.ringB, 1, imgb) * sizeof(float) > 160 * 1024 && A.ringB > 2) --A.ringB;
  while (vb_lds_floats(C, A.ringA, A.ringB, 1, imgb) * sizeof(float) > 160 * 1024 && A.ringA > 2) --A.ringA;
  while (A.nbank < VB_MAXBANK && vb_lds_floats(C, A.ringA, A.ringB, A.nbank + 1, imgb) * sizeof(float) <= 160 * 1024) ++A.nbank;
  const size_t lds = vb_lds_floats(C, A.ringA, A.ringB, A.nbank, imgb) * sizeof(float);
  FE_REQUIRE(lds <= 160 * 1024, "virt_backward: LDS budget exceeded");
  {
    ProfScope ps(K_VIRT_BWD, st);
    const dim3 g3(grid), b3(64 * VB_WAVES);
    if (bf) { if (att) hipLaunchKernelGGL((virt_bwd_pc_kernel<true, true>), g3, b3, lds, st, A); else hipLaunchKernelGGL((virt_bwd_pc_kernel<true, false>), g3, b3, lds, st, A); }
    else { if (att) hipLaunchKernelGGL((virt_bwd_pc_kernel<false, true>), g3, b3, lds, st, A); else hipLaunchKernelGGL((virt_bwd_pc_kernel<false, false>), g3, b3, lds, st, A); }
  }
  if ((rc = check_launch("virt_bwd_pc_kernel"))) return rc;
  if (NGF > 1) {
    hipLaunchKernelGGL(virt_bwd_combine_kernel, dim3(grid * VB_FINE_TILES), dim3(256), 0, st, L->g_A, L->g_x, gA_part, gx_part, N, NGF - 1, grid);
    if ((rc = check_launch("virt_bwd_combine_kernel"))) return rc;
  }
  if (!rf && node) {
    const int ld_n0 = 2 * H + H * C + L->na;
    if ((rc = bb.add(wg_gnp, H, wg_v, H, N, g[FASTEGNN_P_NODE0_W], ld_n0, 2 * H, C, nullptr, C, 0, (long)cstride, 1))) return rc;
  }
  return bb.finish();
}

int virt_backward(const fastegnn_layer_t *L, hipStream_t st, WgradBatch *shared) {
  const bool egnn = has(L, FASTEGNN_F_EGNN), rf = has(L, FASTEGNN_F_RF);
  const bool node = egnn || rf || L->g_h_out;
  FE_REQUIRE(node || !L->g_HvT_out, "virt_backward: g_h_out is null and g_HvT_out is not (both null: no gradient for h / Hv; otherwise neither)");
  FE_REQUIRE(L->h && L->A && L->x && L->vel && L->aggm && (!node || L->npre) && L->batch && L->wpack && (!egnn || L->aggx),
             "virt_backward: null saved buffer");
  FE_REQUIRE((!node || L->g_h_out) && L->g_x_out && L->g_h && L->g_x && L->g_A && L->g_aggm && L->g_aggx && L->g_svel && L->wg_node &&
                 L->grads && L->wg_slab,
             "virt_backward: null gradient buffer");
  FE_REQUIRE(egnn ? L->C == 0
                  : (L->Bc && L->Z && (rf || !node || L->g_poolV) && L->g_poolX && L->g_Bc && L->g_Zp && L->wg_virt && L->C >= 1 && L->C <= 64),
             "virt_backward: virtual buffers null or virtual_channels outside [1,64] (0 with FASTEGNN_F_EGNN)");
  const int N = L->N, C = L->C;
  if (C > 0) {
    (void)hipMemsetAsync(L->g_Bc, 0, (size_t)L->B * C * H * sizeof(float), st);
    (void)hipMemsetAsync(L->g_Zp, 0, (size_t)L->B * 3 * C * sizeof(float), st);
  }
  if (N == 0) return check_launch("virt_backward(memset)");
  const bool bf = has(L, FASTEGNN_F_BF16);
  float *const *g = L->grads;
  FE_REQUIRE(!has(L, FASTEGNN_F_ATTENTION) || C == 0 || (g[FASTEGNN_P_ATTV_W] && g[FASTEGNN_P_ATTV_B]), "virt_backward: attention grads null");
  FE_REQUIRE(!has(L, FASTEGNN_F_GRAVITY) || L->g_sgrav, "virt_backward: g_sgrav null");
  float *wg_t3 = L->wg_node, *wg_gnp = L->wg_node + (size_t)N * H;
  const int ntiles = cdiv(N, 16);
  int rc;
  if (!node) {
    ProfScope ps(K_VIRT_BWD_NODE, st);
    hipLaunchKernelGGL(virt_bwd_node_skip_kernel, dim3(cdiv((long)N * (H / 4), 256)), dim3(256), 0, st, L->g_x_out, L->vel, L->g_h, L->g_aggm,
                       L->g_aggx, L->g_svel, L->g_sgrav, N, L->flags, L->gravity[0], L->gravity[1], L->gravity[2]);
  } else {
    VirtNodeArgs a{L->g_h_out, L->npre, L->g_x_out, L->vel, L->aggx, L->wpack, wg_t3, wg_gnp, L->g_h, L->g_aggm, L->g_aggx,
                   L->g_svel, L->g_sgrav, N, L->flags, C, {L->gravity[0], L->gravity[1], L->gravity[2]}, L->act_param};
    int grid = cdiv(ntiles, VB_NODE_WAVES);
    if (grid > 256) grid = 256;
    ProfScope ps(K_VIRT_BWD_NODE, st);
    if (bf) hipLaunchKernelGGL((virt_bwd_node_kernel<true>), dim3(grid), dim3(64 * VB_NODE_WAVES), 3 * IMG3 * sizeof(float), st, a);
    else hipLaunchKernelGGL((virt_bwd_node_kernel<false>), dim3(grid), dim3(64 * VB_NODE_WAVES), 3 * IMG3 * sizeof(float), st, a);
  }
  if ((rc = check_launch("virt_bwd_node_kernel"))) return rc;
  if (C == 0) {
    (void)hipMemcpyAsync(L->g_x, L->g_x_out, (size_t)N * 3 * sizeof(float), hipMemcpyDeviceToDevice, st);
    (void)hipMemsetAsync(L->g_A, 0, (size_t)N * H * sizeof(float), st);
    if ((rc = check_launch("virt_backward(C = 0)"))) return rc;
  } else if ((rc = virt_backward_channels(L, st, wg_gnp, node))) {
    return rc;
  }
  if (rf || !node) return FASTEGNN_OK;
  WgradBatch local(L->wg_slab, st);
  WgradBatch &wb = shared ? *shared : local;
  wb.round = bf;
  const int ld_n0 = 2 * H + H * C + L->na;
  if ((rc = wb.add(L->g_h_out, H, wg_t3, H, N, g[FASTEGNN_P_NODE2_W], H, 0, 1, g[FASTEGNN_P_NODE2_B]))) return rc;
  if ((rc = wb.add(wg_gnp, H, L->h, H, N, g[FASTEGNN_P_NODE0_W], ld_n0, 0, 1, g[FASTEGNN_P_NODE0_B]))) return rc;
  if ((rc = wb.add(wg_gnp, H, L->aggm, H, N, g[FASTEGNN_P_NODE0_W], ld_n0, H, 1, nullptr))) return rc;
  if (!shared && (rc = wb.finish())) return rc;
  if (L->na > 0) {
    if ((rc = launch_wgrad_small(wg_gnp, H, L->node_attr, L->na, L->na, N, g[FASTEGNN_P_NODE0_W], ld_n0, 2 * H + H * C, st))) return rc;
    if (L->g_node_attr)
      if ((rc = launch_dgrad_small(wg_gnp, N, L->na, L->params[FASTEGNN_P_NODE0_W], ld_n0, 2 * H + H * C, L->g_node_attr, 1, st))) return rc;
  }
  return FASTEGNN_OK;
}

}

#ifdef FE_STAMP
extern "C" int fastegnn_debug_read_vb2_stamps(unsigned long long *out, int reset) {
  if (hipMemcpyFromSymbol(out, HIP_SYMBOL(fe::g_vb2_stamps), sizeof(unsigned long long) * 32) != hipSuccess) return -1;
  if (reset) {
    unsigned long long z[32] = {0};
    (void)hipMemcpyToSymbol(HIP_SYMBOL(fe::g_vb2_stamps), z, sizeof(z));
  }
  return 0;
}
#endif

extern "C" int fastegnn_spin_timeouts(int reset) {
  int n = -1;
  if (hipMemcpyFromSymbol(&n, HIP_SYMBOL(fe::g_vbs_timeouts), sizeof(int)) != hipSuccess) return -1;
  if (reset) {
    const int z = 0;
    (void)hipMemcpyToSymbol(HIP_SYMBOL(fe::g_vbs_timeouts), &z, sizeof(int));
  }
  return n;
}
#ifdef FE_VBS_WATCHDOG
extern "C" int fastegnn_debug_read_vbs_dog(int *out, int reset) {
  if (hipMemcpyFromSymbol(out, HIP_SYMBOL(fe::g_vbs_dog), sizeof(int) * 64) != hipSuccess) return -1;
  if (reset) {
    int z[64] = {0};
    (void)hipMemcpyToSymbol(HIP_SYMBOL(fe::g_vbs_dog), z, sizeof(z));
  }
  return 0;
}
#endif
```

Baseline: 97.97 graphs/s.

## Fuse memsets and xsum partials, restructure graph-post GEMMs, vectorize small wgrad

Several separate changes are bundled. Zeroing of the virtual-gradient accumulators moves into the graph-post backward kernels, and the forward pool zeroing is folded into the xsum partial-sum path, which replaces the segmented per-batch atomic xsum with per-wave partials staged in aggm. The graph-post forward and backward kernels now keep weight fragments in registers, with each wave computing one 16-column block and exchanging activations through LDS. graph_pre_bwd stages weights and g_Bc in LDS, and wgrad_small is templated on kf with vectorized loads across 8 waves. Together these aim to cut launch count and redundant global traffic, at the cost of added barriers and more complex code.

```diff
diff --git a/fastegnn_amd/csrc/api.hip b/fastegnn_amd/csrc/api.hip
--- a/fastegnn_amd/csrc/api.hip
+++ b/fastegnn_amd/csrc/api.hip
@@ -221,10 +221,11 @@
     if ((rc = edge_forward(L, st))) return rc;
     return virt_forward(L, st);
   }
-  if ((rc = graph_xsum(L, st))) return rc;
-  if ((rc = graph_pre_forward(L, st))) return rc;
+  FE_REQUIRE(L->aggm, "fastegnn_layer_forward: aggm null");
+  if ((rc = graph_xsum_partials(L, L->aggm, st))) return rc;
+  if ((rc = graph_pre_forward(L, st, L->aggm))) return rc;
   if ((rc = edge_forward(L, st))) return rc;
-  if ((rc = virt_forward(L, st))) return rc;
+  if ((rc = virt_forward(L, st, true))) return rc;
   return graph_post_forward(L, st);
 }
 
@@ -248,9 +249,9 @@
     if ((rc = node_pre_backward(L, st, &wb))) return rc;
     return wb.finish();
   }
-  if ((rc = graph_post_backward(L, st, &wb))) return rc;
+  if ((rc = graph_post_backward(L, st, &wb, true))) return rc;
   if ((rc = guard_virt())) return rc;
-  if ((rc = virt_backward(L, st, &wb))) return rc;
+  if ((rc = virt_backward(L, st, &wb, true))) return rc;
   if ((rc = guard_stage(L, wb, G_GRAPH_PRE))) return rc;
   if ((rc = graph_pre_backward(L, st, &wb))) return rc;
   if ((rc = guard_edge())) return rc;
diff --git a/fastegnn_amd/csrc/common.h b/fastegnn_amd/csrc/common.h
--- a/fastegnn_amd/csrc/common.h
+++ b/fastegnn_amd/csrc/common.h
@@ -293,6 +293,26 @@
       for (int t = 0; t < 4; ++t)
         acc.t[t] = __builtin_amdgcn_mfma_f32_16x16x4f32(a[t][r], in.t[tp][r], acc.t[t], 0, 0, 0);
   }
+}
+
+__device__ __forceinline__ void gemm64_frags(const float *img, int t, f32x4 frag[4]) {
+  const f32x4 *ip = reinterpret_cast<const f32x4 *>(img) + lane_id();
+#pragma unroll
+  for (int tp = 0; tp < 4; ++tp) frag[tp] = ip[(t * 4 + tp) * 64];
+}
+__device__ __forceinline__ void gemm64_block(const f32x4 frag[4], const Vec &in, f32x4 &acc) {
+#pragma unroll
+  for (int tp = 0; tp < 4; ++tp)
+#pragma unroll
+    for (int r = 0; r < 4; ++r) acc = __builtin_amdgcn_mfma_f32_16x16x4f32(frag[tp][r], in.t[tp][r], acc, 0, 0, 0);
+}
+__device__ __forceinline__ f32x4 vload_block(const float *w, int t, int q) { return *reinterpret_cast<const f32x4 *>(w + 16 * t + 4 * q); }
+__device__ __forceinline__ void vstore_block(float *row, int t, int q, const f32x4 &v) { *reinterpret_cast<f32x4 *>(row + 16 * t + 4 * q) = v; }
+template <class F>
+__device__ __forceinline__ f32x4 vblock(const f32x4 &x, F f) {
+  Vec v;
+  v.t[0] = v.t[1] = v.t[2] = v.t[3] = x;
+  return f(v).t[0];
 }
 
 typedef unsigned u32x4 __attribute__((ext_vector_type(4)));
diff --git a/fastegnn_amd/csrc/kernels.h b/fastegnn_amd/csrc/kernels.h
--- a/fastegnn_amd/csrc/kernels.h
+++ b/fastegnn_amd/csrc/kernels.h
@@ -81,12 +81,13 @@
 int pack_weights_all(const fastegnn_layer_t *const *layers, int n, hipStream_t st);
 int node_pre_forward(const fastegnn_layer_t *L, hipStream_t st);
 int graph_xsum(const fastegnn_layer_t *L, hipStream_t st);
-int graph_pre_forward(const fastegnn_layer_t *L, hipStream_t st);
+int graph_xsum_partials(const fastegnn_layer_t *L, float *part, hipStream_t st);
+int graph_pre_forward(const fastegnn_layer_t *L, hipStream_t st, float *part = nullptr);
 int edge_forward(const fastegnn_layer_t *L, hipStream_t st);
-int virt_forward(const fastegnn_layer_t *L, hipStream_t st);
+int virt_forward(const fastegnn_layer_t *L, hipStream_t st, bool pools_zeroed = false);
 int graph_post_forward(const fastegnn_layer_t *L, hipStream_t st);
-int graph_post_backward(const fastegnn_layer_t *L, hipStream_t st, WgradBatch *shared = nullptr);
-int virt_backward(const fastegnn_layer_t *L, hipStream_t st, WgradBatch *shared = nullptr);
+int graph_post_backward(const fastegnn_layer_t *L, hipStream_t st, WgradBatch *shared = nullptr, bool zero_acc = false);
+int virt_backward(const fastegnn_layer_t *L, hipStream_t st, WgradBatch *shared = nullptr, bool acc_zeroed = false);
 int graph_pre_backward(const fastegnn_layer_t *L, hipStream_t st, WgradBatch *shared = nullptr);
 int edge_backward(const fastegnn_layer_t *L, hipStream_t st, WgradBatch *shared = nullptr);
 size_t virt_pc_wg_floats(size_t N, size_t C);
diff --git a/fastegnn_amd/csrc/layer_bwd.hip b/fastegnn_amd/csrc/layer_bwd.hip
--- a/fastegnn_amd/csrc/layer_bwd.hip
+++ b/fastegnn_amd/csrc/layer_bwd.hip
@@ -21,13 +21,20 @@
   float *g_Z, *g_HvT, *g_poolV, *g_poolX, *wg_u, *wg_gz5, *wg_pm;
   int B, C, flags;
   float act_param = 0.f;
+  float *z_Bc = nullptr, *z_Zp = nullptr;
 };
+__device__ __forceinline__ void zero_virt_acc(float *z_Bc, float *z_Zp, int B, int C) {
+  const int i0 = blockIdx.x * blockDim.x + threadIdx.x, step = gridDim.x * blockDim.x;
+  if (z_Bc) for (int i = i0; i < B * C * H; i += step) z_Bc[i] = 0.f;
+  if (z_Zp) for (int i = i0; i < B * 3 * C; i += step) z_Zp[i] = 0.f;
+}
 __global__ __launch_bounds__(256) void graph_post_bwd_kernel(GraphPostBwdArgs a) {
   const bool bf = a.flags & FASTEGNN_F_BF16;
   auto rb = [&](const Vec &v) { return bf ? vround(v) : v; };
-  const int l = lane_id(), j = l & 15, q = l >> 4;
-  const int wave = global_wave_id(), nwaves = (gridDim.x * blockDim.x) >> 6;
+  __shared__ __attribute__((aligned(16))) float xt[16 * TS];
+  const int l = lane_id(), j = l & 15, q = l >> 4, w = wave_id();
   const int M = a.B * a.C, ntiles = (M + 15) >> 4;
+  zero_virt_acc(a.z_Bc, a.z_Zp, a.B, a.C);
   for (int i = blockIdx.x * blockDim.x + threadIdx.x; i < a.B * 3 * a.C; i += gridDim.x * blockDim.x) {
     const int b = i / (3 * a.C);
     const float g = a.g_Z_out[i];
@@ -41,7 +48,14 @@
     }
     return;
   }
-  for (int tile = wave; tile < ntiles; tile += nwaves) {
+  f32x4 f5a[4], f5b[4], f6t[4], f5at[4], f5bt[4];
+  gemm64_frags(a.wpack + (size_t)I_W5A * IMG, w, f5a);
+  gemm64_frags(a.wpack + (size_t)I_W5B * IMG, w, f5b);
+  gemm64_frags(a.wpack + (size_t)I_W6T * IMG, w, f6t);
+  gemm64_frags(a.wpack + (size_t)I_W5AT * IMG, w, f5at);
+  gemm64_frags(a.wpack + (size_t)I_W5BT * IMG, w, f5bt);
+  const f32x4 zero4 = {0.f, 0.f, 0.f, 0.f};
+  for (int tile = blockIdx.x; tile < ntiles; tile += gridDim.x) {
     const int m = tile * 16 + j;
     const bool valid = m < M;
     const int mc = valid ? m : M - 1;
@@ -49,29 +63,37 @@
     const float inv = 1.0f / fmaxf(a.xsum[b * 4 + 3], 1.f);
     const Vec hv = vload_row(a.HvT + (size_t)mc * H, q);
     const Vec pm = vscale(vload_row(a.poolV + (size_t)mc * H, q), inv);
-    Vec z5 = vload_vec(a.b5, q);
-    gemm64(a.wpack + (size_t)I_W5A * IMG, rb(hv), z5);
-    gemm64(a.wpack + (size_t)I_W5B * IMG, rb(pm), z5);
     const Vec g_out = vload_row(a.g_HvT_out + (size_t)mc * H, q);
-    Vec g_u = vzero();
-    gemm64(a.wpack + (size_t)I_W6T * IMG, rb(g_out), g_u);
-    const Vec g_z5 = vdsilu_mul(g_u, z5 FE_ACT(a));
-    Vec g_hv = (a.flags & FASTEGNN_F_RESIDUAL) ? g_out : vzero();
-    gemm64(a.wpack + (size_t)I_W5AT * IMG, rb(g_z5), g_hv);
-    Vec g_pm = vzero();
-    gemm64(a.wpack + (size_t)I_W5BT * IMG, rb(g_z5), g_pm);
+    f32x4 z5 = vload_block(a.b5, w, q);
+    gemm64_block(f5a, rb(hv), z5);
+    gemm64_block(f5b, rb(pm), z5);
+    f32x4 g_u = zero4;
+    gemm64_block(f6t, rb(g_out), g_u);
+    Vec Z, G;
+    Z.t[0] = Z.t[1] = Z.t[2] = Z.t[3] = z5;
+    G.t[0] = G.t[1] = G.t[2] = G.t[3] = g_u;
+    const f32x4 g_z5w = vdsilu_mul(G, Z FE_ACT(a)).t[0];
+    vstore_block(xt + j * TS, w, q, g_z5w);
+    __syncthreads();
+    const Vec g_z5 = rb(vload_row(xt + j * TS, q));
+    f32x4 g_hv = (a.flags & FASTEGNN_F_RESIDUAL) ? vload_block(a.g_HvT_out + (size_t)mc * H, w, q) : zero4;
+    gemm64_block(f5at, g_z5, g_hv);
+    f32x4 g_pm = zero4;
+    gemm64_block(f5bt, g_z5, g_pm);
     if (valid) {
-      vstore_row(a.wg_u + (size_t)m * H, q, vsilu(z5 FE_ACT(a)));
-      vstore_row(a.wg_gz5 + (size_t)m * H, q, g_z5);
-      vstore_row(a.wg_pm + (size_t)m * H, q, pm);
-      vstore_row(a.g_HvT + (size_t)m * H, q, g_hv);
-      vstore_row(a.g_poolV + (size_t)m * H, q, vscale(g_pm, inv));
-    }
+      vstore_block(a.wg_u + (size_t)m * H, w, q, vblock(z5, [&](const Vec &v) { return vsilu(v FE_ACT(a)); }));
+      vstore_block(a.wg_gz5 + (size_t)m * H, w, q, g_z5w);
+      vstore_block(a.wg_pm + (size_t)m * H, w, q, vload_block(a.poolV + (size_t)mc * H, w, q) * inv);
+      vstore_block(a.g_HvT + (size_t)m * H, w, q, g_hv);
+      vstore_block(a.g_poolV + (size_t)m * H, w, q, g_pm * inv);
+    }
+    __syncthreads();
   }
 }
 
 __global__ __launch_bounds__(256) void graph_post_bwd_coords_kernel(const float *xsum, const float *g_Z_out, float *g_Z, float *g_poolX,
-                                                                    float *g_HvT, int B, int C) {
+                                                                    float *g_HvT, int B, int C, float *z_Bc, float *z_Zp) {
+  zero_virt_acc(z_Bc, z_Zp, B, C);
   for (int i = blockIdx.x * blockDim.x + threadIdx.x; i < B * 3 * C; i += gridDim.x * blockDim.x) {
     const int b = i / (3 * C);
     const float g = g_Z_out[i];
@@ -81,14 +103,16 @@
   for (int i = blockIdx.x * blockDim.x + threadIdx.x; i < B * C * H; i += gridDim.x * blockDim.x) g_HvT[i] = 0.f;
 }
 
-int graph_post_backward(const fastegnn_layer_t *L, hipStream_t st, WgradBatch *shared) {
+int graph_post_backward(const fastegnn_layer_t *L, hipStream_t st, WgradBatch *shared, bool zero_acc) {
+  FE_REQUIRE(!zero_acc || (L->g_Bc && L->g_Zp), "graph_post_backward: g_Bc / g_Zp null");
+  float *z_Bc = zero_acc ? L->g_Bc : nullptr, *z_Zp = zero_acc ? L->g_Zp : nullptr;
   if (!L->g_HvT_out && !has(L, FASTEGNN_F_RF)) {
     FE_REQUIRE(!L->g_h_out, "graph_post_backward: g_HvT_out is null and g_h_out is not (both null: no gradient for h / Hv; otherwise neither)");
     FE_REQUIRE(L->xsum && L->g_Z_out && L->g_Z && L->g_HvT && L->g_poolX, "graph_post_backward: null buffer");
     int grid = cdiv((long)L->B * L->C * H, 256);
     if (grid > 256) grid = 256;
     if (grid < 1) grid = 1;
-    { ProfScope _ps_graph_post_bwd_kernel(K_GRAPH_POST_BWD, st); hipLaunchKernelGGL(graph_post_bwd_coords_kernel, dim3(grid), dim3(256), 0, st, L->xsum, L->g_Z_out, L->g_Z, L->g_poolX, L->g_HvT, L->B, L->C); }
+    { ProfScope _ps_graph_post_bwd_kernel(K_GRAPH_POST_BWD, st); hipLaunchKernelGGL(graph_post_bwd_coords_kernel, dim3(grid), dim3(256), 0, st, L->xsum, L->g_Z_out, L->g_Z, L->g_poolX, L->g_HvT, L->B, L->C, z_Bc, z_Zp); }
     return check_launch("graph_post_bwd_coords_kernel");
   }
   FE_REQUIRE(L->xsum && L->HvT && L->poolV && L->g_Z_out && L->g_HvT_out && L->g_Z && L->g_HvT && L->g_poolV &&
@@ -98,8 +122,8 @@
   float *wg_gp = L->wg_node + 4 * wg_node_rows(L) * H;
   float *wg_u = wg_gp, *wg_gz5 = wg_gp + M * H, *wg_pm = wg_gp + 2 * M * H;
   GraphPostBwdArgs a{L->xsum, L->HvT, L->poolV, L->g_Z_out, L->g_HvT_out, L->wpack, L->params[FASTEGNN_P_NODEV0_B],
-                     L->g_Z, L->g_HvT, L->g_poolV, L->g_poolX, wg_u, wg_gz5, wg_pm, L->B, L->C, L->flags, L->act_param};
-  int grid = cdiv(cdiv(M, 16), 4);
+                     L->g_Z, L->g_HvT, L->g_poolV, L->g_poolX, wg_u, wg_gz5, wg_pm, L->B, L->C, L->flags, L->act_param, z_Bc, z_Zp};
+  int grid = cdiv(M, 16);
   if (grid > 256) grid = 256;
   if (grid < 1) grid = 1;
   { ProfScope _ps_graph_post_bwd_kernel(K_GRAPH_POST_BWD, st); hipLaunchKernelGGL(graph_post_bwd_kernel, dim3(grid), dim3(256), 0, st, a); }
@@ -123,6 +147,8 @@
   int B, C, bf16;
 };
 constexpr int GPB_SPLIT = 4;
+constexpr int GPB_GLD = H + 1;
+static size_t graph_pre_bwd_lds_floats(int C) { return (size_t)6 * C + C * C + (size_t)C * GPB_GLD + (size_t)H * (C + 1) + H * H; }
 __global__ __launch_bounds__(256) void graph_pre_bwd_kernel(GraphPreBwdArgs a) {
   extern __shared__ float sm[];
   const int C = a.C, b = blockIdx.x, ld = 2 * H + 1 + C;
@@ -130,6 +156,12 @@
   float *mz = sm;
   float *gmX = sm + 3 * C;
   float *gmz = gmX + C * C;
+  float *gbs = gmz + 3 * C;
+  float *wd = gbs + C * GPB_GLD;
+  float *wb = wd + H * (C + 1);
+  for (int i = threadIdx.x; i < H * H; i += 256) wb[i] = a.V0W[(size_t)(i >> 6) * ld + H + (i & 63)];
+  for (int i = threadIdx.x; i < C * H; i += 256) gbs[(i >> 6) * GPB_GLD + (i & 63)] = a.g_Bc[(size_t)b * C * H + i];
+  for (int i = threadIdx.x; i < H * C; i += 256) wd[(i / C) * (C + 1) + i % C] = a.V0W[(size_t)(i / C) * ld + 2 * H + 1 + i % C];
   const float cnt = fmaxf(a.xsum[b * 4 + 3], 1.f);
   for (int i = threadIdx.x; i < 3 * C; i += 256) mz[i] = a.Z[(size_t)b * 3 * C + i] - a.xsum[b * 4 + i / C] / cnt;
   __syncthreads();
@@ -141,17 +173,17 @@
   }
   for (int i = i0; i < C * H; i += istep) {
     int c = i >> 6, k = i & 63;
-    const float *gb = a.g_Bc + ((size_t)b * C + c) * H;
+    const float *gb = gbs + c * GPB_GLD;
     float acc = 0.f;
-    if (a.bf16) { for (int o = 0; o < H; ++o) acc += round_bf(gb[o]) * round_bf(a.V0W[(size_t)o * ld + H + k]); }
-    else { for (int o = 0; o < H; ++o) acc += gb[o] * a.V0W[(size_t)o * ld + H + k]; }
+    if (a.bf16) { for (int o = 0; o < H; ++o) acc += round_bf(gb[o]) * round_bf(wb[o * H + k]); }
+    else { for (int o = 0; o < H; ++o) acc += gb[o] * wb[o * H + k]; }
     a.g_HvT[((size_t)b * C + c) * H + k] += acc;
   }
   for (int i = threadIdx.x; i < C * C; i += 256) {
     int cp = i / C, c = i % C;
-    const float *gb = a.g_Bc + ((size_t)b * C + c) * H;
+    const float *gb = gbs + c * GPB_GLD;
     float acc = 0.f;
-    for (int o = 0; o < H; ++o) acc += gb[o] * a.V0W[(size_t)o * ld + 2 * H + 1 + cp];
+    for (int o = 0; o < H; ++o) acc += gb[o] * wd[o * (C + 1) + cp];
     gmX[cp * C + c] = acc;
   }
   __syncthreads();
@@ -176,7 +208,7 @@
   float *wg_mxt = L->wg_node + 7 * wg_node_rows(L) * H;
   GraphPreBwdArgs a{L->xsum, L->Z, L->g_Bc, L->g_Zp, L->params[FASTEGNN_P_VIRT0_W], L->g_Z, L->g_HvT, L->g_xbar, wg_mxt,
                     L->B, L->C, has(L, FASTEGNN_F_BF16) ? 1 : 0};
-  const size_t lds = (size_t)(6 * L->C + L->C * L->C) * sizeof(float);
+  const size_t lds = graph_pre_bwd_lds_floats(L->C) * sizeof(float);
   { ProfScope _ps_graph_pre_bwd_kernel(K_GRAPH_PRE_BWD, st); hipLaunchKernelGGL(graph_pre_bwd_kernel, dim3(L->B, GPB_SPLIT), dim3(256), lds, st, a); }
   int rc = check_launch("graph_pre_bwd_kernel");
   if (rc) return rc;
diff --git a/fastegnn_amd/csrc/layer_fwd.hip b/fastegnn_amd/csrc/layer_fwd.hip
--- a/fastegnn_amd/csrc/layer_fwd.hip
+++ b/fastegnn_amd/csrc/layer_fwd.hip
@@ -101,90 +101,138 @@
   return check_launch("node_pre_fwd_kernel");
 }
 
-#ifndef FE_XSUM_PER_WAVE
-#define FE_XSUM_PER_WAVE 1024
-#endif
-constexpr int XSUM_PER_WAVE = FE_XSUM_PER_WAVE;
-__global__ __launch_bounds__(256) void graph_xsum_kernel(const float *x, const int32_t *batch, int N, float *xsum, int PER_WAVE) {
-  const int l = lane_id();
-  const int n0 = global_wave_id() * PER_WAVE, n1 = min(N, n0 + PER_WAVE);
-  if (n0 >= n1) return;
-  int cur = -1;
-  float s[4] = {0.f, 0.f, 0.f, 0.f};
-  auto flush = [&]() {
-    float mine = 0.f;
-#pragma unroll
-    for (int k = 0; k < 4; ++k) {
-      float v = s[k];
-      for (int off = 32; off > 0; off >>= 1) v += __shfl_xor(v, off);
-      if (l == k) mine = v;
-      s[k] = 0.f;
+constexpr int XS_BLOCK = 256;
+constexpr int XS_MAXBLK = 4096;
+__device__ float g_xsum_part[XS_MAXBLK * 4];
+static int xsum_block_nodes(int N) {
+  const int k = cdiv(N, XS_BLOCK * XS_MAXBLK);
+  return XS_BLOCK * (k < 1 ? 1 : k);
+}
+
+__global__ __launch_bounds__(256) void graph_xsum_part_kernel(const float *x, int N, int NB, float *part) {
+  if (!part) part = g_xsum_part;
+  const int l = lane_id(), blk = global_wave_id();
+  if ((long)blk * NB >= N) return;
+  const int n0 = blk * NB, n1 = min(N, n0 + NB);
+  float s[3] = {0.f, 0.f, 0.f};
+#pragma unroll 4
+  for (int n = n0 + l; n < n1; n += 64) {
+#pragma unroll
+    for (int k = 0; k < 3; ++k) s[k] += x[(size_t)n * 3 + k];
+  }
+#pragma unroll
+  for (int k = 0; k < 3; ++k)
+    for (int off = 32; off > 0; off >>= 1) s[k] += __shfl_xor(s[k], off);
+  if (l == 0) *reinterpret_cast<f32x4 *>(part + (size_t)blk * 4) = f32x4{s[0], s[1], s[2], 0.f};
+}
+
+__device__ __forceinline__ int xsum_lower_bound(const int32_t *batch, int N, int key) {
+  int a = 0, e = N;
+  while (a < e) {
+    const int S = (e - a + 255) / 256, idx = a + (int)threadIdx.x * S;
+    const int c = __syncthreads_count(idx < e && batch[idx] < key);
+    if (c == 0) e = a;
+    else {
+      e = min(e, a + c * S);
+      a += (c - 1) * S + 1;
     }
-    if (l < 4) atomicAdd(&xsum[cur * 4 + l], mine);
-  };
-  for (int base = n0; base < n1; base += 64) {
-    const int n = base + l;
-    const bool ok = n < n1;
-    const int b = batch[ok ? n : n1 - 1];
-    const int bf = __builtin_amdgcn_readfirstlane(b), bl = batch[min(base + 63, n1 - 1)];
-    float xv[3] = {0.f, 0.f, 0.f};
-    if (ok) { xv[0] = x[(size_t)n * 3]; xv[1] = x[(size_t)n * 3 + 1]; xv[2] = x[(size_t)n * 3 + 2]; }
-    if (bf == bl) {
-      if (bf != cur) {
-        if (cur >= 0) flush();
-        cur = bf;
-      }
-      s[0] += xv[0]; s[1] += xv[1]; s[2] += xv[2]; s[3] += ok ? 1.f : 0.f;
-    } else {
-      if (cur >= 0) flush();
-      cur = -1;
-      const int bb = ok ? b : -1;
-      float v[4] = {xv[0], xv[1], xv[2], ok ? 1.f : 0.f};
-#pragma unroll
-      for (int off = 1; off < 64; off <<= 1) {
-        const int bu = __shfl_up(bb, off);
-        float u[4];
-#pragma unroll
-        for (int k = 0; k < 4; ++k) u[k] = __shfl_up(v[k], off);
-        if (l >= off && bu == bb) {
-#pragma unroll
-          for (int k = 0; k < 4; ++k) v[k] += u[k];
-        }
-      }
-      const int bn = __shfl_down(bb, 1);
-      if (ok && (l == 63 || bn != bb)) {
-#pragma unroll
-        for (int k = 0; k < 4; ++k) atomicAdd(&xsum[b * 4 + k], v[k]);
-      }
-    }
-  }
-  if (cur >= 0) flush();
-}
-
+  }
+  return a;
+}
+__device__ __forceinline__ void xsum_combine(const float *x, const float *part, const int32_t *batch, const int32_t *gptr, int N,
+                                             int NB, int b, float *red, float out[4]) {
+  if (!part) part = g_xsum_part;
+  int lo, hi;
+  if (gptr) {
+    lo = min(max(gptr[b], 0), N);
+    hi = min(max(gptr[b + 1], lo), N);
+  } else {
+    lo = xsum_lower_bound(batch, N, b);
+    hi = xsum_lower_bound(batch, N, b + 1);
+  }
+  int fb = (lo + NB - 1) / NB, lb = hi / NB;
+  if (fb >= lb) fb = lb = hi / NB + 1;
+  const int nhead = min(hi, fb * NB) - lo, nblk = lb - fb, nitems = hi - lo - nblk * (NB - 1);
+  float s[3] = {0.f, 0.f, 0.f};
+  for (int i = threadIdx.x; i < nitems; i += 256) {
+    const float *p = i < nhead ? x + (size_t)(lo + i) * 3
+                               : (i < nhead + nblk ? part + (size_t)(fb + i - nhead) * 4 : x + (size_t)(lb * NB + i - nhead - nblk) * 3);
+#pragma unroll
+    for (int k = 0; k < 3; ++k) s[k] += p[k];
+  }
+#pragma unroll
+  for (int k = 0; k < 3; ++k)
+    for (int off = 32; off > 0; off >>= 1) s[k] += __shfl_xor(s[k], off);
+  const int l = lane_id(), w = threadIdx.x >> 6;
+  if (l < 3) red[w * 4 + l] = s[l];
+  __syncthreads();
+#pragma unroll
+  for (int k = 0; k < 3; ++k) out[k] = (red[k] + red[4 + k]) + (red[8 + k] + red[12 + k]);
+  out[3] = (float)(hi - lo);
+}
+__device__ __forceinline__ float xsum_pick(const float v[4], int k) { return k == 0 ? v[0] : (k == 1 ? v[1] : (k == 2 ? v[2] : v[3])); }
+__global__ __launch_bounds__(256) void graph_xsum_combine_kernel(const float *x, const int32_t *batch, const int32_t *gptr, int N, int NB,
+                                                                 float *xsum) {
+  __shared__ float red[16];
+  float v[4];
+  xsum_combine(x, nullptr, batch, gptr, N, NB, blockIdx.x, red, v);
+  if (threadIdx.x < 4) xsum[blockIdx.x * 4 + threadIdx.x] = xsum_pick(v, threadIdx.x);
+}
+
+int graph_xsum_partials(const fastegnn_layer_t *L, float *part, hipStream_t st) {
+  FE_REQUIRE(L->x && (L->gptr || L->batch), "graph_xsum: null buffer");
+  if (L->N == 0) return FASTEGNN_OK;
+  const int NB = xsum_block_nodes(L->N);
+  { ProfScope _ps_graph_xsum_kernel(K_XSUM, st); hipLaunchKernelGGL(graph_xsum_part_kernel, dim3(cdiv(cdiv(L->N, NB), 4)), dim3(256), 0, st, L->x, L->N, NB, part); }
+  return check_launch("graph_xsum_part_kernel");
+}
 int graph_xsum(const fastegnn_layer_t *L, hipStream_t st) {
-  FE_REQUIRE(L->xsum && L->batch && L->x, "graph_xsum: null buffer");
-  (void)hipMemsetAsync(L->xsum, 0, (size_t)L->B * 4 * sizeof(float), st);
-  int per_wave = (cdiv(L->N, 64) + 63) / 64 * 64;
-  per_wave = per_wave < 64 ? 64 : (per_wave > XSUM_PER_WAVE ? XSUM_PER_WAVE : per_wave);
-  if (L->N > 0) { ProfScope _ps_graph_xsum_kernel(K_XSUM, st); hipLaunchKernelGGL(graph_xsum_kernel, dim3(cdiv(L->N, 4 * per_wave)), dim3(256), 0, st, L->x, L->batch, L->N, L->xsum, per_wave); }
-  return check_launch("graph_xsum_kernel");
+  FE_REQUIRE(L->xsum, "graph_xsum: null buffer");
+  int rc = graph_xsum_partials(L, nullptr, st);
+  if (rc || L->B == 0) return rc;
+  { ProfScope _ps_graph_xsum_kernel(K_XSUM, st); hipLaunchKernelGGL(graph_xsum_combine_kernel, dim3(L->B), dim3(256), 0, st, L->x, L->batch, L->gptr, L->N, xsum_block_nodes(L->N), L->xsum); }
+  return check_launch("graph_xsum_combine_kernel");
 }
 
 struct GraphPreArgs {
   const float *xsum, *Z, *HvT, *V0W, *V0B;
   float *Bc;
   int B, C, bf16;
+  const float *x, *part;
+  const int32_t *batch, *gptr;
+  int N, NB;
+  float *xsum_out, *poolV, *poolX;
 };
 constexpr int GP_SPLIT = 4;
+constexpr int GP_WLD = H + 1;
+static size_t graph_pre_lds_floats(int C) { return (size_t)3 * C + C * C + H * GP_WLD + (size_t)H * (C + 1) + (size_t)C * H + 16; }
 __global__ __launch_bounds__(256) void graph_pre_fwd_kernel(GraphPreArgs a) {
   extern __shared__ float sm[];
   const int C = a.C, b = blockIdx.x, ld = 2 * H + 1 + C;
   float *mz = sm;
-  float *mX = sm + 3 * C;
-  const float cnt = fmaxf(a.xsum[b * 4 + 3], 1.f);
+  float *mX = mz + 3 * C;
+  float *wb = mX + C * C;
+  float *wd = wb + H * GP_WLD;
+  float *hv = wd + H * (C + 1);
+  float *red = hv + C * H;
+  for (int i = threadIdx.x; i < H * H; i += 256) wb[(i >> 6) * GP_WLD + (i & 63)] = a.V0W[(size_t)(i >> 6) * ld + H + (i & 63)];
+  for (int i = threadIdx.x; i < H * C; i += 256) wd[(i / C) * (C + 1) + i % C] = a.V0W[(size_t)(i / C) * ld + 2 * H + 1 + i % C];
+  for (int i = threadIdx.x; i < C * H; i += 256) hv[i] = a.HvT[(size_t)b * C * H + i];
+  float xs[4];
+  if (a.x) {
+    const int gid = (blockIdx.x * gridDim.y + blockIdx.y) * 256 + threadIdx.x, gstep = gridDim.x * gridDim.y * 256;
+    if (a.poolV) for (int i = gid; i < a.B * C * H; i += gstep) a.poolV[i] = 0.f;
+    for (int i = gid; i < a.B * 3 * C; i += gstep) a.poolX[i] = 0.f;
+    xsum_combine(a.x, a.part, a.batch, a.gptr, a.N, a.NB, b, red, xs);
+    if (blockIdx.y == 0 && threadIdx.x < 4) a.xsum_out[b * 4 + threadIdx.x] = xsum_pick(xs, threadIdx.x);
+  } else {
+#pragma unroll
+    for (int k = 0; k < 4; ++k) xs[k] = a.xsum[b * 4 + k];
+  }
+  const float cnt = fmaxf(xs[3], 1.f);
   for (int i = threadIdx.x; i < 3 * C; i += 256) {
     int k = i / C;
-    mz[i] = a.Z[(size_t)b * 3 * C + i] - a.xsum[b * 4 + k] / cnt;
+    mz[i] = a.Z[(size_t)b * 3 * C + i] - (k == 0 ? xs[0] : (k == 1 ? xs[1] : xs[2])) / cnt;
   }
   __syncthreads();
   for (int i = threadIdx.x; i < C * C; i += 256) {
@@ -194,20 +242,21 @@
   __syncthreads();
   for (int i = blockIdx.y * 256 + threadIdx.x; i < C * H; i += 256 * gridDim.y) {
     int c = i >> 6, o = i & 63;
-    const float *w = a.V0W + (size_t)o * ld;
-    const float *hv = a.HvT + ((size_t)b * C + c) * H;
+    const float *w = wb + o * GP_WLD, *h = hv + c * H;
     float acc = a.V0B[o];
-    if (a.bf16) { for (int k = 0; k < H; ++k) acc += round_bf(w[H + k]) * round_bf(hv[k]); }
-    else { for (int k = 0; k < H; ++k) acc += w[H + k] * hv[k]; }
-    for (int d = 0; d < C; ++d) acc += w[2 * H + 1 + d] * mX[d * C + c];
+    if (a.bf16) { for (int k = 0; k < H; ++k) acc += round_bf(w[k]) * round_bf(h[k]); }
+    else { for (int k = 0; k < H; ++k) acc += w[k] * h[k]; }
+    for (int d = 0; d < C; ++d) acc += wd[o * (C + 1) + d] * mX[d * C + c];
     a.Bc[((size_t)b * C + c) * H + o] = acc;
   }
 }
-int graph_pre_forward(const fastegnn_layer_t *L, hipStream_t st) {
+int graph_pre_forward(const fastegnn_layer_t *L, hipStream_t st, float *part) {
   FE_REQUIRE(L->xsum && L->Z && L->HvT && L->Bc, "graph_pre_forward: null buffer");
+  FE_REQUIRE(!part || (L->x && L->poolX && (L->gptr || L->batch)), "graph_pre_forward: null buffer");
   GraphPreArgs a{L->xsum, L->Z, L->HvT, L->params[FASTEGNN_P_VIRT0_W], L->params[FASTEGNN_P_VIRT0_B], L->Bc, L->B, L->C,
-                 has(L, FASTEGNN_F_BF16) ? 1 : 0};
-  const size_t lds = (size_t)(3 * L->C + L->C * L->C) * sizeof(float);
+                 has(L, FASTEGNN_F_BF16) ? 1 : 0, part ? L->x : nullptr, part, L->batch, L->gptr, L->N, xsum_block_nodes(L->N),
+                 L->xsum, L->poolV, L->poolX};
+  const size_t lds = graph_pre_lds_floats(L->C) * sizeof(float);
   { ProfScope _ps_graph_pre_fwd_kernel(K_GRAPH_PRE_FWD, st); hipLaunchKernelGGL(graph_pre_fwd_kernel, dim3(L->B, GP_SPLIT), dim3(256), lds, st, a); }
   return check_launch("graph_pre_fwd_kernel");
 }
@@ -338,7 +387,7 @@
 #include "virt_fwd.h"
 namespace fe {
 
-int virt_forward(const fastegnn_layer_t *L, hipStream_t st) {
+int virt_forward(const fastegnn_layer_t *L, hipStream_t st, bool pools_zeroed) {
   const bool egnn = has(L, FASTEGNN_F_EGNN);
   const bool node = egnn || has(L, FASTEGNN_F_RF) || L->h_out;
   FE_REQUIRE(node || !L->HvT_out, "virt_forward: h_out is null and HvT_out is not (both null: no node update; otherwise neither)");
@@ -348,7 +397,7 @@
   FE_REQUIRE(egnn ? L->C == 0 : (L->Bc && L->Z && (!node || L->poolV) && L->poolX && L->C >= 1 && L->C <= 64),
              "virt_forward: virtual_channels must be in [1,64] (0 with FASTEGNN_F_EGNN) and the virtual buffers non-null");
   FE_REQUIRE(L->na == 0 || L->node_attr, "virt_forward: node_attr null");
-  if (L->C > 0) {
+  if (L->C > 0 && !pools_zeroed) {
     if (node) (void)hipMemsetAsync(L->poolV, 0, (size_t)L->B * L->C * H * sizeof(float), st);
     (void)hipMemsetAsync(L->poolX, 0, (size_t)L->B * 3 * L->C * sizeof(float), st);
   }
@@ -382,8 +431,8 @@
 };
 __global__ __launch_bounds__(256) void graph_post_fwd_kernel(GraphPostArgs a) {
   const bool bf = a.flags & FASTEGNN_F_BF16;
-  const int l = lane_id(), j = l & 15, q = l >> 4;
-  const int wave = global_wave_id(), nwaves = (gridDim.x * blockDim.x) >> 6;
+  __shared__ __attribute__((aligned(16))) float xt[16 * TS];
+  const int l = lane_id(), j = l & 15, q = l >> 4, w = wave_id();
   const int M = a.B * a.C, ntiles = (M + 15) >> 4;
   for (int i = blockIdx.x * blockDim.x + threadIdx.x; i < a.B * 3 * a.C; i += gridDim.x * blockDim.x) {
     const int b = i / (3 * a.C);
@@ -393,7 +442,11 @@
     for (int i = blockIdx.x * blockDim.x + threadIdx.x; i < M * H; i += gridDim.x * blockDim.x) a.HvT_out[i] = a.HvT[i];
     return;
   }
-  for (int tile = wave; tile < ntiles; tile += nwaves) {
+  f32x4 f5a[4], f5b[4], f6[4];
+  gemm64_frags(a.wpack + (size_t)I_W5A * IMG, w, f5a);
+  gemm64_frags(a.wpack + (size_t)I_W5B * IMG, w, f5b);
+  gemm64_frags(a.wpack + (size_t)I_W6 * IMG, w, f6);
+  for (int tile = blockIdx.x; tile < ntiles; tile += gridDim.x) {
     const int m = tile * 16 + j;
     const bool valid = m < M;
     const int mc = valid ? m : M - 1;
@@ -401,14 +454,17 @@
     const float inv = 1.0f / fmaxf(a.xsum[b * 4 + 3], 1.f);
     const Vec hv = vload_row(a.HvT + (size_t)mc * H, q);
     const Vec pm = vscale(vload_row(a.poolV + (size_t)mc * H, q), inv);
-    Vec z5 = vload_vec(a.b5, q);
-    gemm64(a.wpack + (size_t)I_W5A * IMG, bf ? vround(hv) : hv, z5);
-    gemm64(a.wpack + (size_t)I_W5B * IMG, bf ? vround(pm) : pm, z5);
-    Vec out = vload_vec(a.b6, q);
-    const Vec u5 = vsilu(z5 FE_ACT(a));
-    gemm64(a.wpack + (size_t)I_W6 * IMG, bf ? vround(u5) : u5, out);
-    if (a.flags & FASTEGNN_F_RESIDUAL) vadd(out, hv);
-    if (valid) vstore_row(a.HvT_out + (size_t)m * H, q, out);
+    f32x4 z5 = vload_block(a.b5, w, q);
+    gemm64_block(f5a, bf ? vround(hv) : hv, z5);
+    gemm64_block(f5b, bf ? vround(pm) : pm, z5);
+    vstore_block(xt + j * TS, w, q, vblock(z5, [&](const Vec &v) { return vsilu(v FE_ACT(a)); }));
+    __syncthreads();
+    const Vec u5 = vload_row(xt + j * TS, q);
+    f32x4 out = vload_block(a.b6, w, q);
+    gemm64_block(f6, bf ? vround(u5) : u5, out);
+    if (a.flags & FASTEGNN_F_RESIDUAL) out += vload_block(a.HvT + (size_t)mc * H, w, q);
+    if (valid) vstore_block(a.HvT_out + (size_t)m * H, w, q, out);
+    __syncthreads();
   }
 }
 __global__ __launch_bounds__(256) void graph_post_fwd_coords_kernel(const float *xsum, const float *Z, const float *poolX, float *Z_out,
@@ -432,7 +488,7 @@
              "graph_post_forward: null buffer");
   GraphPostArgs a{L->xsum, L->Z, L->HvT, L->poolV, L->poolX, L->wpack, L->params[FASTEGNN_P_NODEV0_B],
                   L->params[FASTEGNN_P_NODEV2_B], L->Z_out, L->HvT_out, L->B, L->C, L->flags, L->act_param};
-  int grid = cdiv(cdiv((long)L->B * L->C, 16), 4);
+  int grid = cdiv((long)L->B * L->C, 16);
   if (grid > 256) grid = 256;
   if (grid < 1) grid = 1;
   { ProfScope _ps_graph_post_fwd_kernel(K_GRAPH_POST_FWD, st); hipLaunchKernelGGL(graph_post_fwd_kernel, dim3(grid), dim3(256), 0, st, a); }
diff --git a/fastegnn_amd/csrc/misc.hip b/fastegnn_amd/csrc/misc.hip
--- a/fastegnn_amd/csrc/misc.hip
+++ b/fastegnn_amd/csrc/misc.hip
@@ -455,55 +455,87 @@
   long M;
   int ldg, ldf, kf, lddw, c0, rows_per_wg;
 };
-__global__ __launch_bounds__(256) void wgrad_small_kernel(WgsArgs a) {
-  const int o = threadIdx.x & 63, w = wave_id();
+constexpr int WGS_U = 8, WGS_WAVES = 8;
+template <int KF>
+__global__ __launch_bounds__(64 * WGS_WAVES) void wgrad_small_kernel(WgsArgs a) {
+  constexpr int KA = KF > 0 ? KF : 1;
+  const int l = lane_id(), w = wave_id(), sub = l >> 4, o4 = (l & 15) * 4;
   const long m0 = (long)blockIdx.x * a.rows_per_wg;
   long m1 = m0 + a.rows_per_wg;
   if (m1 > a.M) m1 = a.M;
-  double acc[8] = {0, 0, 0, 0, 0, 0, 0, 0};
-  double bs = 0.;
-  long m = m0 + w;
-  for (; m + 12 < m1; m += 16) {
-    float g[4];
-#pragma unroll
-    for (int u = 0; u < 4; ++u) g[u] = a.G[(size_t)(m + 4 * u) * a.ldg + o];
-#pragma unroll
-    for (int u = 0; u < 4; ++u) {
-      bs += (double)g[u];
-#pragma unroll
-      for (int k = 0; k < 8; ++k)
-        if (k < a.kf) acc[k] += (double)g[u] * (double)a.F[(size_t)(m + 4 * u) * a.ldf + k];
-    }
-  }
-  for (; m < m1; m += 4) {
-    const float g = a.G[(size_t)m * a.ldg + o];
-    bs += (double)g;
-#pragma unroll
-    for (int k = 0; k < 8; ++k)
-      if (k < a.kf) acc[k] += (double)g * (double)a.F[(size_t)m * a.ldf + k];
-  }
-  __shared__ double red[4][9][H];
-#pragma unroll
-  for (int k = 0; k < 8; ++k) red[w][k][o] = acc[k];
-  red[w][8][o] = bs;
+  double acc[KA][4], bs[4] = {0., 0., 0., 0.};
+#pragma unroll
+  for (int k = 0; k < KA; ++k)
+#pragma unroll
+    for (int c = 0; c < 4; ++c) acc[k][c] = 0.;
+  for (long mb = m0 + 4 * w; mb < m1; mb += 4 * WGS_WAVES * WGS_U) {
+    f32x4 g[WGS_U];
+    float f[WGS_U][KA];
+#pragma unroll
+    for (int u = 0; u < WGS_U; ++u) {
+      const long r = mb + 4 * WGS_WAVES * u + sub;
+      const bool ok = r < m1;
+      const size_t rc = (size_t)(ok ? r : m0);
+      g[u] = *reinterpret_cast<const f32x4 *>(a.G + rc * a.ldg + o4);
+      if (!ok) g[u] = f32x4{0.f, 0.f, 0.f, 0.f};
+#pragma unroll
+      for (int k = 0; k < KF; ++k) f[u][k] = a.F[rc * a.ldf + k];
+    }
+#pragma unroll
+    for (int u = 0; u < WGS_U; ++u)
+#pragma unroll
+      for (int c = 0; c < 4; ++c) {
+        const double gd = (double)g[u][c];
+        bs[c] += gd;
+#pragma unroll
+        for (int k = 0; k < KF; ++k) acc[k][c] += gd * (double)f[u][k];
+      }
+  }
+  __shared__ double red[WGS_WAVES][KA + 1][H];
+  auto rows4 = [&](double v) {
+    v += __shfl_xor(v, 16);
+    return v + __shfl_xor(v, 32);
+  };
+#pragma unroll
+  for (int c = 0; c < 4; ++c) {
+#pragma unroll
+    for (int k = 0; k < KF; ++k) {
+      const double s = rows4(acc[k][c]);
+      if (sub == 0) red[w][k][o4 + c] = s;
+    }
+    const double s = rows4(bs[c]);
+    if (sub == 0) red[w][KA][o4 + c] = s;
+  }
   __syncthreads();
+  const int o = l;
+  auto waves8 = [&](int k) {
+    return ((red[0][k][o] + red[1][k][o]) + (red[2][k][o] + red[3][k][o])) + ((red[4][k][o] + red[5][k][o]) + (red[6][k][o] + red[7][k][o]));
+  };
   if (w == 0) {
-    for (int k = 0; k < a.kf; ++k)
-      atomicAdd(&a.dW[(size_t)o * a.lddw + a.c0 + k], (float)((red[0][k][o] + red[1][k][o]) + (red[2][k][o] + red[3][k][o])));
-    if (a.db) atomicAdd(&a.db[o], (float)((red[0][8][o] + red[1][8][o]) + (red[2][8][o] + red[3][8][o])));
-  }
+#pragma unroll
+    for (int k = 0; k < KF; ++k) atomicAdd(&a.dW[(size_t)o * a.lddw + a.c0 + k], (float)waves8(k));
+    if (a.db) atomicAdd(&a.db[o], (float)waves8(KA));
+  }
+}
+template <int KF>
+static void wgrad_small_launch(const WgsArgs &a, unsigned grid, hipStream_t st) {
+  if constexpr (KF < 8) {
+    if (a.kf > KF) return wgrad_small_launch<KF + 1>(a, grid, st);
+  }
+  hipLaunchKernelGGL(wgrad_small_kernel<KF>, dim3(grid), dim3(64 * WGS_WAVES), 0, st, a);
 }
 static int launch_wgrad_small_b(const float *G, int ldg, const float *F, int ldf, int kf, long M, float *dW, int lddw,
                                 int c0, float *db, hipStream_t st) {
   if (M <= 0 || !dW) return FASTEGNN_OK;
   FE_REQUIRE(kf >= 0 && kf <= 8, "wgrad_small: kf > 8 unsupported");
+  FE_REQUIRE(reinterpret_cast<uintptr_t>(G) % 16 == 0 && ldg % 4 == 0, "wgrad_small: G rows must be 16-byte aligned");
   WgsArgs a{G, F, dW, db, M, ldg, ldf, kf, lddw, c0, 0};
   long nsplit = (M + 255) / 256;
   if (nsplit > 256) nsplit = 256;
   long rows = (M + nsplit - 1) / nsplit;
   a.rows_per_wg = (int)rows;
   nsplit = (M + rows - 1) / rows;
-  { ProfScope _ps_wgrad_small_kernel(K_WGRAD_SMALL, st); hipLaunchKernelGGL(wgrad_small_kernel, dim3((unsigned)nsplit), dim3(256), 0, st, a); }
+  { ProfScope _ps_wgrad_small_kernel(K_WGRAD_SMALL, st); wgrad_small_launch<0>(a, (unsigned)nsplit, st); }
   return check_launch("wgrad_small_kernel");
 }
 int launch_dgrad_small(const float *G, long N, int kf, const float *W, int ldw, int c0, float *g_in, int accumulate,
diff --git a/fastegnn_amd/csrc/virt_bwd.hip b/fastegnn_amd/csrc/virt_bwd.hip
--- a/fastegnn_amd/csrc/virt_bwd.hip
+++ b/fastegnn_amd/csrc/virt_bwd.hip
@@ -1526,7 +1526,7 @@
   return bb.finish();
 }
 
-int virt_backward(const fastegnn_layer_t *L, hipStream_t st, WgradBatch *shared) {
+int virt_backward(const fastegnn_layer_t *L, hipStream_t st, WgradBatch *shared, bool acc_zeroed) {
   const bool egnn = has(L, FASTEGNN_F_EGNN), rf = has(L, FASTEGNN_F_RF);
   const bool node = egnn || rf || L->g_h_out;
   FE_REQUIRE(node || !L->g_HvT_out, "virt_backward: g_h_out is null and g_HvT_out is not (both null: no gradient for h / Hv; otherwise neither)");
@@ -1539,7 +1539,7 @@
                   : (L->Bc && L->Z && (rf || !node || L->g_poolV) && L->g_poolX && L->g_Bc && L->g_Zp && L->wg_virt && L->C >= 1 && L->C <= 64),
              "virt_backward: virtual buffers null or virtual_channels outside [1,64] (0 with FASTEGNN_F_EGNN)");
   const int N = L->N, C = L->C;
-  if (C > 0) {
+  if (C > 0 && !acc_zeroed) {
     (void)hipMemsetAsync(L->g_Bc, 0, (size_t)L->B * C * H * sizeof(float), st);
     (void)hipMemsetAsync(L->g_Zp, 0, (size_t)L->B * 3 * C * sizeof(float), st);
   }
```

After: 99.90 graphs/s, median of 6. 1.02x the previous value.
